# urbste/OpenImuCameraCalibrator

Measured on AMD Instinct MI355X. Metric: residual+Jacobian blocks/sec; wall-clock per LM iter, GoPro9 full calib, higher is better.
Workload: dtype f64

## Files before the change

include/oicc_hip.h:

```cpp
#ifndef OICC_HIP_H_
#define OICC_HIP_H_

#include <stdint.h>

#ifdef __cplusplus
extern "C" {
#endif

#define OICC_SPLINE_N 6
#define OICC_BIAS_SPLINE_N 3

typedef struct oicc_problem oicc_problem;

typedef enum oicc_status {
  OICC_OK = 0,
  OICC_ERR_INVALID_ARG = -1,
  OICC_ERR_NO_DEVICE = -2,
  OICC_ERR_HIP = -3,
  OICC_ERR_STATE = -4,
  OICC_ERR_UNSUPPORTED = -5
} oicc_status;

typedef enum oicc_camera_model {
  OICC_CAM_PINHOLE = 0,
// ... 189 lines not shown
int oicc_get_imu_intrinsics(const oicc_problem* p, double accl[6], double gyro[9]);
int oicc_get_bias_knots(const oicc_problem* p, double* accl_xyz, int64_t n_accl,
                        double* gyro_xyz, int64_t n_gyro);
int64_t oicc_get_num_accl_bias_knots(const oicc_problem* p);
int64_t oicc_get_num_gyro_bias_knots(const oicc_problem* p);
int oicc_get_mean_reprojection_error(oicc_problem* p, double* mean_px,
                                     int64_t* num_points);
int oicc_get_trajectory(oicc_problem* p, int64_t n, const int64_t* t_ns,
                        double* pose7, double* gyro3, double* accel3,
                        double* gyro_bias3, double* accl_bias3, uint8_t* valid);


int oicc_sew_knot_spacing_and_variance(int32_t device_ordinal, int32_t dims, int64_t n, const double* signal,
                                       const double* times, double quality, double min_dt, double max_dt,
                                       double* dt, double* variance, int32_t* num_evaluations);


int oicc_estimate_imu_to_camera_rotation(int32_t device_ordinal, int64_t n_vis, const double* t_vis_s, const double* q_vis_xyzw,
                                         int64_t n_imu, const double* t_imu_s, const double* gyro_xyz, double dt_imu,
                                         int32_t estimate_gyro_bias, double q_imu_to_cam_xyzw[4], double* time_offset_imu_to_cam,
                                         double gyro_bias[3], double* alignment_error, int32_t* iterations);

enum { OICC_ALLAN_GYRO = 0, OICC_ALLAN_ACC = 1, OICC_ALLAN_REPORT_SIZE = 6 };
int oicc_allan_factors(int64_t n, int32_t num_clusters, int32_t* factors, int32_t* num_factors);
int oicc_allan_variance(int32_t device_ordinal, int32_t channels, int64_t n, const double* samples, const double* t_s,
                        const double* scale, int32_t num_clusters, int32_t* num_factors, int32_t* factors, double* taus,
                        double* sigma2, double* freq, double* period, double* mean, double* device_ms);
int oicc_allan_fit(int32_t kind, int64_t num, const double* taus, const double* sigma2, double freq, double params_QNBKR[5],
                   double init_C[5], double report[6], int32_t* num_used, int32_t* iterations);

typedef struct oicc_ba oicc_ba;
enum { OICC_BA_POSITION = 1, OICC_BA_ORIENTATION = 2,
       OICC_BA_POINTS = 4 };
int oicc_ba_create(oicc_ba** out, int32_t device_ordinal);
void oicc_ba_destroy(oicc_ba* p);
const char* oicc_ba_last_error(const oicc_ba* p);
int oicc_ba_set_option(oicc_ba* p, const char* name, double value);
int oicc_ba_set_camera(oicc_ba* p, int32_t model, const double* intrinsics, int32_t n);
int oicc_ba_get_camera(const oicc_ba* p, double* intrinsics, int32_t n);
int oicc_ba_set_scene_points(oicc_ba* p, const double* xyzw, int64_t n);
int oicc_ba_get_scene_points(const oicc_ba* p, double* xyzw, int64_t n);
int oicc_ba_set_variable_points(oicc_ba* p, const uint8_t* variable, int64_t n);
int oicc_ba_set_views(oicc_ba* p, int64_t nv, const double* pose6, const int64_t* corner_offsets, const double* uv,
                      const int32_t* point_ids);
int oicc_ba_set_poses(oicc_ba* p, const double* pose6, int64_t nv);
int oicc_ba_get_poses(const oicc_ba* p, double* pose6, int64_t nv);
int oicc_ba_evaluate(oicc_ba* p, int32_t flags, int32_t intrinsics_mask, double* cost, double* H, double* g, int32_t Pcap);
int oicc_ba_optimize(oicc_ba* p, int32_t max_iters, int32_t flags, int32_t intrinsics_mask, oicc_summary* summary);
int oicc_ba_get_iterations(const oicc_ba* p, oicc_iteration* out, int32_t cap);
int oicc_ba_optimize_views(oicc_ba* p, int32_t max_iters, int32_t flags, int32_t* iterations, double* final_cost);
int oicc_ba_point_covariances(oicc_ba* p, double* cov9, int64_t n, double* variance_factor);
typedef struct oicc_ba_covariance_info {
  int32_t status;
  int32_t P, pose_dim, a;
  int32_t views_used;
  int32_t first_bad;
  int64_t num_residuals;
  double cost, variance_factor, rcond;
} oicc_ba_covariance_info;
int oicc_ba_estimate_covariance(oicc_ba* p, int32_t flags, int32_t intrinsics_mask, oicc_ba_covariance_info* info);
int oicc_ba_get_covariance_intrinsics(const oicc_ba* p, double* cov, int32_t a_capacity);
int oicc_ba_get_covariance_poses(const oicc_ba* p, double* blocks, int64_t nv);
int oicc_ba_get_covariance_pose_intrinsics(const oicc_ba* p, double* cross, int64_t nv);
int oicc_ba_get_covariance_timing(const oicc_ba* p, double ms[2]);
int oicc_ba_view_reprojection_errors(oicc_ba* p, double* mean_px);

enum {
  OICC_SIMU_THRESHOLDS = 10,
  OICC_SIMU_ACC_IMPOSSIBLE = 1,
  OICC_SIMU_TERM_SKIPPED = -1,
  OICC_SIMU_TERM_GRADIENT = 0,
  OICC_SIMU_TERM_FUNCTION = 1,
  OICC_SIMU_TERM_PARAMETER = 2,
  OICC_SIMU_TERM_MAX_ITERATIONS = 3,
  OICC_SIMU_TERM_MIN_RADIUS = 4,
  OICC_SIMU_TERM_INVALID_STEPS = 5,
  OICC_SIMU_TERM_EVAL_FAILED = 6
};
typedef struct oicc_static_imu_options {
  double gravity_magnitude;
  double init_interval_duration_s;
  double gyro_dt;
  int32_t interval_n_samples;
  int32_t min_num_intervals;
  int32_t win_size;
  int32_t acc_use_means;
  int32_t optimize_gyro_bias;
  int32_t reserved;
} oicc_static_imu_options;
typedef struct oicc_static_imu_report {
  int32_t th_mult;
  int32_t num_intervals[OICC_SIMU_THRESHOLDS];
  int32_t acc_iterations[OICC_SIMU_THRESHOLDS];
  int32_t acc_termination[OICC_SIMU_THRESHOLDS];
  int32_t gyro_num_blocks, gyro_iterations, gyro_termination;
  double norm_th;
  double init_acc_bias[3];
  double acc_final_cost[OICC_SIMU_THRESHOLDS];
  double gyro_init_bias[3];
  double gyro_initial_cost, gyro_final_cost;
  double ms_detector, ms_acc, ms_gyro;
} oicc_static_imu_report;
int oicc_static_imu_intervals(int32_t device_ordinal, int64_t n, const double* acc, int32_t num_thresholds,
                              const double* thresholds, int32_t win_size, int32_t capacity, int32_t* counts,
                              int32_t* intervals, double* norms, double* device_ms);
int oicc_static_imu_eval_acc(int32_t device_ordinal, int64_t num, const double* samples, double g_mag, const double* params,
                             double* residuals, double* jacobian, double* cost, double* gram, double* gradient);
int oicc_static_imu_eval_gyro(int32_t device_ordinal, int64_t n, const double* t_s, const double* gyro, int32_t num_blocks,
                              const int32_t* ranges, const double* g_versors, int32_t optimize_bias, double gyro_dt,
                              const double* params, double* residuals, double* jacobian, double* cost, double* gram,
                              double* gradient, double* device_ms);
int oicc_static_imu_calibrate(int32_t device_ordinal, int64_t n, const double* t_s, const double* acc, const double* gyro,
                              const oicc_static_imu_options* opt, double* acc_params, double* gyro_params,
                              oicc_static_imu_report* report);

typedef struct oicc_board_options {
  int32_t radius;
  float threshold_rel;
  int32_t max_candidates;
  int32_t subpix_iterations;
  double subpix_eps;
  int32_t batch;
  int32_t reserved;
} oicc_board_options;
typedef struct oicc_board_report {
  int32_t frames_found, frames_overflow;
  int32_t output_width, output_height;
  int64_t num_candidates;
  double ms_resize, ms_response, ms_candidates, ms_subpix, ms_marker;
  double ms_assembly_host;
  double ms_total;
} oicc_board_report;
typedef struct oicc_board_stages {
  uint8_t* gray;
  float* response;
  int32_t* candidates;
  double* refined;
  int32_t capacity;
  int32_t reserved;
} oicc_board_stages;
int oicc_board_output_size(int32_t width, int32_t height, double downsample_factor, int32_t* out_width, int32_t* out_height);
int oicc_board_radon_detect(int32_t device_ordinal, int32_t num_frames, int32_t width, int32_t height, int32_t channels,
                            const uint8_t* frames, double downsample_factor, int32_t W, int32_t H,
                            const oicc_board_options* opt, double* corners, int32_t* found, int32_t* candidates_per_frame,
                            oicc_board_report* report, const oicc_board_stages* stages);

int oicc_planar_ransac(int32_t device_ordinal, int32_t num_views, const int64_t* corner_offsets, const double* ab, const double* xy,
                       int32_t mode, double threshold, int32_t num_hypotheses, uint64_t seed, uint8_t* inlier,
                       int32_t* num_inliers, double* q, double* pose, int32_t* hypothesis_counts, double* device_ms);

int oicc_debug_bcr_plan(int32_t n, int32_t ghost, int32_t odd_only, int64_t* levels, int32_t cap_levels, int64_t info[3]);
int oicc_debug_bcr_join_plan(int32_t n, int32_t ghost, int32_t odd_only, int32_t b0, int32_t rtf, int32_t join_levels, int32_t budget,
                             int32_t build_inverts, int32_t* joined, int32_t cap_levels);

#ifdef __cplusplus
}
#endif
#endif
```

openimucameracalibrator_amd/_abi.py:

```python
import ctypes as C

c_i64p = C.POINTER(C.c_int64)
c_i32p = C.POINTER(C.c_int32)
c_dp = C.POINTER(C.c_double)
c_u8p = C.POINTER(C.c_uint8)


class Summary(C.Structure):
    _fields_ = [
        ("termination", C.c_int32), ("num_iterations", C.c_int32),
        ("num_successful_steps", C.c_int32), ("num_unsuccessful_steps", C.c_int32),
        ("num_parameters_tangent", C.c_int32), ("band_dim", C.c_int32),
        ("arrow_dim", C.c_int32), ("half_bandwidth", C.c_int32),
        ("num_residual_blocks", C.c_int64), ("num_residuals", C.c_int64),
        ("initial_cost", C.c_double), ("final_cost", C.c_double),
        ("final_radius", C.c_double), ("final_gradient_max_norm", C.c_double),
        ("seconds_total", C.c_double), ("seconds_jacobian", C.c_double),
        ("seconds_residual", C.c_double), ("seconds_linear_solver", C.c_double),
        ("message", C.c_char * 128),
        ("inner_sweeps", C.c_int32), ("line_search_steps", C.c_int32), ("inner_lm_iterations", C.c_int64),
        ("seconds_inner", C.c_double),
        ("seconds_setup", C.c_double),
    ]

# ... 151 lines not shown
    "view_reprojection_errors": (C.c_int, [HB, c_dp]),
    "point_covariances": (C.c_int, [HB, c_dp, C.c_int64, c_dp]),
    "estimate_covariance": (C.c_int, [HB, C.c_int32, C.c_int32, C.POINTER(BaCovarianceInfo)]),
    "get_covariance_intrinsics": (C.c_int, [HB, c_dp, C.c_int32]),
    "get_covariance_poses": (C.c_int, [HB, c_dp, C.c_int64]),
    "get_covariance_pose_intrinsics": (C.c_int, [HB, c_dp, C.c_int64]),
    "get_covariance_timing": (C.c_int, [HB, c_dp]),
}
BA_DEVICE_ONLY = ("point_covariances", "estimate_covariance", "get_covariance_intrinsics", "get_covariance_poses",
                  "get_covariance_pose_intrinsics", "get_covariance_timing")


class BoundBa:

    def __init__(self, lib, prefix):
        self.lib = lib
        self.prefix = prefix
        for name, (res, args) in BA_SIGNATURES.items():
            if name in BA_DEVICE_ONLY and prefix != "oicc_ba_" and not hasattr(lib, prefix + name):
                continue
            fn = getattr(lib, prefix + name)
            fn.restype = res
            fn.argtypes = args
            setattr(self, name, fn)


class Bound:

    def __init__(self, lib, prefix, device=True):
        self.lib = lib
        self.prefix = prefix
        table = dict(SIGNATURES)
        if device:
            table.update(DEVICE_ONLY)
        for name, (res, args) in table.items():
            fn = getattr(lib, prefix + name)
            fn.restype = res
            fn.argtypes = args
            setattr(self, name, fn)
        self.device = device


INNER_DEBUG_SIGNATURES = {
    "oicc_debug_inner_first_evaluations": (C.c_int, [H, C.c_int32, c_i32p, c_dp, C.c_int32]),
    "oicc_debug_inner_cholesky": (C.c_int, [C.c_int32, C.c_int32, C.c_int64, c_dp, c_dp, c_dp, c_u8p]),
}
INNER_ROUTES = ("set_kernel<0>", "set_kernel<1>", "set_kernel<2>", "wave_kernel", "shared: resident workgroups", "shared: launches")
INNER_KINDS = ("so3", "r3", "T_i_c", "gravity", "line_delay", "accl_bias", "gyro_bias", "accl_intrinsics", "gyro_intrinsics", "point")


def bind_inner_debug(lib, name):
    fn = getattr(lib, name)
    fn.restype, fn.argtypes = INNER_DEBUG_SIGNATURES[name]
    return fn


ALLAN_SIGNATURES = {
    "factors": (C.c_int, [C.c_int64, C.c_int32, c_i32p, c_i32p]),
    "variance": (C.c_int, [C.c_int32, C.c_int32, C.c_int64, c_dp, c_dp, c_dp, C.c_int32, c_i32p, c_i32p, c_dp,
                           c_dp, c_dp, c_dp, c_dp, c_dp]),
    "fit": (C.c_int, [C.c_int32, C.c_int64, c_dp, c_dp, C.c_double, c_dp, c_dp, c_dp, c_i32p, c_i32p]),
}


class BoundAllan:

    def __init__(self, lib, prefix):
        self.lib = lib
        self.prefix = prefix
        for name, (res, args) in ALLAN_SIGNATURES.items():
            fn = getattr(lib, prefix + name)
            fn.restype = res
            fn.argtypes = args
            setattr(self, name, fn)


class StaticImuOptions(C.Structure):
    _fields_ = [("gravity_magnitude", C.c_double), ("init_interval_duration_s", C.c_double), ("gyro_dt", C.c_double),
                ("interval_n_samples", C.c_int32), ("min_num_intervals", C.c_int32), ("win_size", C.c_int32),
                ("acc_use_means", C.c_int32), ("optimize_gyro_bias", C.c_int32), ("reserved", C.c_int32)]


class StaticImuReport(C.Structure):
    _fields_ = [("th_mult", C.c_int32), ("num_intervals", C.c_int32 * 10), ("acc_iterations", C.c_int32 * 10),
                ("acc_termination", C.c_int32 * 10), ("gyro_num_blocks", C.c_int32), ("gyro_iterations", C.c_int32),
                ("gyro_termination", C.c_int32), ("norm_th", C.c_double), ("init_acc_bias", C.c_double * 3),
                ("acc_final_cost", C.c_double * 10), ("gyro_init_bias", C.c_double * 3), ("gyro_initial_cost", C.c_double),
                ("gyro_final_cost", C.c_double), ("ms_detector", C.c_double), ("ms_acc", C.c_double), ("ms_gyro", C.c_double)]


STATIC_IMU_SIGNATURES = {
    "intervals": (C.c_int, [C.c_int32, C.c_int64, c_dp, C.c_int32, c_dp, C.c_int32, C.c_int32, c_i32p, c_i32p, c_dp, c_dp]),
    "eval_acc": (C.c_int, [C.c_int32, C.c_int64, c_dp, C.c_double, c_dp, c_dp, c_dp, c_dp, c_dp, c_dp]),
    "eval_gyro": (C.c_int, [C.c_int32, C.c_int64, c_dp, c_dp, C.c_int32, c_i32p, c_dp, C.c_int32, C.c_double, c_dp, c_dp, c_dp,
                            c_dp, c_dp, c_dp, c_dp]),
    "calibrate": (C.c_int, [C.c_int32, C.c_int64, c_dp, c_dp, c_dp, C.POINTER(StaticImuOptions), c_dp, c_dp,
                            C.POINTER(StaticImuReport)]),
}


class BoundStaticImu:

    def __init__(self, lib, prefix):
        self.lib = lib
        self.prefix = prefix
        for name, (res, args) in STATIC_IMU_SIGNATURES.items():
            fn = getattr(lib, prefix + name)
            fn.restype = res
            fn.argtypes = args
            setattr(self, name, fn)


class BoardOptions(C.Structure):
    _fields_ = [("radius", C.c_int32), ("threshold_rel", C.c_float), ("max_candidates", C.c_int32), ("subpix_iterations", C.c_int32),
                ("subpix_eps", C.c_double), ("batch", C.c_int32), ("reserved", C.c_int32)]


class BoardReport(C.Structure):
    _fields_ = [("frames_found", C.c_int32), ("frames_overflow", C.c_int32), ("output_width", C.c_int32), ("output_height", C.c_int32),
                ("num_candidates", C.c_int64), ("ms_resize", C.c_double), ("ms_response", C.c_double), ("ms_candidates", C.c_double),
                ("ms_subpix", C.c_double), ("ms_marker", C.c_double), ("ms_assembly_host", C.c_double), ("ms_total", C.c_double)]

    def as_dict(self):
        return {k: getattr(self, k) for k, _ in self._fields_}


class BoardStages(C.Structure):
    _fields_ = [("gray", c_u8p), ("response", C.POINTER(C.c_float)), ("candidates", c_i32p), ("refined", c_dp),
                ("capacity", C.c_int32), ("reserved", C.c_int32)]


BOARD_SIGNATURES = {
    "output_size": (C.c_int, [C.c_int32, C.c_int32, C.c_double, c_i32p, c_i32p]),
    "radon_detect": (C.c_int, [C.c_int32, C.c_int32, C.c_int32, C.c_int32, C.c_int32, c_u8p, C.c_double, C.c_int32, C.c_int32,
                               C.POINTER(BoardOptions), c_dp, c_i32p, c_i32p, C.POINTER(BoardReport), C.POINTER(BoardStages)]),
}


class BoundBoard:

    def __init__(self, lib, prefix):
        self.lib = lib
        self.prefix = prefix
        for name, (res, args) in BOARD_SIGNATURES.items():
            fn = getattr(lib, prefix + name)
            fn.restype = res
            fn.argtypes = args
            setattr(self, name, fn)


BCR_PLAN_SIGNATURES = {
    "plan": (C.c_int, [C.c_int32, C.c_int32, C.c_int32, c_i64p, C.c_int32, c_i64p]),
    "join_plan": (C.c_int, [C.c_int32] * 8 + [c_i32p, C.c_int32]),
}


class BoundBcrPlan:

    def __init__(self, lib, prefix):
        self.lib = lib
        self.prefix = prefix
        for name, (res, args) in BCR_PLAN_SIGNATURES.items():
            fn = getattr(lib, prefix + name)
            fn.restype = res
            fn.argtypes = args
            setattr(self, name, fn)


LM_RETRACT_SIGNATURES = {
    "retract": (C.c_int, [C.c_void_p, C.c_int32, C.c_double, c_i64p] + [c_dp] * 9),
}


class BoundLmRetract:

    def __init__(self, lib, prefix):
        self.lib = lib
        self.prefix = prefix
        for name, (res, args) in LM_RETRACT_SIGNATURES.items():
            fn = getattr(lib, prefix + name)
            fn.restype = res
            fn.argtypes = args
            setattr(self, name, fn)


PLANAR_RANSAC_SIGNATURES = {
    "ransac": (C.c_int, [C.c_int32, C.c_int32, c_i64p, c_dp, c_dp, C.c_int32, C.c_double, C.c_int32, C.c_uint64, c_u8p, c_i32p, c_dp,
                         c_dp, c_i32p, c_dp]),
}


class BoundPlanarRansac:

    def __init__(self, lib, prefix):
        self.lib = lib
        self.prefix = prefix
        for name, (res, args) in PLANAR_RANSAC_SIGNATURES.items():
            fn = getattr(lib, prefix + name)
            fn.restype = res
            fn.argtypes = args
            setattr(self, name, fn)
```

openimucameracalibrator_amd/csrc/kernels_bcr.hip:

```cpp
#include <hip/hip_runtime.h>
#include <mutex>
#include <unordered_map>
#include "oicc_device.h"
#include "lm_decide.h"
#include "lm_launch.h"
#include "lm_retract.h"
#include "../../include/oicc_hip.h"

namespace oicc {


struct BcrArgs {
  double* D;
  double* F;
  double* S;
  double* Lf;
  double* Mc;
  double* x;
  int32_t* fail;
  long long* prof;
  int n, a, Pb, rtf, LD;
  int delay;
  int o, s, p, m, pn;
  int64_t offS_in, offS_out;
  int carry;
  int last;
  int side;
  int top_l, top_r;
  int b0, ghost;
  const LmCtl* ctl;
};
#define BCR_RETURN_IF_DONE(A) do { if ((A).ctl != nullptr && (A).ctl->done != 0) return; } while (0)

__device__ __forceinline__ void bcr_lds_barrier() { asm volatile("s_waitcnt lgkmcnt(0)\n\ts_barrier" ::: "memory"); }
__device__ __forceinline__ double bcr_readlane(double v, int lane) {
  const int lo = __builtin_amdgcn_readlane(__double2loint(v), lane);
  const int hi = __builtin_amdgcn_readlane(__double2hiint(v), lane);
  return __hiloint2double(hi, lo);
}
typedef double bcr_v4d __attribute__((ext_vector_type(4)));

__device__ __forceinline__ void tri10(int t, int& xt, int& yt) {
  xt = t < 1 ? 0 : (t < 3 ? 1 : (t < 6 ? 2 : 3));
  yt = t - (xt * (xt + 1)) / 2;
}

template <int LD>
__device__ __forceinline__ void bcr_corner_solve(double* C, double* da, int* failp, int a, int tid, int wave, int lane) {
  const int a1 = a + 1;
  if (a1 <= 16) {
    if (wave == 0) {
      double av[16], dinv = 0.0;
#pragma unroll
      for (int c = 0; c < 16; ++c) av[c] = (c < a && lane < a1 && lane >= c) ? C[c * LD + lane] : 0.0;
      bool bad = false;
#pragma unroll
      for (int c = 0; c < 16; ++c) {
        if (c < a) {
          const double piv = bcr_readlane(av[c], c);
          bad |= !(piv > 0.0);
          const double y0 = __builtin_amdgcn_rsq(piv);
          const double g0 = piv * y0, h0 = 0.5 * y0;
          const double r0 = fma(-g0, h0, 0.5);
          const double g1 = fma(g0, r0, g0), h1 = fma(h0, r0, h0);
          const double r1 = fma(-g1, h1, 0.5);
          const double u = (av[c] + av[c]) * h1;
          const double l = fma(u, r1, u);
          av[c] = l;
          if (lane == c) { const double y1 = h1 + h1; dinv = fma(y1, r1, y1); }
#pragma unroll
          for (int c2 = c + 1; c2 < 16; ++c2) {
            const double lc2 = bcr_readlane(l, c2);
            av[c2] = fma(-l, lc2, av[c2]);
          }
        }
      }
#pragma unroll
      for (int c = 0; c < 16; ++c) if (c < a && lane < a1 && lane >= c) C[c * LD + lane] = av[c];
      double lt[16];
#pragma unroll
      for (int q = 0; q < 16; ++q) lt[q] = (q < a && lane < q) ? C[lane * LD + q] : 0.0;
      double z = lane < a ? C[lane * LD + a] : 0.0, xq_mine = 0.0;
#pragma unroll
      for (int q = 15; q >= 0; --q) {
        if (q < a) {
          const double xq = bcr_readlane(z * dinv, q);
          if (lane == q) xq_mine = xq;
          z = fma(-lt[q], xq, z);
        }
      }
      if (lane < a) da[lane] = xq_mine;
      if (bad && lane == 0) *failp = 1;
    }
    __syncthreads();
    return;
  }
  if (wave == 0) {
    bool bad = false;
    for (int c = 0; c < a; ++c) {
      double* col = C + c * LD;
      const double mine = lane < a1 ? col[lane] : 0.0;
      double piv = bcr_readlane(mine, c);
      if (!(piv > 0.0)) { bad = true; piv = 1.0; }
      const double d = sqrt(piv);
      const double l = lane == c ? d : (lane > c ? mine / d : 0.0);
      if (lane >= c && lane < a1) col[lane] = l;
      for (int c2 = c + 1; c2 < a; ++c2) {
        const double l2 = bcr_readlane(l, c2);
        if (lane >= c2 && lane < a1) C[c2 * LD + lane] -= l * l2;
      }
    }
    if (bad && lane == 0) *failp = 1;
    double z = lane < a ? C[lane * LD + a] : 0.0;
    const double dc = lane < a ? 1.0 / C[lane * LD + lane] : 0.0;
    double xq_mine = 0.0;
    for (int q = a - 1; q >= 0; --q) {
      const double xq = bcr_readlane(z * dc, q);
      if (lane == q) xq_mine = xq;
      const double l = lane < q ? C[lane * LD + q] : 0.0;
      z = fma(-l, xq, z);
    }
    if (lane < a) da[lane] = xq_mine;
  }
  __syncthreads();
}

constexpr int kBackWaves = 8;
constexpr int kInvWaves = 16;
constexpr int kInvLD = 145;

template <int XT>
__device__ __forceinline__ bcr_v4d bcri_z_tile(const double* W, int yt, int li, int lq) {
  constexpr int LD = kInvLD, K0 = 4 * XT, NK = 16 - K0;
  const double* py = W + lq * LD + 64 + 16 * yt + li;
  const double* px = W + lq * LD + 64 + 16 * XT + li;
  double vy[NK], vx[NK];
#pragma unroll
  for (int kk = 0; kk < NK; ++kk) { vy[kk] = py[4 * (K0 + kk) * LD]; vx[kk] = px[4 * (K0 + kk) * LD]; }
  asm volatile("" ::: "memory");
  bcr_v4d g = {0.0, 0.0, 0.0, 0.0}, g2 = {0.0, 0.0, 0.0, 0.0};
#pragma unroll
  for (int kk = 0; kk < NK; kk += 2) {
    g = __builtin_amdgcn_mfma_f64_16x16x4f64(vy[kk], vx[kk], g, 0, 0, 0);
    g2 = __builtin_amdgcn_mfma_f64_16x16x4f64(vy[kk + 1], vx[kk + 1], g2, 0, 0, 0);
  }
  g += g2;
  return g;
}

template <bool LAST, bool ZLDS>
__device__ __forceinline__ void bcri_tail(const BcrArgs& A, double* W, double* da, int* failp, const double* Fs, double* Zg, int tid, int wave, int lane, bool report,
                                          const double (&ttop)[16], const double ytop, double* x0s) {
  constexpr int LD = kInvLD, NW = kInvWaves, NT = 64 * NW, FLD = 65;
  const int li = lane & 15, lq = lane >> 4;
  const int a = A.a, a1 = a + 1;
  for (int t = wave; t < 10; t += NW) {
    int xt, yt; tri10(t, xt, yt);
    const bcr_v4d g = xt == 0 ? bcri_z_tile<0>(W, yt, li, lq) : (xt == 1 ? bcri_z_tile<1>(W, yt, li, lq) : (xt == 2 ? bcri_z_tile<2>(W, yt, li, lq) : bcri_z_tile<3>(W, yt, li, lq)));
#pragma unroll
    for (int r = 0; r < 4; ++r) {
      const int x = 16 * xt + li, y = 16 * yt + lq + 4 * r;
      if (LAST || ZLDS) { W[y * LD + x] = g[r]; if (xt != yt) W[x * LD + y] = g[r]; }
      else { Zg[y * 64 + x] = g[r]; if (xt != yt) Zg[x * 64 + y] = g[r]; }
    }
  }
  __syncthreads();
  if (!LAST) {
    if (report && tid == 0 && *failp) atomicOr(A.fail, 1);
    return;
  }
  const int rtf = A.rtf;
  if (wave < 4 * rtf) {
    const int t = wave >> 2, w = wave & 3;
    const double* pf = Fs + lq * FLD + 16 * t + li;
    const double* pz = W + lq * LD + 16 * w + li;
    double vf[16], vz[16];
#pragma unroll
    for (int kk = 0; kk < 16; ++kk) { vf[kk] = pf[4 * kk * FLD]; vz[kk] = pz[4 * kk * LD]; }
    asm volatile("" ::: "memory");
    bcr_v4d tq = {0.0, 0.0, 0.0, 0.0};
#pragma unroll
    for (int kk = 0; kk < 16; ++kk) tq = __builtin_amdgcn_mfma_f64_16x16x4f64(vf[kk], vz[kk], tq, 0, 0, 0);
#pragma unroll
    for (int r = 0; r < 4; ++r) W[(16 * w + li) * LD + 64 + 16 * t + lq + 4 * r] = tq[r];
  }
  __syncthreads();
  if (wave < (rtf * (rtf + 1)) / 2) {
    int t1 = 0, u = wave; while (u >= t1 + 1) { u -= t1 + 1; ++t1; }
    const int t2 = u;
    const double* pt = W + lq * LD + 64 + 16 * t1 + li;
    const double* pf = Fs + lq * FLD + 16 * t2 + li;
    double vt[16], vf[16];
#pragma unroll
    for (int kk = 0; kk < 16; ++kk) { vt[kk] = pt[4 * kk * LD]; vf[kk] = pf[4 * kk * FLD]; }
    asm volatile("" ::: "memory");
    bcr_v4d g = {0.0, 0.0, 0.0, 0.0};
#pragma unroll
    for (int kk = 0; kk < 16; ++kk) g = __builtin_amdgcn_mfma_f64_16x16x4f64(vf[kk], vt[kk], g, 0, 0, 0);
    const double* Sm = A.side != 0 ? A.Lf + (int64_t)A.last * (192 + a1) * 64 + 4096 + 64 * a1 : nullptr;
    double mc[4];
#pragma unroll
    for (int r = 0; r < 4; ++r) { const int q1 = 16 * t1 + li, q2 = 16 * t2 + lq + 4 * r; mc[r] = (q1 < a1 && q2 < a1) ? A.Mc[q1 * a1 + q2] + (Sm != nullptr ? Sm[q1 * a1 + q2] : 0.0) : 0.0; }
#pragma unroll
    for (int r = 0; r < 4; ++r) { const int q1 = 16 * t1 + li, q2 = 16 * t2 + lq + 4 * r; if (q1 < a1 && q2 < a1) W[q2 * LD + q1] = mc[r] - g[r]; }
  }
  __syncthreads();
  bcr_corner_solve<LD>(W, da, failp, a, tid, wave, lane);
  for (int q = tid; q < a; q += NT) A.x[A.Pb + q] = da[q];
  if (wave == 0) {
    const double* tc = W + lane * LD + 64;
    double v = tc[a];
    for (int q = 0; q < a; q += 8) {
      double t8[8], d8[8];
#pragma unroll
      for (int k = 0; k < 8; ++k) { const bool ok = q + k < a; t8[k] = ok ? tc[q + k] : 0.0; d8[k] = ok ? da[q + k] : 0.0; }
#pragma unroll
      for (int k = 0; k < 8; ++k) v = fma(-t8[k], d8[k], v);
    }
    const int gi = A.last * 64 + lane;
    if (gi < A.Pb) A.x[gi] = v;
    x0s[lane] = gi < A.Pb ? v : 0.0;
  }
  __syncthreads();
  if (tid == 0 && *failp) atomicOr(A.fail, 1);
  if (A.top_l >= 0 || A.top_r >= 0) {
    double sum_r = 0.0, sum_l = 0.0;
#pragma unroll
    for (int k = 0; k < 4; ++k) {
      const int r = wave + NW * k;
      const double xn = x0s[r], xa = r < a ? da[r] : 0.0;
      sum_r = fma(ttop[k], xn, sum_r);     sum_r = fma(ttop[4 + k], xa, sum_r);
      sum_l = fma(ttop[8 + k], xn, sum_l); sum_l = fma(ttop[12 + k], xa, sum_l);
    }
    W[wave * 64 + lane] = sum_r;
    W[(NW + wave) * 64 + lane] = sum_l;
    __syncthreads();
    if (wave < 2) {
      const int blk = wave == 0 ? A.top_r : A.top_l;
      double acc = 0.0;
#pragma unroll
      for (int w = 0; w < NW; ++w) acc += W[(wave * NW + w) * 64 + lane];
      const int gi = blk * 64 + lane;
      if (blk >= 0 && gi < A.Pb) A.x[gi] = ytop - acc;
    }
  }
}


struct BcrNoPark { __device__ __forceinline__ void operator()(double*) const {} };
template <bool LAST, bool PROF, bool ZLDS = false, class LoadD, class Park = BcrNoPark>
__device__ __forceinline__ void bcri_invert_body(const BcrArgs& A, const int i, LoadD load_d, const bool report = true, Park park = Park()) {
  constexpr int LD = kInvLD, NW = kInvWaves, NT = 64 * NW, NTILE = 20, SLOTS = (NTILE + NW - 1) / NW, RU = 128, NAW = 3, FLD = 65;
  static_assert(NW == 16, "the corner phases of block 0 take one tile per wave");
  extern __shared__ double lds[];
  const int tid = threadIdx.x, lane = tid & 63;
  const int wave = __builtin_amdgcn_readfirstlane(tid >> 6);
  const int li = lane & 15, lq = lane >> 4;
  double* const W = lds;
  double* const da = W + 64 * LD;
  int* const failp = reinterpret_cast<int*>(da + 64);
  double* const dg = da + 64 + 8;
  double* const Fs = dg + 256;
  const int a1 = A.a + 1;
  double* Zg = A.Lf + (int64_t)i * (192 + a1) * 64;
  const double* Fg = A.F + (int64_t)i * 64 * a1;
  const double* Sf = (LAST && A.side != 0) ? Zg + 4096 : nullptr;
  const bool prof = PROF && A.prof != nullptr && blockIdx.x == 0 && wave == 0;
  long long pc[8] = {0, 0, 0, 0, 0, 0, 0, 0};
  long long tprev = prof ? clock64() : 0;
#define BCR_MARK(k) do { if (PROF && prof) { const long long tn_ = clock64(); pc[k] += tn_ - tprev; tprev = tn_; } } while (0)
  if (tid == 0) *failp = 0;
  double ttop[16], ytop = 0.0;
#pragma unroll
  for (int k = 0; k < 16; ++k) ttop[k] = 0.0;
  if (LAST && (A.top_l >= 0 || A.top_r >= 0)) {
    const int64_t ru64 = (int64_t)(192 + a1) * 64;
    const double* Tr = A.Lf + (A.top_r >= 0 ? A.top_r : 0) * ru64 + 4096;
    const double* Tl = A.Lf + (A.top_l >= 0 ? A.top_l : 0) * ru64 + 4096;
#pragma unroll
    for (int k = 0; k < 4; ++k) {
      const int r = wave + NW * k;
      if (A.top_r >= 0) { ttop[k] = Tr[r * 64 + lane]; if (r < A.a) ttop[4 + k] = Tr[(128 + r) * 64 + lane]; }
      if (A.top_l >= 0) { ttop[8 + k] = Tl[(64 + r) * 64 + lane]; if (r < A.a) ttop[12 + k] = Tl[(128 + r) * 64 + lane]; }
    }
    if (wave == 0 && A.top_r >= 0) ytop = Tr[(128 + A.a) * 64 + lane];
    if (wave == 1 && A.top_l >= 0) ytop = Tl[(128 + A.a) * 64 + lane];
    asm volatile("" ::: "memory");
  }
  {
    constexpr int PER = 4096 / NT;
    double gd[PER], gf[PER];
#pragma unroll
    for (int k = 0; k < PER; ++k) {
      const int e = tid + k * NT;
      gd[k] = load_d(e);
      if (LAST) { const int c = e >> 6, q = e & 63; gf[k] = q < a1 ? Fg[c * a1 + q] + (Sf != nullptr ? Sf[c * a1 + q] : 0.0) : 0.0; }
    }
#pragma unroll
    for (int k = 0; k < PER; ++k) {
      const int e = tid + k * NT;
      const int c = e >> 6, r = e & 63;
      W[c * LD + r] = r >= c ? gd[k] : 0.0;
      if (c < 16 && r < 16) dg[c * 16 + r] = r >= c ? gd[k] : 0.0;
      W[c * LD + 64 + r] = r == c ? 1.0 : 0.0;
      if (LAST) Fs[c * FLD + r] = gf[k];
    }
    park(Fs);
  }
  __syncthreads();
  int t_rt[SLOTS], t_ct[SLOTS]; bool t_ok[SLOTS];
  bcr_v4d acc[SLOTS];
#pragma unroll
  for (int k = 0; k < SLOTS; ++k) {
    const int t = wave + NW * k;
    t_ok[k] = t < NTILE;
    int xt, yt; tri10(t < 10 ? t : (t < NTILE ? t - 10 : 0), xt, yt);
    if (t < 10) { t_rt[k] = xt; t_ct[k] = yt; } else { t_rt[k] = 4 + yt; t_ct[k] = xt; }
    const double* src = W + (16 * t_ct[k] + lq) * LD + 16 * t_rt[k] + li;
    acc[k][0] = src[0]; acc[k][1] = src[4 * LD]; acc[k][2] = src[8 * LD]; acc[k][3] = src[12 * LD];
  }
  BCR_MARK(0);
  const int prow = 16 + wave * 48 + (lane - 16);
  for (int p = 0; p < 4; ++p) {
    const int j0 = 16 * p;
    if (wave < NAW) {
      const int rho = lane < 16 ? j0 + lane : prow;
      const bool act = lane < 16 || (rho >= j0 + 16 && rho < RU && !(rho >= 64 && rho - 64 > j0 + 15));
      if (A.delay > 0 && wave > 0) for (int k = 0; k < A.delay; ++k) __builtin_amdgcn_s_sleep(16);
      const double* colp = lane < 16 ? dg + lane : W + j0 * LD + (act ? rho : 0);
      const int cstride = lane < 16 ? 16 : LD;
      double av[16];
#pragma unroll
      for (int c = 0; c < 16; ++c) { const double v = colp[c * cstride]; av[c] = (act && (lane >= 16 || lane >= c)) ? v : 0.0; }
      if (PROF && prof) { asm volatile("s_waitcnt lgkmcnt(0)" ::: "memory"); }
      BCR_MARK(6);
      bool bad = false;
#pragma unroll
      for (int c = 0; c < 16; ++c) {
        const double piv = bcr_readlane(av[c], c);
        bad |= !(piv > 0.0);
        const double y0 = __builtin_amdgcn_rsq(piv);
        const double g0 = piv * y0, h0 = 0.5 * y0;
        const double r0 = fma(-g0, h0, 0.5);
        const double g1 = fma(g0, r0, g0), h1 = fma(h0, r0, h0);
        const double r1 = fma(-g1, h1, 0.5);
        const double u = (av[c] + av[c]) * h1;
        const double l = fma(u, r1, u);
        av[c] = l;
#pragma unroll
        for (int c2 = c + 1; c2 < 16; ++c2) {
          const double lc2 = bcr_readlane(l, c2);
          av[c2] = fma(-l, lc2, av[c2]);
        }
      }
      if (PROF && prof) { asm volatile("s_nop 0" :: "v"(av[15])); }
      BCR_MARK(7);
      if (act && (lane >= 16 || wave == 0)) {
        double* cp = W + j0 * LD + rho;
#pragma unroll
        for (int c = 0; c < 16; ++c) cp[c * LD] = av[c];
      }
      if (bad && lane == 0) *failp = 1;
    }
    BCR_MARK(1);
    bcr_lds_barrier();
    BCR_MARK(2);
    if (p < 3) {
#pragma unroll
      for (int k = 0; k < SLOTS; ++k) {
        if (t_ok[k] && t_ct[k] > p && (t_rt[k] < 4 || t_rt[k] - 4 <= p)) {
          const double* pa = W + (j0 + lq) * LD + 16 * t_ct[k] + li;
          const double* pb = W + (j0 + lq) * LD + 16 * t_rt[k] + li;
          double va[4], vb[4];
#pragma unroll
          for (int kq = 0; kq < 4; ++kq) { va[kq] = pa[4 * kq * LD]; vb[kq] = -pb[4 * kq * LD]; }
#pragma unroll
          for (int kq = 0; kq < 4; ++kq) acc[k] = __builtin_amdgcn_mfma_f64_16x16x4f64(va[kq], vb[kq], acc[k], 0, 0, 0);
          if (t_ct[k] == p + 1) {
            double* dst = W + (16 * t_ct[k] + lq) * LD + 16 * t_rt[k] + li;
            dst[0] = acc[k][0]; dst[4 * LD] = acc[k][1]; dst[8 * LD] = acc[k][2]; dst[12 * LD] = acc[k][3];
            if (t_rt[k] == t_ct[k]) { dg[lq * 16 + li] = acc[k][0]; dg[(lq + 4) * 16 + li] = acc[k][1]; dg[(lq + 8) * 16 + li] = acc[k][2]; dg[(lq + 12) * 16 + li] = acc[k][3]; }
          }
        }
      }
    }
    BCR_MARK(3);
    bcr_lds_barrier();
    BCR_MARK(4);
  }
  BCR_MARK(4);
  bcri_tail<LAST, ZLDS>(A, W, da, failp, Fs, Zg, tid, wave, lane, report, ttop, ytop, dg);
  BCR_MARK(5);
  if (PROF && prof && lane == 0) for (int k = 0; k < 8; ++k) A.prof[k] = pc[k];
#undef BCR_MARK
}

template <bool LAST, bool PROF>
__global__ __launch_bounds__(64 * kInvWaves) void bcri_invert_kernel(BcrArgs A) {
  BCR_RETURN_IF_DONE(A);
  const int i = LAST ? A.last : A.o + A.s * (2 * (int)blockIdx.x + A.p);
  const double* Dg = A.D + (int64_t)i * 4096;
  const double* Sd = (LAST && A.side != 0) ? A.Lf + (int64_t)i * (192 + A.a + 1) * 64 : nullptr;
  bcri_invert_body<LAST, PROF>(A, i, [Dg, Sd](int e) { double v = Dg[e]; if (LAST && Sd != nullptr && (e & 63) >= (e >> 6)) v += Sd[e]; return v; });
}

struct BcrSchurGroup {
  int k, i, irs;
  bool hasL, hasR, ghostR;
  int xk, xt, yk, ny;
  bool store_t;
  bool leaves;
};
__device__ __forceinline__ BcrSchurGroup bcri_schur_group(const BcrArgs& A, int g, int piv) {
  BcrSchurGroup G;
  const int rtf = A.rtf;
  G.k = 2 * piv + A.p;
  G.i = A.o + G.k * A.s;
  G.hasL = G.k > 0;
  G.ghostR = A.ghost != 0 && G.k == A.m - 1;
  G.hasR = G.k < A.m - 1 || G.ghostR;
  G.irs = G.ghostR ? A.n : G.i + A.s;
  if (g < 4) { G.xk = 0; G.xt = g; G.yk = 0; G.ny = g + 1; G.store_t = true; }
  else if (g < 8) { G.xk = 1; G.xt = g - 4; G.yk = 0; G.ny = 4; G.store_t = false; }
  else if (g < 12) { G.xk = 1; G.xt = g - 8; G.yk = 1; G.ny = G.xt + 1; G.store_t = true; }
  else { g -= 12; G.yk = g / rtf; G.xt = g - G.yk * rtf; G.xk = 2; G.ny = G.yk < 2 ? 4 : G.xt + 1; G.store_t = G.yk == (G.hasL ? 0 : 1); }
  G.leaves = ((G.xk == 1 || G.yk == 1) && !G.hasR) || ((G.xk == 0 || G.yk == 0) && !G.hasL);
  return G;
}
struct BcrSchurGlobalOps {
  static constexpr bool kLateY = false;
  const double *px, *pz, *py; int sx, sy; bool okx, oky;
  __device__ __forceinline__ double x(int kk) const { return px[4 * kk * sx]; }
  __device__ __forceinline__ double z(int kk) const { return pz[4 * kk * 64]; }
  __device__ __forceinline__ double y(int kk) const { return oky ? py[4 * kk * sy] : 0.0; }
};
struct BcrSchurLdsOps {
  static constexpr bool kLateY = true;
  const double *px, *pz, *py; bool okx;
  __device__ __forceinline__ double x(int kk) const { return px[64 * kk]; }
  __device__ __forceinline__ double z(int kk) const { return pz[4 * kk * kInvLD]; }
  __device__ __forceinline__ double y(int kk) const { return py[64 * kk]; }
};
template <class Ops>
__device__ __forceinline__ void bcri_schur_body(const BcrArgs& A, const BcrSchurGroup& G, double (*Ts)[68], const Ops& ops, const bool active, const int wave, const int lane) {
  const int li = lane & 15, lq = lane >> 4;
  const int a1 = A.a + 1, s = A.s;
  const int k = G.k, i = G.i, il = i - s, irs = G.irs, xk = G.xk, xt = G.xt, yk = G.yk, ny = G.ny;
  const bool hasL = G.hasL, ghostR = G.ghostR, store_t = G.store_t, okx = ops.okx;
  double* Tg = A.Lf + (int64_t)i * (192 + a1) * 64 + 4096;
  double vx[16], vz[16], vy[16];
  if (active) {
#pragma unroll
    for (int kk = 0; kk < 16; ++kk) { vx[kk] = ops.x(kk); vz[kk] = ops.z(kk); }
    if (!Ops::kLateY) {
#pragma unroll
      for (int kk = 0; kk < 16; ++kk) vy[kk] = ops.y(kk);
    }
    asm volatile("" ::: "memory");
    bcr_v4d tq = {0.0, 0.0, 0.0, 0.0}, tq2 = {0.0, 0.0, 0.0, 0.0};
#pragma unroll
    for (int kk = 0; kk < 16; kk += 2) {
      tq = __builtin_amdgcn_mfma_f64_16x16x4f64(okx ? vx[kk] : 0.0, vz[kk], tq, 0, 0, 0);
      tq2 = __builtin_amdgcn_mfma_f64_16x16x4f64(okx ? vx[kk + 1] : 0.0, vz[kk + 1], tq2, 0, 0, 0);
    }
    tq += tq2;
    const int trow0 = xk == 0 ? 16 * xt : (xk == 1 ? 64 + 16 * xt : 128 + 16 * xt);
#pragma unroll
    for (int r = 0; r < 4; ++r) {
      const int row = lq + 4 * r;
      Ts[row][16 * wave + li] = tq[r];
      if (store_t && (xk != 2 || 16 * xt + row < a1)) Tg[(int64_t)(trow0 + row) * 64 + 16 * wave + li] = tq[r];
    }
  }
  __syncthreads();
  if (!active || wave >= ny) return;
  const int yt = wave;
  const int kn = hasL ? (k - 2 + A.p) / 2 : 0;
  const bool il_is_pivot = (kn & 1) == A.pn;
  const bool swap = xk == 1 && yk == 0 && !il_is_pivot && !ghostR;
  double vt[16];
  if (Ops::kLateY) {
#pragma unroll
    for (int kk = 0; kk < 16; ++kk) vy[kk] = ops.y(kk);
  }
#pragma unroll
  for (int kk = 0; kk < 16; ++kk) vt[kk] = Ts[li][4 * kk + lq];
  asm volatile("" ::: "memory");
  bcr_v4d gq = {0.0, 0.0, 0.0, 0.0}, gq2 = {0.0, 0.0, 0.0, 0.0};
  if (swap) {
#pragma unroll
    for (int kk = 0; kk < 16; kk += 2) {
      gq = __builtin_amdgcn_mfma_f64_16x16x4f64(vt[kk], vy[kk], gq, 0, 0, 0);
      gq2 = __builtin_amdgcn_mfma_f64_16x16x4f64(vt[kk + 1], vy[kk + 1], gq2, 0, 0, 0);
    }
  } else {
#pragma unroll
    for (int kk = 0; kk < 16; kk += 2) {
      gq = __builtin_amdgcn_mfma_f64_16x16x4f64(vy[kk], vt[kk], gq, 0, 0, 0);
      gq2 = __builtin_amdgcn_mfma_f64_16x16x4f64(vy[kk + 1], vt[kk + 1], gq2, 0, 0, 0);
    }
  }
  gq += gq2;
  const int ils = hasL ? il : i;
  double* Dl = A.D + (int64_t)ils * 4096; double* Dr = A.D + (int64_t)irs * 4096;
  double* Fl = A.F + (int64_t)ils * 64 * a1; double* Fr = A.F + (int64_t)irs * 64 * a1;
  double* So = A.S + (A.offS_out + kn) * 4096;
  const bool to_side = A.side != 0 && !hasL;
  double* Sd = A.Lf + (int64_t)irs * (192 + a1) * 64;
#pragma unroll
  for (int r = 0; r < 4; ++r) {
    const double v = -gq[r];
    if (xk == 1 && yk == 0) {
      if (!swap) { const int x = 16 * xt + li, y = 16 * yt + lq + 4 * r; So[y * 64 + x] = v; }
      else       { const int y = 16 * yt + li, x = 16 * xt + lq + 4 * r; So[x * 64 + y] = v; }
    } else if (xk < 2) {
      const int x = 16 * xt + li, y = 16 * yt + lq + 4 * r;
      if (to_side) { if (x >= y) Sd[y * 64 + x] = v; }
      else if (x >= y && v != 0.0) unsafeAtomicAdd((xk == 0 ? Dl : Dr) + y * 64 + x, v);
    } else if (yk < 2) {
      const int q = 16 * xt + li, y = 16 * yt + lq + 4 * r;
      if (to_side) { if (q < a1) Sd[4096 + y * a1 + q] = v; }
      else if (q < a1 && v != 0.0) unsafeAtomicAdd((yk == 0 ? Fl : Fr) + y * a1 + q, v);
    } else {
      const int q1 = 16 * xt + li, q2 = 16 * yt + lq + 4 * r;
      if (to_side) { if (q1 < a1 && q2 <= q1) { Sd[4096 + 64 * a1 + q1 * a1 + q2] = v; Sd[4096 + 64 * a1 + q2 * a1 + q1] = v; } }
      else if (q1 < a1 && q2 <= q1 && v != 0.0) {
        unsafeAtomicAdd(A.Mc + q1 * a1 + q2, v);
        if (q1 != q2) unsafeAtomicAdd(A.Mc + q2 * a1 + q1, v);
      }
    }
  }
}

__global__ __launch_bounds__(256) void bcri_schur_kernel(BcrArgs A) {
  BCR_RETURN_IF_DONE(A);
  __shared__ double Ts[16][68];
  const int tid = threadIdx.x, lane = tid & 63;
  const int wave = __builtin_amdgcn_readfirstlane(tid >> 6);
  const int li = lane & 15, lq = lane >> 4;
  const int a1 = A.a + 1;
  if ((int)blockIdx.y == (int)gridDim.y - 1 && A.carry > 0) {
    const int m = A.carry;
    const double* src = A.S + (A.offS_in + (m - 1)) * 4096; double* dst = A.S + (A.offS_out + (m - 1) / 2) * 4096;
    for (int e = (int)blockIdx.x * 256 + tid; e < 4096; e += (int)gridDim.x * 256) dst[e] = src[e];
    return;
  }
  const BcrSchurGroup G = bcri_schur_group(A, (int)blockIdx.x, (int)blockIdx.y);
  if (G.leaves) return;
  const double* SL = A.S + (A.offS_in + (G.hasL ? G.k - 1 : 0)) * 4096;
  const double* SR = A.S + (A.offS_in + G.k) * 4096;
  const double* Fg = A.F + (int64_t)G.i * 64 * a1;
  const double* Zg = A.Lf + (int64_t)G.i * (192 + a1) * 64;
  auto border_ptr = [&](int kind, int t, int& stride, bool& ok) -> const double* {
    if (kind == 0) { stride = 64; ok = true; return SL + lq * 64 + 16 * t + li; }
    if (kind == 1) { stride = 64; ok = true; return SR + lq * 64 + 16 * t + li; }
    const int q = 16 * t + li; ok = q < a1; stride = a1; return Fg + lq * a1 + (ok ? q : 0);
  };
  BcrSchurGlobalOps ops;
  ops.px = border_ptr(G.xk, G.xt, ops.sx, ops.okx);
  ops.py = border_ptr(G.yk, wave < G.ny ? wave : 0, ops.sy, ops.oky);
  ops.pz = Zg + lq * 64 + 16 * wave + li;
  bcri_schur_body(A, G, Ts, ops, true, wave, lane);
}

constexpr int kInvLdsDoubles = 64 * kInvLD + 64 + 8 + 256;
constexpr int kJoinLdsDoubles = kInvLdsDoubles + 5 * 1024 + 16 * 68;
__global__ __launch_bounds__(64 * kInvWaves) void bcri_invert_schur_kernel(BcrArgs A) {
  BCR_RETURN_IF_DONE(A);
  const BcrSchurGroup G = bcri_schur_group(A, (int)blockIdx.x, (int)blockIdx.y);
  if (G.leaves) return;
  const int tid = threadIdx.x, lane = tid & 63;
  const int wave = __builtin_amdgcn_readfirstlane(tid >> 6);
  const int li = lane & 15, lq = lane >> 4;
  const int a1 = A.a + 1;
  const double* SL = A.S + (A.offS_in + (G.hasL ? G.k - 1 : 0)) * 4096;
  const double* SR = A.S + (A.offS_in + G.k) * 4096;
  const double* Fg = A.F + (int64_t)G.i * 64 * a1;
  const int kv = tid >> 4, l = tid & 15;
  auto border_at = [&](int kind, int t) -> double {
    if (kind == 0) return SL[kv * 64 + 16 * t + l];
    if (kind == 1) return SR[kv * 64 + 16 * t + l];
    const int q = 16 * t + l; return q < a1 ? Fg[kv * a1 + q] : 0.0;
  };
  double bx = border_at(G.xk, G.xt), by[4];
#pragma unroll
  for (int t = 0; t < 4; ++t) by[t] = t < G.ny ? border_at(G.yk, t) : 0.0;
  asm volatile("" ::: "memory");
  const double* Dg = A.D + (int64_t)G.i * 4096;
  const bool report = (int)blockIdx.x == (G.hasL ? 0 : 8);
  bcri_invert_body<false, false, true>(A, G.i, [Dg](int e) { return Dg[e]; }, report,
    [&](double* P) {
      P[tid] = bx;
#pragma unroll
      for (int t = 0; t < 4; ++t) P[1024 * (1 + t) + tid] = by[t];
    });
  extern __shared__ double lds[];
  const double* W = lds;
  const double* P = lds + kInvLdsDoubles;
  double (*Ts)[68] = reinterpret_cast<double (*)[68]>(lds + kInvLdsDoubles + 5 * 1024);
  const bool active = wave < 4;
  BcrSchurLdsOps ops;
  ops.okx = true;
  ops.px = P + lq * 16 + li;
  ops.py = P + 1024 * (1 + (active && wave < G.ny ? wave : 0)) + lq * 16 + li;
  ops.pz = W + lq * kInvLD + 16 * (active ? wave : 0) + li;
  bcri_schur_body(A, G, Ts, ops, active, wave, lane);
}

struct BcrOwn {
  int e = -1, code = -1;
  double sc0 = 0.0, d2 = 0.0, g = 0.0;
  const double* x = nullptr; double* xc = nullptr;
};
constexpr int kRetractPark = 12;
template <int NB>
__device__ __forceinline__ BcrOwn bcr_retract_claim(const BcrArgs& A, const RetractReq& R, const SolveBuffers& sb, int b_lo, int b_hi, bool arrow_wg, int tid) {
  BcrOwn o; o.x = R.x; o.xc = R.xc;
  NormalEq ne = R.ne;
  if (A.ctl != nullptr) { o.x = A.ctl->xp[0]; o.xc = A.ctl->xp[1]; ne.base = A.ctl->nep[0]; }
  const int e_hi = b_hi * 64 < A.Pb ? b_hi * 64 : A.Pb;
  if (tid < 64 * NB) { const int e = b_lo * 64 + tid; if (e < e_hi) o.e = e; }
  else if (tid < 64 * NB + A.a && arrow_wg) o.e = A.Pb + (tid - 64 * NB);
  if (o.e >= 0) { o.code = R.rmap[o.e]; o.sc0 = sb.scale[o.e]; o.d2 = sb.D2[o.e]; o.g = ne.g()[o.e]; }
  return o;
}
__device__ __forceinline__ int bcr_rm_steps(int kind) { return kind == kRmEucl ? 1 : (kind == kRmTic ? 6 : 3); }
__device__ __forceinline__ int bcr_rm_params(int kind) { return kind == kRmEucl ? 1 : (kind == kRmTic ? 7 : (kind == kRmSo3 || kind == kRmPt ? 4 : 3)); }
__device__ __forceinline__ void bcr_retract_park(const SolveBuffers& sb, const BcrOwn& o, double* rpark, int stride, int tid) {
  if (o.code < 0) return;
  const int kind = o.code & 7; const int64_t po = o.code >> 3;
  const int nd = bcr_rm_steps(kind), np = bcr_rm_params(kind);
  for (int c = 0; c < np; ++c) rpark[c * stride + tid] = o.x[po + c];
  for (int c = 1; c < nd; ++c) rpark[(6 + c) * stride + tid] = sb.scale[o.e + c];
}
template <int OW>
__device__ __forceinline__ void bcr_retract_finish(const BcrArgs& A, const RetractReq& R, const SolveBuffers& sb, const BcrOwn& o, const double* xflat, int e_base,
                                                   const double* xarrow, const double* rpark, int stride, double* red, int tid, int wave, int lane) {
  __syncthreads();
  if (blockIdx.x == 0 && tid == 0) {
    if (A.ctl != nullptr) { if (A.ctl->stamps != nullptr && A.ctl->seq < A.ctl->trace_cap) A.ctl->stamps[3 * A.ctl->seq + 1] = wall_clock64(); }
    else *R.ne.cost() = 0.0;
  }
  double step_sq = 0.0, x_sq = 0.0, model = 0.0;
  if (o.e >= 0) {
    auto step_at = [&](int e) { return e >= A.Pb ? xarrow[e - A.Pb] : xflat[e - e_base]; };
    model = lm_model_term(step_at(o.e), o.d2, o.g, o.sc0);
    if (o.code >= 0) {
      const int kind = o.code & 7;
      const double alpha = R.alpha;
      const int nd = bcr_rm_steps(kind), np = bcr_rm_params(kind);
      double d[6], sc[6], pv[7];
#pragma unroll
      for (int c = 0; c < 6; ++c) { d[c] = c < nd ? step_at(o.e + c) : 0.0; sc[c] = c == 0 ? o.sc0 : (c < nd ? rpark[(6 + c) * stride + tid] : 0.0); }
#pragma unroll
      for (int c = 0; c < 7; ++c) pv[c] = c < np ? rpark[c * stride + tid] : 0.0;
      double* out = o.xc + (o.code >> 3);
      if (kind == kRmSo3) lm_store_so3(lm_retract_so3(Quat{pv[0], pv[1], pv[2], pv[3]}, d, sc, alpha), pv, out, step_sq, x_sq);
      else if (kind == kRmEucl) lm_retract_eucl(pv[0], d[0], sc[0], alpha, out, step_sq, x_sq);
      else if (kind == kRmAb || kind == kRmGb) { const double bound = kind == kRmAb ? R.max_ab : R.max_gb; for (int c = 0; c < 3; ++c) lm_retract_box(pv[c], d[c], sc[c], alpha, bound, out + c, step_sq, x_sq); }
      else if (kind == kRmPt) lm_retract_point(pv, d, sc, alpha, out, step_sq, x_sq);
      else if (kind == kRmTic) lm_retract_tic(pv, d, sc, alpha, out, step_sq, x_sq);
    }
  }
  if (wave < OW) {
#pragma unroll
    for (int off = 32; off > 0; off >>= 1) { step_sq += __shfl_xor(step_sq, off); x_sq += __shfl_xor(x_sq, off); model += __shfl_xor(model, off); }
    if (lane == 0) { red[wave] = step_sq; red[64 + wave] = x_sq; red[128 + wave] = model; }
  }
  __syncthreads();
  if (tid < 3) {
    double acc = 0.0;
    for (int w = 0; w < OW; ++w) acc += red[64 * tid + w];
    unsafeAtomicAdd(tid == 0 ? &sb.st->step_norm_sq : (tid == 1 ? &sb.st->x_norm_sq : &sb.st->model_cost_change), acc);
  }
}

__global__ __launch_bounds__(64 * kBackWaves) void bcri_backward_kernel(BcrArgs A) {
  BCR_RETURN_IF_DONE(A);
  __shared__ double xs[192];
  __shared__ double part[kBackWaves][64];
  const int tid = threadIdx.x, lane = tid & 63;
  const int wave = __builtin_amdgcn_readfirstlane(tid >> 6);
  const int a = A.a, a1 = a + 1, s = A.s;
  const int kp = 2 * (int)blockIdx.x + A.p;
  const int i = A.o + kp * s, il = i - s;
  const bool hasL = kp > 0;
  const bool hasR = kp < A.m - 1 || A.ghost != 0;
  const int ir = kp < A.m - 1 ? i + s : A.n;
  const double* Tg = A.Lf + (int64_t)i * (192 + a1) * 64 + 4096;
  constexpr int RW = 192 / kBackWaves;
  double lv[RW];
#pragma unroll
  for (int k = 0; k < RW; ++k) {
    const int r = wave + kBackWaves * k;
    const bool ok = r < 128 + a && (hasL || r >= 64) && (hasR || r < 64 || r >= 128);
    lv[k] = ok ? Tg[r * 64 + lane] : 0.0;
  }
  const double yv = wave == 0 ? Tg[(128 + a) * 64 + lane] : 0.0;
  double xin = 0.0;
  if (tid < 64) { const int gi = il * 64 + tid; xin = (hasL && gi < A.Pb) ? A.x[gi] : 0.0; }
  else if (tid < 128) { const int gi = ir * 64 + (tid - 64); xin = (hasR && gi < A.Pb) ? A.x[gi] : 0.0; }
  else if (tid < 128 + a) xin = A.x[A.Pb + (tid - 128)];
  if (tid < 192) xs[tid] = xin;
  __syncthreads();
  double sum = 0.0;
#pragma unroll
  for (int k = 0; k < RW; ++k) { const int r = wave + kBackWaves * k; sum = fma(lv[k], r < 128 + a ? xs[r] : 0.0, sum); }
  part[wave][lane] = sum;
  __syncthreads();
  if (wave == 0) {
    double acc = 0.0;
#pragma unroll
    for (int w = 0; w < kBackWaves; ++w) acc += part[w][lane];
    const int gi = i * 64 + lane;
    if (gi < A.Pb) A.x[gi] = yv - acc;
  }
}

template <bool RETRACT>
__device__ __forceinline__ void bcri_backward2_body(const BcrArgs& A, int ou, int pu, int mu, int npiv_upper, int orphan_l, int orphan_r, const RetractReq& R, const SolveBuffers& sb) {
  constexpr int NW = 16, RW1 = 192 / NW, RW2 = 192 / (NW / 2);
  __shared__ double xw[6][64];
  __shared__ double part[NW][64];
  double* const xs0 = xw[0]; double* const xs1 = xw[2]; double* const xs2 = xw[4]; double* const xs3 = xw[5];
  const int tid = threadIdx.x, lane = tid & 63;
  const int wave = __builtin_amdgcn_readfirstlane(tid >> 6);
  const int a = A.a, a1 = a + 1, s = A.s, n = A.n;
  const int64_t ru64 = (int64_t)(192 + a1) * 64;
  const int lone_ix = (int)blockIdx.x - npiv_upper;
  const bool lone = lone_ix >= 0;
  const bool lone_l = lone && orphan_l >= 0 && lone_ix == 0, lone_r = lone && !lone_l;
  const int ku = 2 * (int)blockIdx.x + pu;
  const int j = lone_l ? orphan_l - s : (lone_r ? orphan_r + s : ou + ku * 2 * s);
  const int jl = j - 2 * s, jr = j + 2 * s;
  const bool ghost = A.ghost != 0;
  const bool has_jl = lone_r || (!lone && ku > 0);
  const bool has_jr = lone_l || (!lone && (ku < mu - 1 || ghost));
  const int jrs = (!lone && ku == mu - 1) ? n : jr;
  const int half = wave >> 3, hw = wave & 7;
  const int ci = half == 0 ? j - s : j + s;
  const bool child = lone ? (half == 0 ? lone_r : lone_l) : (half == 0 ? ci >= A.o : ci <= A.o + (A.m - 1) * s);
  const bool child_hasL = half == 0 ? has_jl : !lone;
  const bool child_hasR = half == 0 ? (!lone || ghost) : has_jr;
  auto xin = [&](int blk, int r) { const int gi = blk * 64 + r; return gi < A.Pb ? A.x[gi] : 0.0; };
  if (tid < 64) xs0[tid] = has_jl ? xin(jl, tid) : 0.0;
  else if (tid < 128) xs2[tid - 64] = has_jr ? xin(jrs, tid - 64) : 0.0;
  else if (tid < 192) xs3[tid - 128] = tid - 128 < a ? A.x[A.Pb + (tid - 128)] : 0.0;
  else if (tid < 256 && lone) xs1[tid - 192] = (lone_r && ghost) ? xin(n, tid - 192) : 0.0;
  __shared__ double rpark[RETRACT ? kRetractPark : 1][384];
  BcrOwn own;
  if (RETRACT) {
    const int b_lo = j - 2 > 0 ? j - 2 : 0;
    int b_hi = j + 2 < n ? j + 2 : n;
    if (!lone && (int)blockIdx.x == npiv_upper - 1 && orphan_r < 0) b_hi = n;
    own = bcr_retract_claim<5>(A, R, sb, b_lo, b_hi, blockIdx.x == 0, tid);
  }
  double l1[RW1], l2[RW2], y1 = 0.0, y2 = 0.0;
  {
    const double* T1 = A.Lf + (lone ? 0 : j) * ru64 + 4096;
#pragma unroll
    for (int k = 0; k < RW1; ++k) {
      const int r = wave + NW * k;
      const bool ok = !lone && r < 128 + a && (has_jl || r >= 64) && (has_jr || r < 64 || r >= 128);
      l1[k] = ok ? T1[r * 64 + lane] : 0.0;
    }
    if (wave == 0 && !lone) y1 = T1[(128 + a) * 64 + lane];
    const double* T2 = A.Lf + (child ? ci : 0) * ru64 + 4096;
#pragma unroll
    for (int k = 0; k < RW2; ++k) {
      const int r = hw + 8 * k;
      const bool ok = child && r < 128 + a && (child_hasL || r >= 64) && (child_hasR || r < 64 || r >= 128);
      l2[k] = ok ? T2[r * 64 + lane] : 0.0;
    }
    if (hw == 0 && child) y2 = T2[(128 + a) * 64 + lane];
  }
  if (RETRACT) bcr_retract_park(sb, own, &rpark[0][0], 384, tid);
  __syncthreads();
  if (!lone) {
    double sum = 0.0;
#pragma unroll
    for (int k = 0; k < RW1; ++k) {
      const int r = wave + NW * k;
      const double xv = r < 64 ? xs0[r] : (r < 128 ? xs2[r - 64] : (r < 128 + a ? xs3[r - 128] : 0.0));
      sum = fma(l1[k], xv, sum);
    }
    part[wave][lane] = sum;
    __syncthreads();
    if (wave == 0) {
      double acc = 0.0;
#pragma unroll
      for (int w = 0; w < NW; ++w) acc += part[w][lane];
      const double xv = y1 - acc;
      const int gi = j * 64 + lane;
      xs1[lane] = gi < A.Pb ? xv : 0.0;
      if (gi < A.Pb) A.x[gi] = xv;
    }
    __syncthreads();
  }
  {
    const double* xl = half == 0 ? xs0 : xs1;
    const double* xr = half == 0 ? xs1 : xs2;
    double sum = 0.0;
#pragma unroll
    for (int k = 0; k < RW2; ++k) {
      const int r = hw + 8 * k;
      const double xv = r < 64 ? xl[r] : (r < 128 ? xr[r - 64] : (r < 128 + a ? xs3[r - 128] : 0.0));
      sum = fma(l2[k], xv, sum);
    }
    part[wave][lane] = sum;
    __syncthreads();
    if (hw == 0 && child) {
      double acc = 0.0;
#pragma unroll
      for (int w = 0; w < 8; ++w) acc += part[8 * half + w][lane];
      const int gi = ci * 64 + lane;
      const double xv = y2 - acc;
      if (gi < A.Pb) A.x[gi] = xv;
      if (RETRACT) xw[half == 0 ? 1 : 3][lane] = gi < A.Pb ? xv : 0.0;
    }
  }
  if (RETRACT) bcr_retract_finish<6>(A, R, sb, own, &xw[0][0], (j - 2) * 64, xs3, &rpark[0][0], 384, &part[0][0], tid, wave, lane);
}
__global__ __launch_bounds__(1024) void bcri_backward2_kernel(BcrArgs A, int ou, int pu, int mu, int npiv_upper, int orphan_l, int orphan_r) {
  BCR_RETURN_IF_DONE(A);
  bcri_backward2_body<false>(A, ou, pu, mu, npiv_upper, orphan_l, orphan_r, RetractReq{}, SolveBuffers{});
}
__global__ __launch_bounds__(1024) void bcri_backward2_retract_kernel(BcrArgs A, int ou, int pu, int mu, int npiv_upper, int orphan_l, int orphan_r, RetractReq R, SolveBuffers sb) {
  BCR_RETURN_IF_DONE(A);
  bcri_backward2_body<true>(A, ou, pu, mu, npiv_upper, orphan_l, orphan_r, R, sb);
}

__device__ __forceinline__ void bcr_build_body(const NormalEq& ne, const TangentLayout& tl, const SolveBuffers& sb, int reuse_diagonal, double min_diag,
                                               double max_diag, const BcrArgs& A, const int64_t tid, const int64_t nthreads) {
  const int Pb = tl.Pb, a = tl.a, W = tl.W, a1 = a + 1, hb = tl.hb, n = A.n;
  const int64_t r0 = (int64_t)A.b0 * 64;
  const double radius = sb.radius;
  if (tid == 0) {
    sb.st->radius = radius; sb.st->model_cost_change = 0.0; sb.st->step_norm_sq = 0.0; sb.st->x_norm_sq = 0.0; sb.st->cand_cost = 0.0; sb.st->chol_failed = 0;
    if (sb.ctl != nullptr && sb.ctl->stamps != nullptr && sb.ctl->seq < sb.ctl->trace_cap) sb.ctl->stamps[3 * sb.ctl->seq] = wall_clock64();
  }
  auto damp = [&](int64_t i, double hii) -> double {
    const double sc = sb.scale[i];
    return (reuse_diagonal ? sb.diag[i] : fmin(fmax(hii * sc * sc, min_diag), max_diag)) / radius;
  };
  for (int64_t i = tid; i < tl.P; i += nthreads) {
    const double hii = i < Pb ? ne.band()[i * W] : ne.C()[(i - Pb) * a + (i - Pb)];
    const double sc = sb.scale[i];
    double d;
    if (!reuse_diagonal) { d = fmin(fmax(hii * sc * sc, min_diag), max_diag); sb.diag[i] = d; }
    else d = sb.diag[i];
    sb.D2[i] = d / radius;
  }
  for (int64_t e = tid; e < (int64_t)n * 4096; e += nthreads) {
    const int blk = int(e >> 12), c = int(e >> 6) & 63, r = int(e) & 63;
    {
      const int64_t gc = r0 + (int64_t)blk * 64 + c, gr = r0 + (int64_t)blk * 64 + r;
      double v = 0.0;
      if (r >= c) {
        const int k = r - c;
        if (gr < Pb) {
          if (k <= hb) v = ne.band()[gc * W + k] * sb.scale[gc] * sb.scale[gr];
          if (k == 0) v += damp(gc, ne.band()[gc * W]);
        } else if (gc >= Pb && k == 0) v = 1.0;
      }
      A.D[e] = v;
    }
    if (blk < n - 1 || A.ghost != 0) {
      const bool right = (blk & 1) == A.p || blk == n - 1;
      const int64_t gr = r0 + (int64_t)(blk + 1) * 64 + (right ? r : c);
// ... 34 lines not shown
  ne.base = s_c.nep[0]; sb.radius = s_c.radius; reuse_diagonal = s_c.reuse_diagonal;
  return true;
}

__global__ void bcr_build_kernel(NormalEq ne, TangentLayout tl, SolveBuffers sb, int reuse_diagonal, double min_diag,
                                 double max_diag, BcrArgs A) {
  if (!lm_ctl_build_inputs(ne, sb, reuse_diagonal, blockIdx.x == 0 && threadIdx.x == 0)) return;
  bcr_build_body(ne, tl, sb, reuse_diagonal, min_diag, max_diag, A, (int64_t)blockIdx.x * blockDim.x + threadIdx.x, (int64_t)gridDim.x * blockDim.x);
}

__global__ __launch_bounds__(64 * kInvWaves) void bcri_build_invert_kernel(NormalEq ne, TangentLayout tl, SolveBuffers sb, int reuse_diagonal,
                                                                           double min_diag, double max_diag, BcrArgs A) {
  const int npiv = (A.n + 1 - A.p) / 2;
  if (!lm_ctl_build_inputs(ne, sb, reuse_diagonal, (int)blockIdx.x == npiv && threadIdx.x == 0)) return;
  if ((int)blockIdx.x >= npiv) {
    bcr_build_body(ne, tl, sb, reuse_diagonal, min_diag, max_diag, A, (int64_t)((int)blockIdx.x - npiv) * blockDim.x + threadIdx.x, (int64_t)((int)gridDim.x - npiv) * blockDim.x);
    return;
  }
  const int i = 2 * (int)blockIdx.x + A.p;
  const int Pb = tl.Pb, Wd = tl.W, hb = tl.hb;
  const double radius = sb.radius;
  const double* band = ne.band();
  bcri_invert_body<false, false>(A, i, [&](int e) -> double {
    const int c = e >> 6, r = e & 63, k = r - c;
    const int64_t gc = (int64_t)(A.b0 + i) * 64 + c, gr = (int64_t)(A.b0 + i) * 64 + r;
    if (k < 0) return 0.0;
    if (gr >= Pb) return (gc >= Pb && k == 0) ? 1.0 : 0.0;
    const double sc = sb.scale[gc];
    double v = k <= hb ? band[gc * Wd + k] * sc * sb.scale[gr] : 0.0;
    if (k == 0) v += (reuse_diagonal ? sb.diag[gc] : fmin(fmax(band[gc * Wd] * sc * sc, min_diag), max_diag)) / radius;
    return v;
  }, false);
}

static void bcr_allow_lds(const void* fn, size_t bytes) {
  static std::mutex mu;
  static std::unordered_map<const void*, uint64_t> done;
  int dev = 0; (void)hipGetDevice(&dev);
  const uint64_t bit = 1ull << (dev & 63);
  {
    std::lock_guard<std::mutex> lock(mu);
    uint64_t& mask = done[fn];
    if (dev < 64 && (mask & bit)) return;
    mask |= bit;
  }
  (void)hipFuncSetAttribute(fn, hipFuncAttributeMaxDynamicSharedMemorySize, (int)bytes);
}


static inline int bcr_blocks(int Pb) { return (Pb + 63) / 64; }
static size_t bcr_lds_inv() { return (size_t)kInvLdsDoubles * sizeof(double); }
static int64_t bcr_coupling_slots(int nblk) { return 2 * (int64_t)nblk + 40; }
static void bcr_carve(BcrArgs& A, double* w, int nblk, int a1) {
  A.D = w; w += (int64_t)nblk * 4096;
  A.F = w; w += (int64_t)nblk * 64 * a1;
  A.S = w; w += bcr_coupling_slots(nblk) * 4096;
  A.Lf = w;
}
static int64_t bcr_carve_doubles(int nblk, int a1) { return (int64_t)nblk * 4096 + (int64_t)nblk * 64 * a1 + bcr_coupling_slots(nblk) * 4096 + (int64_t)nblk * (192 + a1) * 64 + 64; }
bool bcr_applicable(const TangentLayout& tl) { return tl.Pb >= 1 && tl.hb <= 64 && tl.a + 1 <= 64; }
int64_t bcr_workspace_doubles(const TangentLayout& tl) {
  if (!bcr_applicable(tl)) return 0;
  const int64_t n = bcr_blocks(tl.Pb), a1 = tl.a + 1;
  return bcr_carve_doubles(int(n), int(a1));
}

struct BcrLevels {
  int origin[40], strides[40], parity[40], active[40], npivs[40];
  int64_t offS[41];
  int nlev = 0, last = 0;
  int64_t off_end = 0;
};
static BcrLevels bcr_plan(int n, int ghost, bool odd_only) {
  BcrLevels L;
  const int g = ghost != 0 ? 1 : 0;
  int o = 0, s = 1, m = n; int64_t off = 0;
  while (m > 1) {
    const int p = (odd_only || (m & 1) == 0) ? 1 : 0;
    const int npiv = (m + 1 - p) / 2, l = L.nlev++;
    L.origin[l] = o; L.strides[l] = s; L.parity[l] = p; L.active[l] = m; L.npivs[l] = npiv; L.offS[l] = off;
    off += m - 1 + g; o += (1 - p) * s; s *= 2; m -= npiv;
  }
  L.offS[L.nlev] = off; L.off_end = off; L.last = o;
  return L;
}
static void bcr_set_level(BcrArgs& A, const BcrLevels& L, int l) {
  A.o = L.origin[l]; A.s = L.strides[l]; A.p = L.parity[l]; A.m = L.active[l];
  A.pn = l + 1 < L.nlev ? L.parity[l + 1] : 1;
  A.offS_in = L.offS[l]; A.offS_out = L.offS[l + 1];
}
static bool bcr_fused_build(int n, const long long* prof) { return n >= 2 && n <= 512 && prof == nullptr; }
static bool bcr_launch_build(const NormalEq& ne, const TangentLayout& tl, const SolveBuffers& sb, int reuse_diagonal, double min_diag, double max_diag, BcrArgs A, const BcrLevels& L, hipStream_t st) {
  const int n = A.n;
  const bool fused_build = bcr_fused_build(n, A.prof);
  const int64_t work = (int64_t)(n + A.ghost) * 4096;
  A.o = 0; A.s = 1; A.p = 1; A.m = n; A.pn = 1; A.offS_in = 0; A.offS_out = 0;
  if (L.nlev > 0) bcr_set_level(A, L, 0);
  if (fused_build) {
    int grid = int((work + 1023) / 1024); if (grid > 1024) grid = 1024;
    bcr_allow_lds(reinterpret_cast<const void*>(bcri_build_invert_kernel), bcr_lds_inv());
    hipLaunchKernelGGL(bcri_build_invert_kernel, dim3(L.npivs[0] + grid), dim3(64 * kInvWaves), bcr_lds_inv(), st, ne, tl, sb, reuse_diagonal, min_diag, max_diag, A);
  } else {
    int grid = int((work + 255) / 256); if (grid > 4096) grid = 4096;
    hipLaunchKernelGGL(bcr_build_kernel, dim3(grid), dim3(256), 0, st, ne, tl, sb, reuse_diagonal, min_diag, max_diag, A);
  }
  return fused_build;
}
struct BcrJoin { int on = 0; int budget = 0; };
static bool bcr_level_joined(const BcrJoin& J, bool prof, int ghost, int b0, bool carry, bool in_build, int npiv, int rtf) {
  return J.on != 0 && !prof && ghost == 0 && b0 == 0 && !carry && !in_build && (int64_t)npiv * (12 + 3 * rtf) <= (int64_t)J.budget;
}
static int bcr_launch_forward(BcrArgs A, bool level0_inverted, const BcrLevels& L, hipStream_t st, const BcrJoin& J = BcrJoin()) {
  using KernelFn = void (*)(BcrArgs);
  KernelFn k_inv = A.prof ? bcri_invert_kernel<false, true> : bcri_invert_kernel<false, false>;
  bcr_allow_lds(reinterpret_cast<const void*>(k_inv), bcr_lds_inv());
  const int g = A.ghost != 0 ? 1 : 0;
  int joined = 0;
  for (int l = 0; l < L.nlev; ++l) {
    const int m = L.active[l], npiv = L.npivs[l];
    bcr_set_level(A, L, l);
    A.side = (l == L.nlev - 1 && L.parity[l] == 0) ? 1 : 0;
    const bool carry = g != 0 && (m & 1) != 0;
    A.carry = carry ? m : 0;
    if (bcr_level_joined(J, A.prof != nullptr, A.ghost, A.b0, carry, level0_inverted && l == 0, npiv, A.rtf)) {
      const size_t lds_join = (size_t)kJoinLdsDoubles * sizeof(double);
      bcr_allow_lds(reinterpret_cast<const void*>(bcri_invert_schur_kernel), lds_join);
      hipLaunchKernelGGL(bcri_invert_schur_kernel, dim3(12 + 3 * A.rtf, npiv), dim3(64 * kInvWaves), lds_join, st, A);
      ++joined;
      continue;
    }
    BcrArgs Ai = A; if (l != 0) Ai.prof = nullptr;
    if (!(level0_inverted && l == 0)) hipLaunchKernelGGL(k_inv, dim3(npiv), dim3(64 * kInvWaves), bcr_lds_inv(), st, Ai);
    hipLaunchKernelGGL(bcri_schur_kernel, dim3(12 + 3 * A.rtf, npiv + (carry ? 1 : 0)), dim3(256), 0, st, A);
  }
  return joined;
}
static bool bcr_launch_back(BcrArgs A, const BcrLevels& L, int top, hipStream_t st, const RetractReq* R = nullptr, const SolveBuffers* sb = nullptr) {
  int l = top;
  bool fused = false;
  if (l >= 0 && !(l & 1)) { bcr_set_level(A, L, l); hipLaunchKernelGGL(bcri_backward_kernel, dim3(L.npivs[l]), dim3(64 * kBackWaves), 0, st, A); --l; }
  for (; l >= 1; l -= 2) {
    const int lo = l - 1;
    const int orphan_l = (L.parity[lo] == 0 && L.parity[l] == 1) ? L.origin[lo] : -1;
    const int orphan_r = (((L.active[lo] - 1) & 1) == L.parity[lo] && ((L.active[l] - 1) & 1) != L.parity[l]) ? L.origin[lo] + (L.active[lo] - 1) * L.strides[lo] : -1;
    bcr_set_level(A, L, lo);
    const dim3 grid(L.npivs[l] + (orphan_l >= 0 ? 1 : 0) + (orphan_r >= 0 ? 1 : 0));
    if (lo == 0 && R != nullptr) {
      hipLaunchKernelGGL(bcri_backward2_retract_kernel, grid, dim3(1024), 0, st, A, L.origin[l], L.parity[l], L.active[l], L.npivs[l], orphan_l, orphan_r, *R, *sb);
      fused = true;
    } else hipLaunchKernelGGL(bcri_backward2_kernel, grid, dim3(1024), 0, st, A, L.origin[l], L.parity[l], L.active[l], L.npivs[l], orphan_l, orphan_r);
  }
  return fused;
}
static bool bcr_launch_last_and_back(BcrArgs A, const BcrLevels& L, hipStream_t st, const RetractReq* R = nullptr, const SolveBuffers* sb = nullptr) {
  using KernelFn = void (*)(BcrArgs);
  KernelFn k_inv_last = bcri_invert_kernel<true, false>;
  const size_t lds_inv_last = bcr_lds_inv() + (size_t)64 * 65 * sizeof(double);
  bcr_allow_lds(reinterpret_cast<const void*>(k_inv_last), lds_inv_last);
  const int nlev = L.nlev;
  A.o = 0; A.s = 0; A.p = 1; A.m = 1; A.pn = 1; A.offS_in = 0; A.offS_out = 0; A.carry = 0;
  A.last = L.last; A.top_l = -1; A.top_r = -1; A.side = (nlev >= 1 && L.parity[nlev - 1] == 0) ? 1 : 0;
  if (nlev >= 1) {
    const int t = nlev - 1;
    A.top_r = L.last + L.strides[t];
    if (L.parity[t] == 0) A.top_l = L.last - L.strides[t];
  }
  hipLaunchKernelGGL(k_inv_last, dim3(1), dim3(64 * kInvWaves), lds_inv_last, st, A);
  return bcr_launch_back(A, L, nlev - 2, st, R, sb);
}

int bcr_route(const TangentLayout& tl, const SolveBuffers& sb) {
  if (!bcr_applicable(tl) || tl.a + 1 > sb.bcr_max_border || sb.ws == nullptr || sb.ws_doubles < bcr_workspace_doubles(tl)) return kRouteNone;
  if (sb.algo != 0 && sb.algo != 4) return kRouteNone;
  return bcr_fused_build(bcr_blocks(tl.Pb), sb.prof) ? kRouteBcrFused : kRouteBcrUnfused;
}
int launch_bcr_solve(const NormalEq& ne, const TangentLayout& tl, const SolveBuffers& sb, int reuse_diagonal,
                     double min_diag, double max_diag, hipStream_t st, const RetractReq* retract, bool* fused) {
  if (fused) *fused = false;
  if (bcr_route(tl, sb) == kRouteNone) return -1;
  const int n = bcr_blocks(tl.Pb), a1 = tl.a + 1;
  BcrArgs A{};
  bcr_carve(A, sb.ws, n, a1);
  A.Mc = sb.Mc; A.x = sb.step_s; A.fail = &sb.st->chol_failed; A.prof = sb.prof;
  A.n = n; A.a = tl.a; A.Pb = tl.Pb; A.delay = sb.bcr_delay;
  A.rtf = (a1 + 15) / 16; A.ctl = sb.ctl;
  const BcrLevels L = bcr_plan(n, 0, false);
  const bool inverted = bcr_launch_build(ne, tl, sb, reuse_diagonal, min_diag, max_diag, A, L, st);
  BcrJoin J; J.on = sb.bcr_join; J.budget = sb.bcr_join_budget;
  const int joined = bcr_launch_forward(A, inverted, L, st, J);
  if (sb.bcr_joined != nullptr) { sb.bcr_joined[0] = joined; sb.bcr_joined[1] += joined; }
  const bool honour = retract != nullptr && retract->on != 0 && retract->rmap != nullptr && retract->alpha == 1.0 && L.nlev >= 3 && A.ghost == 0 && A.b0 == 0;
  RetractReq R{}; if (honour) { R = *retract; R.ne = ne; }
  const bool did = bcr_launch_last_and_back(A, L, st, honour ? &R : nullptr, &sb);
  if (fused) *fused = did;
  return 0;
}

__global__ void bcr_dist_pack_kernel(BcrArgs A, int64_t off_final, double* msg) {
  const int a1 = A.a + 1; const int64_t fsz = (int64_t)64 * a1;
  const int64_t total = 3 * 4096 + 2 * fsz + (int64_t)a1 * a1;
  for (int64_t e = (int64_t)blockIdx.x * blockDim.x + threadIdx.x; e < total; e += (int64_t)gridDim.x * blockDim.x) {
    double v;
    if (e < 4096) v = A.D[e];
    else if (e < 4096 + fsz) v = A.F[e - 4096];
    else if (e < 2 * 4096 + fsz) v = A.ghost ? A.S[off_final * 4096 + (e - 4096 - fsz)] : 0.0;
    else if (e < 3 * 4096 + fsz) v = A.ghost ? A.D[(int64_t)A.n * 4096 + (e - 2 * 4096 - fsz)] : 0.0;
    else if (e < 3 * 4096 + 2 * fsz) v = A.ghost ? A.F[(int64_t)A.n * fsz + (e - 3 * 4096 - fsz)] : 0.0;
    else v = A.Mc[e - 3 * 4096 - 2 * fsz];
    msg[e] = v;
  }
}
__global__ void bcr_dist_top_kernel(BcrArgs T, const double* msgs, int64_t piece) {
  const int N = T.n, a1 = T.a + 1; const int64_t fsz = (int64_t)64 * a1;
  const int64_t nD = (int64_t)N * 4096, nF = (int64_t)N * fsz, nS = (int64_t)(N - 1) * 4096, nC = (int64_t)a1 * a1;
  for (int64_t e = (int64_t)blockIdx.x * blockDim.x + threadIdx.x; e < nD + nF + nS + nC; e += (int64_t)gridDim.x * blockDim.x) {
    if (e < nD) {
      const int k = int(e >> 12); const int64_t o = e & 4095;
      T.D[e] = msgs[k * piece + o] + (k > 0 ? msgs[(k - 1) * piece + 2 * 4096 + fsz + o] : 0.0);
    } else if (e < nD + nF) {
      const int64_t f = e - nD; const int k = int(f / fsz); const int64_t o = f - k * fsz;
      T.F[f] = msgs[k * piece + 4096 + o] + (k > 0 ? msgs[(k - 1) * piece + 3 * 4096 + fsz + o] : 0.0);
    } else if (e < nD + nF + nS) {
      const int64_t f = e - nD - nF; const int k = int(f >> 12), c = int(f >> 6) & 63, r = int(f) & 63;
      const double* src = msgs + k * piece + 4096 + fsz;
      T.S[f] = (k & 1) ? src[c * 64 + r] : src[r * 64 + c];
    } else {
      const int64_t f = e - nD - nF - nS;
      double v = 0.0;
      for (int k = 0; k < N; ++k) v += msgs[k * piece + 3 * 4096 + 2 * fsz + f];
      T.Mc[f] = v;
    }
  }
}
__global__ void bcr_dist_scatter_kernel(BcrArgs A, const double* xt, int N, int rank) {
  const int t = threadIdx.x;
  if (t < 64) A.x[t] = xt[rank * 64 + t];
  else if (t < 128) { if (A.ghost) A.x[(int64_t)A.n * 64 + (t - 64)] = xt[(rank + 1) * 64 + (t - 64)]; }
  else if (t < 128 + A.a) A.x[A.Pb + (t - 128)] = xt[N * 64 + (t - 128)];
}
__global__ void bcr_dist_pack_x_kernel(BcrArgs A, double* slot, int64_t arrow_at) {
  const int64_t nx = (int64_t)A.n * 64;
  for (int64_t e = (int64_t)blockIdx.x * blockDim.x + threadIdx.x; e < nx + A.a; e += (int64_t)gridDim.x * blockDim.x) {
    if (e < nx) slot[e] = A.x[e]; else slot[arrow_at + (e - nx)] = A.x[A.Pb + (e - nx)];
  }
}
__global__ void bcr_dist_unpack_x_kernel(const double* slots, int64_t piece, const int32_t* b0s, int N, int Pb, int a, int64_t arrow_at, double* x) {
  for (int64_t i = (int64_t)blockIdx.x * blockDim.x + threadIdx.x; i < (int64_t)Pb + a; i += (int64_t)gridDim.x * blockDim.x) {
    if (i >= Pb) { x[i] = slots[arrow_at + (i - Pb)]; continue; }
    const int blk = int(i >> 6); int k = 0; while (k + 1 < N && blk >= b0s[k + 1]) ++k;
    x[i] = slots[k * piece + (i - (int64_t)b0s[k] * 64)];
  }
}

int64_t bcr_dist_workspace_doubles(const TangentLayout& tl, int n_loc, int nranks) {
  const int a1 = tl.a + 1;
  return bcr_carve_doubles(n_loc + 1, a1) + ((int64_t)(n_loc + 1) * 64 + tl.a + 8) + bcr_carve_doubles(nranks, a1) + ((int64_t)nranks * 64 + tl.a + 8) + 2 * (int64_t)a1 * a1 + 64;
}
int64_t bcr_dist_msg_doubles(const TangentLayout& tl) { const int a1 = tl.a + 1; return 3 * 4096 + 2 * (int64_t)64 * a1 + (int64_t)a1 * a1; }

namespace {
struct DistViews { BcrArgs A, T; double* xt; };
DistViews bcr_dist_views(const TangentLayout& tl, const SolveBuffers& sb, const BcrDist& d) {
  const int a1 = tl.a + 1, ghost = d.rank + 1 < d.nranks ? 1 : 0;
  DistViews v{};
  double* w = d.ws;
  BcrArgs& A = v.A;
  bcr_carve(A, w, d.n_loc + 1, a1); w += bcr_carve_doubles(d.n_loc + 1, a1);
  A.x = w; w += (int64_t)(d.n_loc + 1) * 64 + tl.a + 8;
  A.Mc = w; w += (int64_t)a1 * a1;
  A.fail = &sb.st->chol_failed; A.prof = nullptr; A.n = d.n_loc; A.a = tl.a; A.Pb = (d.n_loc + ghost) * 64; A.delay = sb.bcr_delay;
  A.rtf = (a1 + 15) / 16; A.ctl = nullptr; A.b0 = d.b0; A.ghost = ghost;
  BcrArgs& T = v.T;
  bcr_carve(T, w, d.nranks, a1); w += bcr_carve_doubles(d.nranks, a1);
  T.x = w; w += (int64_t)d.nranks * 64 + tl.a + 8;
  T.Mc = w; w += (int64_t)a1 * a1;
  T.fail = A.fail; T.prof = nullptr; T.n = d.nranks; T.a = tl.a; T.Pb = d.nranks * 64; T.delay = sb.bcr_delay; T.rtf = A.rtf; T.ctl = nullptr; T.b0 = 0; T.ghost = 0;
  v.xt = T.x;
  return v;
}
}

int launch_bcr_dist_forward(const NormalEq& ne, const TangentLayout& tl, const SolveBuffers& sb_in, int reuse_diagonal, double min_diag, double max_diag, const BcrDist& d, hipStream_t st) {
  if (!bcr_applicable(tl) || tl.a + 1 > sb_in.bcr_max_border || d.ws == nullptr || d.n_loc < 1 || d.nranks < 2 || d.ws_doubles < bcr_dist_workspace_doubles(tl, d.n_loc, d.nranks)) return -1;
  DistViews v = bcr_dist_views(tl, sb_in, d);
  SolveBuffers sb = sb_in; sb.Mc = v.A.Mc; sb.ctl = nullptr;
  const BcrLevels L = bcr_plan(v.A.n, v.A.ghost, true);
  const bool inverted = bcr_launch_build(ne, tl, sb, reuse_diagonal, min_diag, max_diag, v.A, L, st);
  bcr_launch_forward(v.A, inverted, L, st);
  const int64_t total = bcr_dist_msg_doubles(tl);
  hipLaunchKernelGGL(bcr_dist_pack_kernel, dim3(int((total + 255) / 256)), dim3(256), 0, st, v.A, L.off_end, d.msg + (int64_t)d.rank * d.msg_piece);
  return 0;
}
int launch_bcr_dist_middle(const TangentLayout& tl, const SolveBuffers& sb, const BcrDist& d, hipStream_t st) {
  DistViews v = bcr_dist_views(tl, sb, d);
  const int a1 = tl.a + 1, N = d.nranks;
  const int64_t work = (int64_t)N * 4096 + (int64_t)N * 64 * a1 + (int64_t)(N - 1) * 4096 + (int64_t)a1 * a1;
  hipLaunchKernelGGL(bcr_dist_top_kernel, dim3(int(std::min<int64_t>(1024, (work + 255) / 256))), dim3(256), 0, st, v.T, d.msg, d.msg_piece);
  const BcrLevels LT = bcr_plan(N, 0, true);
  bcr_launch_forward(v.T, false, LT, st);
  bcr_launch_last_and_back(v.T, LT, st);
  hipLaunchKernelGGL(bcr_dist_scatter_kernel, dim3(1), dim3(256), 0, st, v.A, v.xt, N, d.rank);
  BcrArgs A = v.A;
  const BcrLevels L = bcr_plan(A.n, A.ghost, true);
  bcr_launch_back(A, L, L.nlev - 1, st);
  const int64_t nx = (int64_t)A.n * 64 + A.a;
  hipLaunchKernelGGL(bcr_dist_pack_x_kernel, dim3(int((nx + 255) / 256)), dim3(256), 0, st, v.A, d.xg + (int64_t)d.rank * d.x_piece, (int64_t)d.max_loc * 64);
  return 0;
}
void launch_bcr_dist_finish(const TangentLayout& tl, const SolveBuffers& sb, const BcrDist& d, hipStream_t st) {
  const int64_t n = (int64_t)tl.Pb + tl.a;
  hipLaunchKernelGGL(bcr_dist_unpack_x_kernel, dim3(int(std::min<int64_t>(1024, (n + 255) / 256))), dim3(256), 0, st, d.xg, d.x_piece, d.d_b0, d.nranks, tl.Pb, tl.a, (int64_t)d.max_loc * 64, sb.step_s);
}

}

extern "C" int oicc_debug_bcr_plan(int32_t n, int32_t ghost, int32_t odd_only, int64_t* levels, int32_t cap_levels, int64_t info[3]) {
  if (n < 1 || levels == nullptr || info == nullptr) return OICC_ERR_INVALID_ARG;
  const oicc::BcrLevels L = oicc::bcr_plan(n, ghost, odd_only != 0);
  if (L.nlev > cap_levels) return OICC_ERR_INVALID_ARG;
  for (int l = 0; l < L.nlev; ++l) {
    int64_t* o = levels + 6 * l;
    o[0] = L.origin[l]; o[1] = L.strides[l]; o[2] = L.parity[l]; o[3] = L.active[l]; o[4] = L.npivs[l]; o[5] = L.offS[l];
  }
  info[0] = L.last; info[1] = L.off_end; info[2] = oicc::bcr_coupling_slots(n + (ghost != 0 ? 1 : 0));
  return L.nlev;
}

extern "C" int oicc_debug_bcr_join_plan(int32_t n, int32_t ghost, int32_t odd_only, int32_t b0, int32_t rtf, int32_t join_levels, int32_t budget,
                                        int32_t build_inverts, int32_t* joined, int32_t cap_levels) {
  if (n < 1 || joined == nullptr || rtf < 1 || rtf > 4 || budget < 0 || b0 < 0) return OICC_ERR_INVALID_ARG;
  const oicc::BcrLevels L = oicc::bcr_plan(n, ghost, odd_only != 0);
  if (L.nlev > cap_levels) return OICC_ERR_INVALID_ARG;
  oicc::BcrJoin J; J.on = join_levels; J.budget = budget;
  const bool in_build0 = build_inverts < 0 ? oicc::bcr_fused_build(n, nullptr) : build_inverts != 0;
  for (int l = 0; l < L.nlev; ++l) {
    const bool carry = ghost != 0 && (L.active[l] & 1) != 0;
    joined[l] = oicc::bcr_level_joined(J, false, ghost, b0, carry, in_build0 && l == 0, L.npivs[l], rtf) ? 1 : 0;
  }
  return L.nlev;
}
```

openimucameracalibrator_amd/csrc/oicc_device.h:

```cpp
#pragma once
#include <cstdint>

namespace oicc {

struct ParamLayout {
  int64_t so3, r3, ab, gb, tic, g, ld, ai, gi, total;
  int32_t n_so3, n_r3, n_ab, n_gb;
  int64_t pts; int32_t n_pts, pad_;
};

struct TangentLayout {
  const int32_t* so3;
  const int32_t* r3;
  const int32_t* ab;
  const int32_t* gb;
  int32_t tic, g, ld, ai, gi;
  int32_t P, Pb, a, hb, W;
  const int32_t* pts;
  int32_t n_pts, a_pts;
};

struct NormalEq {
  double* base;
  int64_t off_E, off_C, off_g, off_cost, total;
  __host__ __device__ double* band() const { return base; }
  __host__ __device__ double* Et() const { return base + off_E; }
  __host__ __device__ double* C() const { return base + off_C; }
  __host__ __device__ double* g() const { return base + off_g; }
  __host__ __device__ double* cost() const { return base + off_cost; }
};

struct ViewData {
  int64_t n_views, n_corners;
  const int32_t* corner_view;
  const double* corner_u; const double* corner_v;
  const double* corner_isx; const double* corner_isy;
  const int32_t* corner_pt;
  const int64_t* view_c0;
  const int32_t* view_s_so3; const int32_t* view_s_r3;
  const double* view_u_so3; const double* view_u_r3;
  const uint8_t* view_rs;
  const int64_t* chunk_c0; const int32_t* chunk_n; int32_t n_chunks;
  int32_t max_chunk_n;
};

struct ImuData {
  int64_t n;
  const int32_t* s_so3; const int32_t* s_r3; const int32_t* s_b;
  const double* u_so3; const double* u_r3; const double* u_b;
  const double* mx; const double* my; const double* mz;
  const double* w;
  const int64_t* chunk_i0; const int32_t* chunk_n; int32_t n_chunks;
};

struct EvalCtx {
  const double* x;
  ParamLayout pl;
  TangentLayout tl;
  NormalEq ne;
  const double* pts;
  double inv_so3_dt, inv_r3_dt;
  double intr[10];
  int32_t cam_model;
  int32_t gs_unit_loss;
  int32_t rs_time_in_seconds;
  double* dbg_res;
  double* dbg_jac;
  int32_t only_kind;
  long long* prof;
  int prof_repeat;
};

struct LmState {
  double radius, gradient_max_norm;
  double model_cost_change, step_norm_sq, x_norm_sq, cand_cost;
  int32_t chol_failed, pad;
};
constexpr size_t kLmStepResultsOffset = 2 * sizeof(double);

struct LmIterRec {
  int32_t iteration, step_is_successful;
  double cost, cost_change, gradient_max_norm, step_norm, relative_decrease, trust_region_radius;
};
struct LmHostMsg { long long word; long long pad; };
struct LmCtl {
  double* xp[2];
  double* nep[2];
  double* segp[2];
  double radius, decrease_factor, cost, gmax;
  double ftol, ptol, gtol, min_radius, max_radius, min_rel_dec;
  int32_t reuse_diagonal, done, iter, invalid, num_successful, num_unsuccessful, max_iters, max_invalid;
  int32_t hold;
  int32_t trace_cap, trace_n, pad;
  long long seq;
  LmIterRec* trace;
  long long* stamps;
  LmHostMsg* host;
};
enum { LM_RUNNING = 0, LM_DONE_PARAMETER_TOL = 1, LM_DONE_FUNCTION_TOL = 2, LM_DONE_GRADIENT_TOL = 3, LM_DONE_MIN_RADIUS = 4,
       LM_DONE_MAX_ITERATIONS = 5, LM_DONE_INVALID_STEPS = 6 };

struct SolveBuffers {
  double* Mb;
  double* Mt;
  double* Mc;
  double* scale;
  double* diag;
  double* D2;
  double* step_s;
  LmState* st;
  long long* prof;
  double* ws;
  int64_t ws_doubles;
  int force_p;
  int algo;
  double radius;
  int bcr_max_border = 64;
  int bcr_delay = 0;
  int bcr_join = 0, bcr_join_budget = 0; int64_t* bcr_joined = nullptr;
  const LmCtl* ctl = nullptr;
  const LmCtl* ctl_prev = nullptr; const LmState* st_prev = nullptr; int64_t off_cost = 0;
};

enum { kRmSo3 = 0, kRmEucl = 1, kRmAb = 2, kRmGb = 3, kRmPt = 4, kRmTic = 5 };
constexpr int64_t kRmapMaxParams = int64_t(1) << 28;
__host__ __device__ inline int32_t lm_rmap_code(int kind, int64_t param_off) { return int32_t((param_off << 3) | kind); }

struct RetractReq {
  int on;
  const double* x; double* xc;
  const int32_t* rmap;
  NormalEq ne;
  double max_ab, max_gb, alpha;
};

struct BcrDist {
  int nranks = 1, rank = 0;
  int b0 = 0, n_loc = 0;
  int max_loc = 0;
  const int32_t* d_b0 = nullptr;
  double* ws = nullptr; int64_t ws_doubles = 0;
  double* msg = nullptr; int64_t msg_piece = 0;
  double* xg = nullptr; int64_t x_piece = 0;
};

}
```

openimucameracalibrator_amd/csrc/oicc_exchange.hip:

```cpp
#include "oicc_problem.h"

namespace oicc {


struct RcclApi {
  ncclResult_t (*GetUniqueId)(ncclUniqueId*) = nullptr;
  ncclResult_t (*CommInitRank)(ncclComm_t*, int, ncclUniqueId, int) = nullptr;
  ncclResult_t (*AllReduce)(const void*, void*, size_t, ncclDataType_t, ncclRedOp_t, ncclComm_t, hipStream_t) = nullptr;
  ncclResult_t (*CommDestroy)(ncclComm_t) = nullptr;
  ncclResult_t (*Broadcast)(const void*, void*, size_t, ncclDataType_t, int, ncclComm_t, hipStream_t) = nullptr;
  ncclResult_t (*Send)(const void*, size_t, ncclDataType_t, int, ncclComm_t, hipStream_t) = nullptr;
  ncclResult_t (*Recv)(void*, size_t, ncclDataType_t, int, ncclComm_t, hipStream_t) = nullptr;
  ncclResult_t (*GroupStart)() = nullptr;
  ncclResult_t (*GroupEnd)() = nullptr;
  ncclResult_t (*AllGather)(const void*, void*, size_t, ncclDataType_t, ncclComm_t, hipStream_t) = nullptr;
  bool ok = false, p2p = false;
};
RcclApi& rccl_api() {
  static RcclApi api;
  static bool tried = false;
  if (tried) return api;
  tried = true;
  void* handles[4] = {RTLD_DEFAULT, dlopen("librccl.so.1", RTLD_NOW | RTLD_NOLOAD), dlopen("librccl.so", RTLD_NOW | RTLD_NOLOAD), nullptr};
  for (int k = 0; k < 5 && !api.ok; ++k) {
// ... 249 lines not shown
    BcrDist& d = ds[size_t(k)];
    d.nranks = nranks; d.rank = k; d.b0 = b0[size_t(k)]; d.n_loc = b0[size_t(k) + 1] - d.b0; d.max_loc = max_loc; d.d_b0 = d_b0.p;
    d.ws_doubles = bcr_dist_workspace_doubles(tl, d.n_loc, nranks);
    if (!ws[size_t(k)].resize(size_t(d.ws_doubles))) { p->err = "hipMalloc distributed solve"; return OICC_ERR_HIP; }
    d.ws = ws[size_t(k)].p; d.msg = msg.p; d.msg_piece = msg_piece; d.xg = xg.p; d.x_piece = x_piece;
  }
  EventPair ev;
  if (ms) { HIPCK(p, hipEventCreate(&ev.a)); HIPCK(p, hipEventCreate(&ev.b)); }
  const double min_diag = p->opt["min_lm_diagonal"], max_diag = p->opt["max_lm_diagonal"];
  const int runs = ms ? reps + 1 : 1;
  for (int phase = 0; phase < 2; ++phase)
    for (int k = 0; k < nranks; ++k) {
      for (int it = 0; it < runs; ++it) {
        if (ms && it == 1) HIPCK(p, hipEventRecord(ev.a, st));
        const int r2 = phase == 0 ? launch_bcr_dist_forward(p->ne, tl, sb, reuse_diagonal, min_diag, max_diag, ds[size_t(k)], st) : launch_bcr_dist_middle(tl, sb, ds[size_t(k)], st);
        if (r2 != 0) { p->err = "distributed solve: geometry / workspace"; return OICC_ERR_STATE; }
      }
      if (!ms) continue;
      HIPCK(p, hipEventRecord(ev.b, st)); HIPCK(p, hipEventSynchronize(ev.b));
      float t = 0; (void)hipEventElapsedTime(&t, ev.a, ev.b);
      ms[2 * k + phase] = double(t) / reps;
    }
  launch_bcr_dist_finish(tl, sb, ds[0], st);
  HIPCK(p, hipStreamSynchronize(st));
  return OICC_OK;
}
}
extern "C" {

int oicc_rccl_get_unique_id(uint8_t id[128]) {
  static_assert(sizeof(ncclUniqueId) == 128, "ncclUniqueId is 128 bytes");
  if (!id) return OICC_ERR_INVALID_ARG;
  RcclApi& api = rccl_api();
  if (!api.ok) return OICC_ERR_UNSUPPORTED;
  ncclUniqueId u;
  if (api.GetUniqueId(&u) != ncclSuccess) return OICC_ERR_HIP;
  std::memcpy(id, &u, 128);
  return OICC_OK;
}

int oicc_rccl_init(oicc_problem* p, int32_t nranks, int32_t rank, const uint8_t id[128]) {
  ARG(p, id != nullptr && nranks >= 1 && rank >= 0 && rank < nranks, "bad RCCL rank / size");
  RcclApi& api = rccl_api();
  if (!api.ok) { p->err = "RCCL (librccl.so.1) not found in this process"; return OICC_ERR_UNSUPPORTED; }
  (void)hipSetDevice(p->device);
  if (p->rccl_comm) { (void)api.CommDestroy(static_cast<ncclComm_t>(p->rccl_comm)); p->rccl_comm = nullptr; }
  ncclUniqueId u; std::memcpy(&u, id, 128);
  ncclComm_t comm = nullptr;
  if (api.CommInitRank(&comm, nranks, u, rank) != ncclSuccess) { p->err = "ncclCommInitRank failed"; return OICC_ERR_HIP; }
  p->rccl_comm = comm; p->rccl_nranks = nranks;
  p->reduce = rccl_reduce_in_place; p->reduce_user = p;
  return OICC_OK;
}

int oicc_set_shard(oicc_problem* p, int32_t nranks, int32_t rank) {
  ARG(p, nranks >= 1 && rank >= 0 && rank < nranks, "shard rank");
  p->shard_n = nranks; p->shard_rank = rank; p->layout_flags = -1;
  return OICC_OK;
}

int oicc_set_exchange(oicc_problem* p, oicc_exchange_fn fn, void* user) { p->exchange = fn; p->exchange_user = user; return OICC_OK; }
int oicc_debug_dist_solve_emulated(oicc_problem* p, int32_t flags, int32_t nranks, double radius, int32_t repeats, double* out) {
  int rc = prepare(p, flags); if (rc) return rc;
  ARG(p, out != nullptr && dist_emulated_applies(p, nranks), "distributed solve: ranks / geometry");
  SolveBuffers sb = solve_buffers(p); sb.radius = radius;
  rc = system_at_current_point(p, local_pass(p->d_x.p, true), sb.scale, p->opt["jacobi_scaling"] != 0, 0.0); if (rc) return rc;
  rc = dist_solve_emulated(p, sb, nranks, 0, std::max<int>(repeats, 1), out + 2); if (rc) return rc;
  return read_solve_residual(p, sb, &out[0], nullptr, &out[1]);
}
int oicc_debug_lm_step(oicc_problem* p, int32_t flags, double radius, int32_t reuse_diagonal, int32_t nranks, int64_t geom[8], double* band,
                       double* Et, double* C, double* g, double* scale, double* diag, double* D2, double* step_s, int32_t* chol_failed) {
  int rc = prepare(p, flags); if (rc) return rc;
  const bool solve = band != nullptr;
  ARG(p, geom != nullptr && (!solve || (Et != nullptr && C != nullptr && g != nullptr && scale != nullptr && diag != nullptr && D2 != nullptr &&
      step_s != nullptr && chol_failed != nullptr)) && radius > 0.0 && (nranks == 0 || nranks >= 2), "debug_lm_step: arguments");
  const TangentLayout& tl = p->tl;
  ARG(p, tl.P > 0, "debug_lm_step: no parameters");
  ARG(p, nranks == 0 || dist_emulated_applies(p, nranks), "debug_lm_step: distributed ranks / geometry");
  SolveBuffers sb = solve_buffers(p); sb.radius = radius;
  const LmRoute route = nranks == 0 ? lm_solve_route(tl, sb) : LmRoute{kRouteDistributed, 1};
  const int64_t P = tl.P, Pb = tl.Pb, a = tl.a;
  geom[0] = Pb; geom[1] = tl.hb; geom[2] = a; geom[3] = (Pb + 63) / 64; geom[4] = route.route; geom[5] = route.p; geom[6] = tl.W; geom[7] = P;
  if (!solve) return OICC_OK;
  ARG(p, route.route != kRouteNone, "debug_lm_step: solver geometry unsupported");
  hipStream_t st = p->stream;
  rc = system_at_current_point(p, local_pass(p->d_x.p, true), sb.scale, p->opt["jacobi_scaling"] != 0, 0.0); if (rc) return rc;
  if (p->opt["debug_poison_lds"] != 0.0) launch_lds_poison(st);
  const double min_diag = p->opt["min_lm_diagonal"], max_diag = p->opt["max_lm_diagonal"];
  if (nranks == 0) {
    if (launch_lm_solve(p->ne, tl, sb, radius, reuse_diagonal ? 1 : 0, min_diag, max_diag, st) != 0) { p->err = "solver geometry unsupported"; return OICC_ERR_UNSUPPORTED; }
  } else {
    rc = dist_solve_emulated(p, sb, nranks, reuse_diagonal ? 1 : 0, 0, nullptr); if (rc) return rc;
  }
  HIPCK(p, hipGetLastError());
  auto d2h = [&](double* dst, const double* src, int64_t count) { return count <= 0 ? hipSuccess : hipMemcpyAsync(dst, src, size_t(count) * sizeof(double), hipMemcpyDeviceToHost, st); };
  HIPCK(p, d2h(band, p->ne.band(), Pb * tl.W)); HIPCK(p, d2h(Et, p->ne.Et(), a * Pb)); HIPCK(p, d2h(C, p->ne.C(), a * a)); HIPCK(p, d2h(g, p->ne.g(), P));
  HIPCK(p, d2h(scale, sb.scale, P)); HIPCK(p, d2h(diag, sb.diag, P)); HIPCK(p, d2h(D2, sb.D2, P)); HIPCK(p, d2h(step_s, sb.step_s, P));
  LmState hs;
  HIPCK(p, hipMemcpyAsync(&hs, p->d_state.p, sizeof(hs), hipMemcpyDeviceToHost, st));
  HIPCK(p, hipStreamSynchronize(st));
  *chol_failed = hs.chol_failed;
  return OICC_OK;
}
int oicc_debug_lm_retract(oicc_problem* p, int32_t flags, double radius, int64_t info[4], double* x, double* xc_loop, double s_loop[3],
                          double* xc_alone, double s_alone[3], double* step_s, double* scale, double* D2, double* g) {
  int rc = prepare(p, flags); if (rc) return rc;
  const bool run = x != nullptr;
  ARG(p, info != nullptr && radius > 0.0 && (!run || (xc_loop && s_loop && xc_alone && s_alone && step_s && scale && D2 && g)), "debug_lm_retract: arguments");
  const TangentLayout& tl = p->tl;
  ARG(p, tl.P > 0, "debug_lm_retract: no parameters");
  const int64_t P = tl.P, N = p->pl.total;
  info[0] = 0; info[1] = P; info[2] = N; info[3] = (tl.Pb + 63) / 64;
  if (!run) return OICC_OK;
  hipStream_t st = p->stream;
  SolveBuffers sb = solve_buffers(p);
  rc = system_at_current_point(p, local_pass(p->d_x.p, true), sb.scale, p->opt["jacobi_scaling"] != 0, 0.0); if (rc) return rc;
  auto d2h = [&](double* dst, const double* src, int64_t count) { return count <= 0 ? hipSuccess : hipMemcpyAsync(dst, src, size_t(count) * sizeof(double), hipMemcpyDeviceToHost, st); };
  LmState hs;
  HIPCK(p, hipMemsetAsync(p->d_xc.p, 0xff, size_t(N) * sizeof(double), st));
  bool fused = false;
  rc = lm_solve_and_retract(p, sb, radius, 0, p->opt["min_lm_diagonal"], p->opt["max_lm_diagonal"], st, &fused, true); if (rc) return rc;
  HIPCK(p, hipGetLastError());
  HIPCK(p, d2h(xc_loop, p->d_xc.p, N));
  HIPCK(p, hipMemcpyAsync(&hs, p->d_state.p, sizeof(hs), hipMemcpyDeviceToHost, st));
  HIPCK(p, hipStreamSynchronize(st));
  s_loop[0] = hs.model_cost_change; s_loop[1] = hs.step_norm_sq; s_loop[2] = hs.x_norm_sq;
  const bool failed = hs.chol_failed != 0;
  HIPCK(p, hipMemsetAsync(p->d_xc.p, 0xff, size_t(N) * sizeof(double), st));
  HIPCK(p, hipMemsetAsync(&p->d_state.p->model_cost_change, 0, 3 * sizeof(double), st));
  launch_lm_retract(p->d_x.p, p->d_xc.p, p->pl, tl, sb, p->ne, p->max_ab, p->max_gb, st, 1.0, 1, nullptr);
  HIPCK(p, hipGetLastError());
  HIPCK(p, d2h(xc_alone, p->d_xc.p, N)); HIPCK(p, d2h(x, p->d_x.p, N));
  HIPCK(p, d2h(step_s, sb.step_s, P)); HIPCK(p, d2h(scale, sb.scale, P)); HIPCK(p, d2h(D2, sb.D2, P)); HIPCK(p, d2h(g, p->ne.g(), P));
  HIPCK(p, hipMemcpyAsync(&hs, p->d_state.p, sizeof(hs), hipMemcpyDeviceToHost, st));
  HIPCK(p, hipMemcpyAsync(p->d_xc.p, p->d_x.p, size_t(N) * sizeof(double), hipMemcpyDeviceToDevice, st));
  HIPCK(p, hipStreamSynchronize(st));
  p->seg_invalidate(p->d_xc.p);
  s_alone[0] = hs.model_cost_change; s_alone[1] = hs.step_norm_sq; s_alone[2] = hs.x_norm_sq;
  info[0] = fused ? 1 : 0;
  if (failed) { p->err = "debug_lm_retract: the factorisation failed"; return OICC_ERR_STATE; }
  return OICC_OK;
}
int oicc_debug_dist_solve_info(const oicc_problem* p, int64_t out4[4]) {
  if (!p || !out4) return OICC_ERR_INVALID_ARG;
  out4[0] = p->dist.solves; out4[1] = p->dist.d.b0; out4[2] = p->dist.d.n_loc; out4[3] = dist_solve_usable(p) ? p->dist.d.nranks : 0;
  return OICC_OK;
}
int oicc_debug_bcr_join_info(oicc_problem* p, int64_t out4[4]) {
  if (!p || !out4) return OICC_ERR_INVALID_ARG;
  const SolveBuffers sb = solve_buffers(p);
  out4[0] = p->bcr_joined[0]; out4[1] = p->bcr_joined[1]; out4[2] = sb.bcr_join_budget; out4[3] = sb.bcr_join;
  return OICC_OK;
}

int oicc_time_allreduce(oicc_problem* p, int32_t flags, int32_t repeats, double* ms_per_call, int64_t* bytes) {
  int rc = prepare(p, flags); if (rc) return rc;
  if (!p->reduce) { p->err = "no reduction path installed (oicc_rccl_init / oicc_set_allreduce)"; return OICC_ERR_STATE; }
  hipStream_t st = p->stream;
  HIPCK(p, hipMemsetAsync(p->d_ne2.p, 0, p->ne.total * sizeof(double), st));
  EventPair ev; HIPCK(p, hipEventCreate(&ev.a)); HIPCK(p, hipEventCreate(&ev.b)); hipEvent_t e0 = ev.a, e1 = ev.b;
  if (p->reduce(p->reduce_user, p->d_ne2.p, p->ne.total, st) != 0) { p->err = "allreduce callback failed"; return OICC_ERR_STATE; }
  HIPCK(p, hipEventRecord(e0, st));
  for (int i = 0; i < repeats; ++i) if (p->reduce(p->reduce_user, p->d_ne2.p, p->ne.total, st) != 0) { p->err = "allreduce callback failed"; return OICC_ERR_STATE; }
  HIPCK(p, hipEventRecord(e1, st)); HIPCK(p, hipEventSynchronize(e1));
  float ms = 0; (void)hipEventElapsedTime(&ms, e0, e1);
  if (ms_per_call) *ms_per_call = double(ms) / std::max(repeats, 1);
  if (bytes) *bytes = int64_t(p->ne.total) * int64_t(sizeof(double));
  return OICC_OK;
}

int oicc_time_exchange(oicc_problem* p, int32_t flags, int32_t repeats, double* ms_per_call, int64_t* bytes_moved) {
  int rc = prepare(p, flags); if (rc) return rc;
  if (!owner_exchange_ready(p)) { p->err = "owner-computes exchange not set up (oicc_set_shard, remote measurements with their owners, a transport)"; return OICC_ERR_STATE; }
  if (repeats < 0) return OICC_OK;
  hipStream_t st = p->stream;
  bool use = false;
  rc = owner_exchange_agree(p, st, &use); if (rc) return rc;
  if (!use) { p->err = "owner-computes exchange not agreed on by all ranks"; return OICC_ERR_STATE; }
  HIPCK(p, hipMemsetAsync(p->d_ne2.p, 0, p->ne.total * sizeof(double), st));
  EventPair ev; HIPCK(p, hipEventCreate(&ev.a)); HIPCK(p, hipEventCreate(&ev.b)); hipEvent_t e0 = ev.a, e1 = ev.b;
  int64_t moved = 0;
  rc = owner_exchange(p, p->ne2, st, false, &moved); if (rc) return rc;
  HIPCK(p, hipEventRecord(e0, st));
  for (int i = 0; i < repeats; ++i) { rc = owner_exchange(p, p->ne2, st, false, &moved); if (rc) return rc; }
  HIPCK(p, hipEventRecord(e1, st)); HIPCK(p, hipEventSynchronize(e1));
  float ms = 0; (void)hipEventElapsedTime(&ms, e0, e1);
  if (ms_per_call) *ms_per_call = double(ms) / std::max(repeats, 1);
  if (bytes_moved) *bytes_moved = moved;
  return OICC_OK;
}

}
```

openimucameracalibrator_amd/csrc/oicc_problem.h:

```cpp
#pragma once
#include <hip/hip_runtime.h>
#include <rccl/rccl.h>
#include <dlfcn.h>

#include <algorithm>
#include <chrono>
#include <cmath>
#include <cstdio>
#include <cstring>
#include <map>
#include <thread>
#include <memory>
#include <type_traits>
#include <string>
#include <vector>

#include "../../include/oicc_hip.h"
#include "oicc_device.h"
#include "lm_launch.h"
#include "tiles.h"
#include "inner_plan.h"
#include "line_search.h"
#include "covariance.h"


namespace oicc {
void launch_trajectory(const EvalCtx& ctx, int64_t n, const int32_t* s_so3, const int32_t* s_r3, const double* u_so3,
                       const double* u_r3, const int32_t* s_gb, const double* u_gb, const int32_t* s_ab, const double* u_ab,
                       double inv_gb_dt, double inv_ab_dt, double* pose7, double* gyro3, double* accel3, double* gb3, double* ab3,
                       hipStream_t st);
int launch_tile_pass(const TileStatic& hS, const TileStatic* dS, const TileDyn& dyn, bool jac, hipStream_t st);
void launch_lds_poison(hipStream_t st);
void launch_point_columns(const EvalCtx& ctx, const ViewData& vd, const uint8_t* view_rs, bool spline_active, hipStream_t st);
void launch_inner_seg(const double* so3, int n_pairs, double* seg, hipStream_t st);
void launch_inner_set(const InnerArgs* dA, double* xv, const InnerWg* wgs, long long* prof, int n_wgs, int mode, hipStream_t st, bool read_out = false);
void launch_inner_wave(const InnerArgs* dA, double* xv, int b0, int n_blocks, bool r3_only, hipStream_t st, bool read_out = false);
void launch_inner_shared_eval(const InnerArgs* dA, double* xv, const InnerWg* wgs, int n_wgs, double* partials, int max_parts, hipStream_t st);
void launch_inner_shared_advance(const InnerArgs* dA, double* xv, const int32_t* block_ids, const int32_t* block_parts, int n_blocks, const double* partials, int max_parts, void* states, bool count_iterations, hipStream_t st, bool read_out = false);
size_t inner_lm_state_bytes();
void launch_inner_records(const ViewData& vd, const ImuData& ia, const ImuData& ig, InnerItemRec* rc, InnerItemRec* ra, InnerItemRec* rg, hipStream_t st);
int inner_set_resident_capacity(int n_cu);
void launch_rank_pack(const double* x, int64_t n, const LmState* s, double* pack, hipStream_t st);
void launch_rank_unpack(double* x, int64_t n, LmState* s, const double* pack, hipStream_t st);
void launch_ne_pack_rows(const NormalEq& ne, const TangentLayout& tl, const int32_t* rows, int n_rows, double* buf, hipStream_t st);
void launch_ne_add_rows(const NormalEq& ne, const TangentLayout& tl, const int32_t* rows, int n_rows, const double* buf, hipStream_t st);
void launch_ne_pack_range(const NormalEq& ne, const TangentLayout& tl, int row0, int n_rows, double* buf, hipStream_t st);
void launch_ne_pack_diag_g(const NormalEq& ne, const TangentLayout& tl, int row0, int n_rows, double* buf, hipStream_t st);
void launch_ne_unpack_diag_g(const NormalEq& ne, const TangentLayout& tl, const int32_t* cut, int n, int me, int64_t piece, const double* buf, hipStream_t st);
void launch_ne_unpack_ranges(const NormalEq& ne, const TangentLayout& tl, const int32_t* cut, int n, int me, int64_t piece, const double* buf, hipStream_t st);
void launch_inner_diff_norm(const double* x, const double* xc, const InnerBlock* blocks, int nb, double* step_norm_sq, hipStream_t st);
void launch_lm_retract(const double* x, double* xc, const ParamLayout& pl, const TangentLayout& tl, const SolveBuffers& sb,
                       const NormalEq& ne, double max_ab, double max_gb, hipStream_t st, double alpha = 1.0, int with_model = 1, double* seg_out = nullptr);
void launch_lm_step_slope(const double* g, const SolveBuffers& sb, int P, double* out, hipStream_t st);
void launch_lm_projected_gradient(const double* x, const ParamLayout& pl, const TangentLayout& tl, const NormalEq& ne, double max_ab, double max_gb, LmState* s, hipStream_t st);
void launch_report_views(const EvalCtx& ctx, const ViewData& vd, const uint8_t* gate, double* e_uv, uint8_t* status, int32_t* n_used,
                         double* sum_sq, double* max_e, hipStream_t st);
void launch_report_imu(const EvalCtx& ctx, const ImuData& id, int kind, double* r3, double* partials, hipStream_t st);
void launch_lm_decide(LmCtl* out, const LmCtl* prev, const LmState* st, int64_t off_cost, hipStream_t stream);
}


namespace oicc {


constexpr int kN = OICC_SPLINE_N;
constexpr int kNb = OICC_BIAS_SPLINE_N;

struct ImuHost {
  std::vector<int32_t> s_so3, s_r3, s_b;
  std::vector<double> u_so3, u_r3, u_b, mx, my, mz, w;
  size_t size() const { return s_so3.size(); }
};
struct ImuDev { DevBuf<int32_t> s_so3, s_r3, s_b; DevBuf<double> u_so3, u_r3, u_b, mx, my, mz, w; };
struct ImuGroups { std::vector<int32_t> first, count; size_t size() const { return first.size(); } };

struct Active { bool tic, ld, g, spline, ab, gb, intr_a, intr_g, pts; };

struct HostLayout {
  std::vector<int32_t> so3, r3, ab, gb;
  int32_t other[5];
  int32_t P, Pb, a, hb;
  std::vector<int32_t> rmap;
  std::vector<int32_t> pts; int32_t a_pts = 0;
};

}

using namespace oicc;

struct InnerPlanOptions { int flags; bool gs_unit; bool general_kernel; int resident_wgs; double shared_share; int64_t layout_gen; int wave_blocks = 0; int n_cu = 256; int big_slots = 65536; };

struct oicc_problem {
  int device = 0;
  hipStream_t stream = nullptr;
  bool own_stream = false;
  std::string err;
  int64_t dt_so3 = 0, dt_r3 = 0, start_ns = 0, end_ns = 0;
  double inv_so3_dt = 0, inv_r3_dt = 0;
  int64_t dt_ab = 0, dt_gb = 0; double inv_ab_dt = 0, inv_gb_dt = 0, max_ab = 1.0, max_gb = 1e-2;
  ParamLayout pl{};
  std::vector<double> x;
  bool x_host_dirty = true;
  bool x_host_dirty_pts = false;
  std::vector<char> so3_in, r3_in, ab_in, gb_in;
  int cam_model = 0, n_intr = 0; double intr[10] = {0};
  std::vector<double> pts;
  int32_t max_corner_pt = -1;
  std::vector<int32_t> corner_view, corner_pt; std::vector<double> cu, cv, cisx, cisy;
  std::vector<double> cisx0, cisy0; std::vector<uint8_t> cgate;
  std::vector<int64_t> view_c0{0}; std::vector<int32_t> view_s_so3, view_s_r3; std::vector<double> view_u_so3, view_u_r3;
  std::vector<uint8_t> view_rs;
  ImuHost acc, gyr;
  ImuGroups acc_groups, gyr_groups;
  bool views_unsorted = false, acc_unsorted = false, gyr_unsorted = false;
  std::vector<int64_t> corner_orig; std::vector<int32_t> acc_orig, gyr_orig;
  std::vector<int32_t> view_orig;
  std::vector<int32_t> remote_so3, remote_r3;
  std::vector<int32_t> remote_owner;
  int shard_n = 1, shard_rank = 0;
  oicc_exchange_fn exchange = nullptr; void* exchange_user = nullptr;
  struct OwnerPlan { bool valid = false; std::vector<int32_t> cut; std::vector<std::vector<int32_t>> send_rows, recv_rows; std::vector<int32_t> flat, send_off, recv_off; int max_rows = 0;
                     int max_owned = 0;
                     int64_t agreed_gen = -1; bool agreed = false;
                     uint32_t hash = 0; } owner;
  DevBuf<int32_t> d_xrows, d_xcut; DevBuf<double> d_xsend, d_xrecv, d_xgather, d_xagree;
  struct DistSolve { bool usable = false; int64_t gen = -1; BcrDist d; std::vector<int32_t> b0; DevBuf<int32_t> d_b0; DevBuf<double> ws, msg, xg; int64_t solves = 0;
                     bool last_step_gathered = false;
                   } dist;
  bool has_ld_block = false, has_tic_block = false, has_acc = false, has_gyr = false;
  std::vector<uint8_t> pts_seen_global; int64_t pts_seen_meas_gen = -1, meas_gen = 0;
  bool has_remote_views = false;
  bool meas_dirty = true, groups_dirty = true;
  std::thread plan_thread; InnerPlanOptions plan_job{}; bool plan_job_valid = false; double plan_ms[3] = {0, 0, 0};
  void wait_plan() { if (plan_thread.joinable()) plan_thread.join(); }
  int plan_wanted_flags = -2;
  std::map<std::string, double> opt;
  std::vector<oicc_iteration> trace;
  std::vector<double> inner_set_costs; DevBuf<double> d_dbg_cost;
  oicc_allreduce_fn reduce = nullptr; void* reduce_user = nullptr;
  void* rccl_comm = nullptr;
  int rccl_nranks = 1;
  oicc_problem* inner_src = nullptr;
  DevBuf<double> d_x, d_xc;
  struct SegTable { DevBuf<double> buf; const double* of = nullptr; bool valid = false; } seg_tab[2];
  SegTable* seg_of(const double* xbuf) { for (auto& t : seg_tab) if (t.of == xbuf) return &t; return nullptr; }
  void seg_invalidate(const double* xbuf) { if (SegTable* t = seg_of(xbuf)) t->valid = false; }
  int n_cu = 256;
  int64_t bcr_joined[2] = {0, 0};
  bool seg_precomputed() const { const auto it = opt.find("debug_seg_precompute"); const int force = it == opt.end() ? 0 : int(it->second); return force == 1 || (force == 0 && tp.n_tiles > n_cu); }
  DevBuf<int32_t> d_corner_view, d_corner_pt, d_view_s_so3, d_view_s_r3;
  DevBuf<double> d_cu, d_cv, d_cisx, d_cisy, d_view_u_so3, d_view_u_r3;
  DevBuf<int64_t> d_view_c0; DevBuf<uint8_t> d_view_rs, d_view_rs_all, d_cgate; std::vector<uint8_t> h_view_rs_all;
  DevArena meas_arena, layout_arena, tile_arena, plan_arena;
  ImuDev d_acc, d_gyr;
  DevBuf<int32_t> d_tl_so3, d_tl_r3, d_tl_ab, d_tl_gb, d_tl_pts, d_tl_rmap;
  DevBuf<double> d_ws;
  DevBuf<double> d_rank_pack;
  DevBuf<double> d_ne2;
  DevBuf<double> d_ne, d_Mb, d_Mt, d_Mc, d_scale, d_diag, d_D2, d_step, d_dbg_res, d_dbg_jac, d_traj;
  DevBuf<int32_t> d_traj_i;
  DevBuf<LmState> d_state; DevBuf<double> d_ls; int64_t line_search_steps = 0;
  DevBuf<LmCtl> d_ctl; DevBuf<LmIterRec> d_trace; DevBuf<long long> d_stamps; LmHostMsg* hmsg = nullptr; LmHostMsg* hmsg_dev = nullptr; double wall_clock_hz = 1e8;
  struct HostPin { LmState st; double cost; double radius; double ls[2]; unsigned int inner_words[32]; };
  HostPin* pin = nullptr;
  hipEvent_t ev[8] = {nullptr, nullptr, nullptr, nullptr, nullptr, nullptr, nullptr, nullptr};
  std::vector<TileDesc> h_tiles; std::vector<UnitDesc> h_units; std::vector<int32_t> h_tile_rows, h_merge_rows; std::vector<uint8_t> h_row_direct;
  DevBuf<int32_t> d_merge_rows, d_merge_ptr; DevBuf<int64_t> d_merge_src, d_merge_tab; DevBuf<uint8_t> d_row_direct; std::vector<int32_t> h_merge_ptr; std::vector<int64_t> h_merge_src, h_merge_tab;
  DevBuf<TileDesc> d_tiles; DevBuf<UnitDesc> d_units; DevBuf<int32_t> d_tile_rows; DevBuf<double> d_slabs;
  RowFmt fv{}, fa{}, fg{}; TileParams tp{}; int tile_T = 0;
  std::unique_ptr<TileStatic> h_tstatic; DevBuf<TileStatic> d_tstatic; bool tstatic_valid = false;
  struct InnerPlan {
    std::vector<InnerBlock> blocks; std::vector<int32_t> group_first; std::vector<InnerRun> runs; std::vector<InnerWg> wgs; std::vector<int32_t> group_wg0; std::vector<char> group_r3only;
    DevBuf<InnerBlock> d_blocks; DevBuf<InnerRun> d_runs; DevBuf<InnerWg> d_wgs; DevBuf<InnerCtl> d_ctls; DevBuf<unsigned long long> d_lm_iterations; DevBuf<double> d_seg; int n_ctls = 0;
    std::vector<InnerWg> big_wgs; std::vector<int32_t> group_bigwg0, big_blocks, big_parts, group_bigb0; int big_max_parts = 1;
    DevBuf<InnerWg> d_big_wgs; DevBuf<int32_t> d_big_blocks, d_big_parts; DevBuf<double> d_partials; DevBuf<unsigned char> d_lm_states;
    std::vector<char> group_wave;
    bool has_points = false;
    DevBuf<InnerItemRec> d_rec[3];
    DevBuf<InnerArgs> d_args; std::unique_ptr<InnerArgs> h_args; bool args_valid = false;
    struct RankPart { std::vector<InnerWg> wgs; std::vector<int32_t> group_wg0; std::vector<uint8_t> group_kinds; std::vector<int32_t> so3_lo, so3_hi, r3_lo, r3_hi;
                      DevBuf<InnerWg> d_wgs; uint64_t key = 0; bool valid = false; } rank_part;
    int flags = -2; int64_t layout_gen = -1; bool gs_unit = false;
    size_t n_items = 0; int64_t lm_iterations = 0; int sweeps = 0;
  } inner;
  int layout_flags = -1; bool layout_ld_zero = false; int64_t opt_gen = 0, layout_opt_gen = -1, layout_gen = 0;
  struct Cov { bool valid = false; int flags = 0; int P = 0, Pb = 0, a = 0; oicc_covariance_info info{};
               std::vector<int32_t> so3, r3;
               std::vector<double> arrow, cov3, cross;
               DevBuf<double> d_s, d_Cs, d_Sc, d_Zaa, d_aa, d_zb, d_G, d_cov3, d_cross, d_zs; DevBuf<int32_t> d_flags;
               double ms[4] = {0, 0, 0, 0};
             } cov;
  struct Report { bool valid = false;
                  std::vector<double> e_uv, view_sum, view_max; std::vector<uint8_t> status; std::vector<int32_t> view_n;
                  size_t n_acc = 0, n_gyr = 0;
                  DevBuf<double> d_e, d_vsum, d_vmax, d_acc_r, d_gyr_r, d_part; DevBuf<uint8_t> d_status; DevBuf<int32_t> d_vn;
                } report;
  void invalidate_estimates() { cov.valid = false; report.valid = false; }
  HostLayout L; TangentLayout tl{}; TangentLayout tl_tiles{}; NormalEq ne{}; NormalEq ne2{};
  Active act{};

  oicc_problem() {
    opt["function_tolerance"] = 1e-4; opt["parameter_tolerance"] = 1e-7; opt["gradient_tolerance"] = 1e-10;
    opt["initial_trust_region_radius"] = 1e4; opt["max_trust_region_radius"] = 1e16;
    opt["min_trust_region_radius"] = 1e-32; opt["min_relative_decrease"] = 1e-3;
    opt["min_lm_diagonal"] = 1e-6; opt["max_lm_diagonal"] = 1e32; opt["jacobi_scaling"] = 1;
    opt["max_num_consecutive_invalid_steps"] = 5; opt["gs_unit_loss"] = 0; opt["rs_time_in_seconds"] = 0;
    opt["verbose"] = 0; opt["num_threads"] = 0; opt["solver_partitions"] = 0; opt["solver_algorithm"] = 0; opt["imu_chunk_cells"] = 0;
    opt["inner_iterations"] = 0;
    opt["inner_iteration_tolerance"] = 1e-3;
    opt["setup_threads"] = 1;
    opt["distributed_solve"] = 1;
    opt["owner_computes_sweeps"] = 1;
    opt["inner_shared_launch_slots"] = 65536;
    opt["inner_wave_blocks"] = 0;
    opt["fused_retract"] = 1;
    opt["device_lm"] = 1;
    opt["inner_shared_residency"] = 0.5;
    opt["debug_inner_general_kernel"] = 0;
    opt["debug_inner_set_costs"] = 0;
    opt["debug_inner_profile"] = 0;
    opt["projected_gradient_norm"] = 0;
    opt["bounds_line_search"] = 0;
    opt["assembly"] = 0;
    opt["tile_windows"] = 0;
    opt["chain_tiles"] = 0;
    opt["accumulation"] = 0;
    opt["view_unit_items"] = 0; opt["accel_unit_items"] = 0; opt["gyro_unit_items"] = 0;
    opt["wide_cells"] = 1;
    opt["debug_unit_order"] = 0;
    opt["debug_no_direct_rows"] = 0;
    opt["debug_seg_precompute"] = 0;
    opt["debug_bcr_delay"] = 0;
    opt["bcr_max_border"] = 64;
    opt["bcr_join_levels"] = 1;
    opt["bcr_join_max_workgroups"] = 0;
    opt["debug_check_ne"] = 0;
    opt["debug_sync"] = 0;
    opt["covariance_min_rcond"] = 1e-12;
    opt["debug_poison_lds"] = 0;
  }
};

#define HIPCK(p, call)                                                                 \
  do {                                                                                 \
    hipError_t e_ = (call);                                                            \
    if (e_ != hipSuccess) {                                                            \
      (p)->err = std::string(#call) + ": " + hipGetErrorString(e_);                    \
      return OICC_ERR_HIP;                                                             \
    }                                                                                  \
  } while (0)
#define ARG(p, c, msg) do { if (!(c)) { (p)->err = msg; return OICC_ERR_INVALID_ARG; } } while (0)


namespace oicc {
double now_s();
bool calc_times(int64_t sensor_time, int64_t start_ns, int64_t dt_ns, size_t nr_knots, int N, double* u, int64_t* s);
double* xs(oicc_problem* p, int64_t off);
void rebuild_param_layout(oicc_problem* p, int64_t n_so3, int64_t n_r3, int64_t n_ab, int64_t n_gb);
int sync_params_to_device(oicc_problem* p);
int sync_params_to_host(oicc_problem* p);
void build_imu_groups(const ImuHost& h, bool accel, ImuGroups& g);
int sync_measurements(oicc_problem* p);
void sync_groups(oicc_problem* p);
Active active_set(const oicc_problem* p, int flags);
void build_owner_plan(oicc_problem* p);
void make_layout_host(oicc_problem* p, int flags);
void layout_scalars(oicc_problem* p);
int make_layout_device(oicc_problem* p, int flags, std::thread* tiles_thread = nullptr, int* tiles_rc = nullptr);
int build_tiles_host(oicc_problem* p);
int build_tiles_device(oicc_problem* p);
int prepare(oicc_problem* p, int flags);
EvalCtx make_ctx(oicc_problem* p, const double* x);
ViewData view_data(oicc_problem* p, bool force_rs = false);
ImuData imu_data(const ImuHost& h, const ImuDev& d);
void build_inner_plan_host(oicc_problem* p, const InnerPlanOptions& o, double t_ms[3]);
InnerPlanOptions inner_plan_options(oicc_problem* p, int flags, int64_t layout_gen);
void start_inner_plan(oicc_problem* p, int flags, int64_t layout_gen);
int build_inner_plan(oicc_problem* p, int flags);
struct InnerFirstEval { double* rows; double* seg; InnerCtl* ctls; InnerArgs* d_args; };
int inner_sweep(oicc_problem* p, double* xv, hipStream_t st, oicc_problem* shard = nullptr, bool* owner_computes = nullptr, const InnerFirstEval* fe = nullptr);
struct PassRequest {
  const double* x = nullptr;
  bool jac = false;
  const NormalEq* target = nullptr;
  double* cost_out = nullptr;
  bool cost_already_zero = false;
  const LmCtl* ctl = nullptr;
  double* dbg_res = nullptr; double* dbg_jac = nullptr;
  int only_kind = -1;
  bool force_rs = false;
  long long* prof = nullptr;
  LmState* gmax_into = nullptr;
  bool* gmax_folded = nullptr;
  bool local = false;
  bool full_system = false;
};
inline PassRequest jacobian_pass(const double* x, const NormalEq* target = nullptr) { PassRequest rq; rq.x = x; rq.jac = true; rq.target = target; return rq; }
inline PassRequest cost_pass(const double* x, double* cost_out = nullptr) { PassRequest rq; rq.x = x; rq.cost_out = cost_out; rq.cost_already_zero = cost_out != nullptr; return rq; }
inline PassRequest local_pass(const double* x, bool jac, int only_kind = -1) { PassRequest rq; rq.x = x; rq.jac = jac; rq.only_kind = only_kind; rq.local = true; return rq; }
int eval_pass(oicc_problem* p, const PassRequest& rq);
struct EventPair { hipEvent_t a = nullptr, b = nullptr; ~EventPair() { if (a) (void)hipEventDestroy(a); if (b) (void)hipEventDestroy(b); } };
SolveBuffers solve_buffers(oicc_problem* p, long long* prof = nullptr);
RetractReq retract_request(oicc_problem* p);
int lm_solve_and_retract(oicc_problem* p, const SolveBuffers& sb, double radius, int reuse_diagonal, double min_diag, double max_diag, hipStream_t st, bool* fused_out = nullptr, bool local = false);
int system_at_current_point(oicc_problem* p, const PassRequest& rq, double* scale, bool jacobi_scaling, double radius);
int read_solve_residual(oicc_problem* p, const SolveBuffers& sb, double* relative, double* rhs_norm, double* chol_failed);
int read_cost(oicc_problem* p, double* cost);
void rccl_release(oicc_problem* p);
int rccl_reduce_in_place(void* user, void* device_ptr, int64_t count, void* stream);
int rccl_broadcast_from_root(oicc_problem* p, void* device_ptr, int64_t count_doubles, hipStream_t stream);
int make_rank_consistent(oicc_problem* p, double* xv, bool with_state, hipStream_t st, bool x_identical = false);
bool owner_exchange_ready(const oicc_problem* p);
int owner_exchange_agree(oicc_problem* p, hipStream_t st, bool* use);
int shard_broadcast_begin(oicc_problem* p);
int shard_broadcast(oicc_problem* p, double* ptr, int64_t count, int root, hipStream_t st);
int shard_broadcast_end(oicc_problem* p);
int owner_exchange(oicc_problem* p, const NormalEq& ne, hipStream_t st, bool full_system, int64_t* bytes_moved = nullptr);
bool dist_solve_usable(const oicc_problem* p);
int dist_solve(oicc_problem* p, const NormalEq& ne, const SolveBuffers& sb, double radius, int reuse_diagonal, double min_diag, double max_diag, hipStream_t st);
int lm_solve_any(oicc_problem* p, const NormalEq& ne, const SolveBuffers& sb, double radius, int reuse_diagonal, double min_diag, double max_diag, hipStream_t st, const RetractReq* retract = nullptr, bool* fused = nullptr, bool local = false);
}
```

openimucameracalibrator_amd/csrc/oicc_problem.hip:

```cpp
#include "oicc_problem.h"

namespace oicc {

int eval_pass(oicc_problem* p, const PassRequest& rq) {
  const double* const x = rq.x; const bool jac = rq.jac; const int only_kind = rq.only_kind;
  const oicc_allreduce_fn reduce = rq.local ? nullptr : p->reduce;
  hipStream_t st = p->stream;
  const NormalEq ne = rq.target ? *rq.target : p->ne;
  if (p->opt["debug_poison_lds"] != 0.0) launch_lds_poison(st);
  {
    const bool with_points = jac && p->tl.a_pts > 0 && (only_kind < 0 || only_kind == 0);
    if (jac && (p->tp.direct || p->tp.n_tiles == 0)) HIPCK(p, hipMemsetAsync(ne.base, 0, ne.total * sizeof(double), st));
    else if (jac && p->tl.a_pts > 0) {
      const int a_np = p->tl.a - p->tl.a_pts;
      HIPCK(p, hipMemsetAsync(ne.base + ne.off_E + int64_t(a_np) * p->tl.Pb, 0, size_t(ne.off_g - ne.off_E - int64_t(a_np) * p->tl.Pb) * sizeof(double), st));
      HIPCK(p, hipMemsetAsync(ne.g() + p->tl.Pb + a_np, 0, size_t(p->tl.a_pts) * sizeof(double), st));
    }
    else if (!jac && !rq.cost_already_zero) HIPCK(p, hipMemsetAsync(ne.cost(), 0, sizeof(double), st));
    const TileParams& tp = p->tp;
    const bool gmax_folded = jac && rq.gmax_into != nullptr && !tp.direct && tp.n_tiles > 0 && !reduce && p->tl.a_pts == 0;
    if (rq.gmax_folded) *rq.gmax_folded = gmax_folded;
    if (!p->h_tstatic) { p->h_tstatic.reset(new TileStatic); std::memset(p->h_tstatic.get(), 0, sizeof(TileStatic)); p->tstatic_valid = false; }
    {
      static_assert(std::is_trivially_copyable<TileStatic>::value, "TileStatic is copied bytewise");
      TileStatic S; std::memset(&S, 0, sizeof(S));
      S.ctx = make_ctx(p, nullptr); S.ctx.ne = p->ne; S.ctx.ne.base = nullptr; S.ctx.pts = nullptr; S.ctx.tl = p->tl_tiles;
      S.vd = view_data(p, false); S.vd.view_rs = nullptr;
      S.ia = imu_data(p->acc, p->d_acc); S.ig = imu_data(p->gyr, p->d_gyr);
      S.fmt[0] = p->fv; S.fmt[1] = p->fa; S.fmt[2] = p->fg; S.tp = tp; S.tp.gmax = nullptr;
      if (!p->tstatic_valid || std::memcmp(&S, p->h_tstatic.get(), sizeof(S)) != 0) {
        if (!p->d_tstatic.resize(1)) { p->err = "hipMalloc tile arguments"; return OICC_ERR_HIP; }
        *p->h_tstatic = S;
        HIPCK(p, hipMemcpyAsync(p->d_tstatic.p, p->h_tstatic.get(), sizeof(TileStatic), hipMemcpyHostToDevice, st));
        HIPCK(p, hipStreamSynchronize(st));
        p->tstatic_valid = true;
      }
    }
    TileDyn dyn{};
    dyn.ctl = rq.ctl;
    if (rq.ctl != nullptr) { if (p->seg_precomputed()) dyn.seg = p->seg_tab[0].buf.p; }
    else if (p->seg_precomputed()) {
      oicc_problem::SegTable* sgt = p->seg_of(x);
      if (sgt == nullptr) { p->err = "residual pass on an unknown parameter buffer"; return OICC_ERR_STATE; }
      if (!sgt->valid) { launch_inner_seg(x + p->pl.so3, int(p->pl.n_so3 - 1), sgt->buf.p, st); sgt->valid = true; }
      dyn.seg = sgt->buf.p;
    }
    dyn.x = x; dyn.ne_base = ne.base; dyn.cost_out = (!jac && rq.cost_out) ? rq.cost_out : ne.cost(); dyn.dbg_res = rq.dbg_res; dyn.dbg_jac = rq.dbg_jac; dyn.prof = rq.prof; dyn.only_kind = only_kind;
    dyn.gmax = gmax_folded ? &rq.gmax_into->gradient_max_norm : nullptr;
    dyn.view_rs = rq.force_rs ? p->d_view_rs_all.p : p->d_view_rs.p;
    if (launch_tile_pass(*p->h_tstatic, p->d_tstatic.p, dyn, jac, st) != 0) {
      p->err = "tile kernel launch failed"; return OICC_ERR_HIP; }
    if (with_points) {
      EvalCtx c = make_ctx(p, x); c.ne = ne;
      launch_point_columns(c, view_data(p, false), dyn.view_rs, p->act.spline, st);
    }
  }
  HIPCK(p, hipGetLastError());
  if (p->opt["debug_sync"] != 0.0) HIPCK(p, hipStreamSynchronize(st));
  if (reduce) {
    double* cdst = (!jac && rq.cost_out) ? rq.cost_out : ne.cost();
    int rc;
    if (jac && p->shard_n > 1) {
      bool use = false; rc = owner_exchange_agree(p, st, &use); if (rc) return rc;
      if (use) return owner_exchange(p, ne, st, rq.full_system);
    }
    rc = jac ? reduce(p->reduce_user, ne.base, ne.total, st) : reduce(p->reduce_user, cdst, 1, st);
    if (rc != 0) { p->err = "allreduce callback failed"; return OICC_ERR_STATE; }
  }
  return OICC_OK;
}

SolveBuffers solve_buffers(oicc_problem* p, long long* prof) {
  SolveBuffers sb{p->d_Mb.p, p->d_Mt.p, p->d_Mc.p, p->d_scale.p, p->d_diag.p, p->d_D2.p, p->d_step.p, p->d_state.p, prof, p->d_ws.p, (int64_t)p->d_ws.n, int(p->opt["solver_partitions"]), int(p->opt["solver_algorithm"])};
  sb.radius = 0.0; sb.bcr_max_border = int(p->opt["bcr_max_border"]); sb.bcr_delay = int(p->opt["debug_bcr_delay"]);
  const int join_max = int(p->opt["bcr_join_max_workgroups"]);
  sb.bcr_join = p->opt["bcr_join_levels"] != 0.0 ? 1 : 0; sb.bcr_join_budget = join_max > 0 ? join_max : p->n_cu; sb.bcr_joined = p->bcr_joined;
  return sb;
}

int read_cost(oicc_problem* p, double* cost) {
  HIPCK(p, hipMemcpyAsync(cost, p->ne.cost(), sizeof(double), hipMemcpyDeviceToHost, p->stream));
  HIPCK(p, hipStreamSynchronize(p->stream));
  return OICC_OK;
}


RetractReq retract_request(oicc_problem* p) {
  RetractReq R{};
  R.on = (p->opt["fused_retract"] != 0.0 && !p->seg_precomputed() && p->d_tl_rmap.p != nullptr && p->pl.total < kRmapMaxParams) ? 1 : 0;
  R.x = p->d_x.p; R.xc = p->d_xc.p; R.rmap = p->d_tl_rmap.p; R.ne = p->ne;
  R.max_ab = p->max_ab; R.max_gb = p->max_gb; R.alpha = 1.0;
  return R;
}
int lm_solve_and_retract(oicc_problem* p, const SolveBuffers& sb, double radius, int reuse_diagonal, double min_diag, double max_diag, hipStream_t st, bool* fused_out, bool local) {
  const RetractReq R = retract_request(p);
  bool fused = false;
  const int rc = lm_solve_any(p, p->ne, sb, radius, reuse_diagonal, min_diag, max_diag, st, &R, &fused, local); if (rc) return rc;
  if (fused_out) *fused_out = fused;
  oicc_problem::SegTable* sgt = p->seg_of(p->d_xc.p);
  if (!fused) launch_lm_retract(p->d_x.p, p->d_xc.p, p->pl, p->tl, sb, p->ne, p->max_ab, p->max_gb, st, 1.0, 1, (sgt && p->seg_precomputed()) ? sgt->buf.p : nullptr);
  if (sgt) sgt->valid = !fused && p->seg_precomputed();
  return OICC_OK;
}

static_assert(sizeof(LmIterRec) == sizeof(oicc_iteration) && offsetof(LmIterRec, trust_region_radius) == offsetof(oicc_iteration, trust_region_radius), "LmIterRec mirrors oicc_iteration");

bool device_lm_applicable(oicc_problem* p, bool inner, bool line_search, bool projected_gmax) {
  if (p->opt["device_lm"] == 0.0 || p->hmsg == nullptr || inner || line_search || projected_gmax || p->reduce != nullptr) return false;
  if (p->tp.direct || p->tp.n_tiles == 0 || p->tl.a_pts != 0 || p->tl.P == 0) return false;
  for (const char* name : {"debug_sync", "debug_check_ne", "debug_poison_lds"}) if (p->opt[name] != 0.0) return false;
  return true;
}
int device_lm_begin(oicc_problem* p, LmCtl h, int trace_cap) {
  hipStream_t st = p->stream;
  if (!p->d_ctl.resize(2) || !p->d_trace.resize(size_t(std::max(trace_cap, 1))) || !p->d_stamps.resize(size_t(3) * std::max(trace_cap, 1))) { p->err = "hipMalloc LM control"; return OICC_ERR_HIP; }
  h.xp[0] = p->d_x.p; h.xp[1] = p->d_xc.p; h.nep[0] = p->ne.base; h.nep[1] = p->ne2.base;
  oicc_problem::SegTable* s0 = p->seg_of(p->d_x.p); oicc_problem::SegTable* s1 = p->seg_of(p->d_xc.p);
  h.segp[0] = s0 ? s0->buf.p : nullptr; h.segp[1] = s1 ? s1->buf.p : nullptr;
  h.done = 0; h.iter = 0; h.invalid = 0; h.num_successful = 0; h.num_unsuccessful = 0; h.seq = 0; h.trace_n = 0; h.trace_cap = trace_cap;
  h.trace = p->d_trace.p; h.stamps = p->d_stamps.p; h.host = p->hmsg_dev;
  __atomic_store_n(&p->hmsg->word, 0ll, __ATOMIC_RELEASE);
  HIPCK(p, hipMemcpyAsync(p->d_ctl.p, &h, sizeof(LmCtl), hipMemcpyHostToDevice, st));
  HIPCK(p, hipMemsetAsync(p->d_state.p, 0, 2 * sizeof(LmState), st));
  HIPCK(p, hipStreamSynchronize(st));
  return OICC_OK;
}
int device_lm_enqueue(oicc_problem* p, SolveBuffers sb, double min_diag, double max_diag, int k) {
  hipStream_t st = p->stream;
  LmCtl* const cur = p->d_ctl.p + (k & 1); LmState* const stc = p->d_state.p + (k & 1);
  sb.ctl = cur; sb.st = stc; sb.off_cost = p->ne.off_cost;
  sb.ctl_prev = k > 0 ? p->d_ctl.p + ((k - 1) & 1) : nullptr; sb.st_prev = k > 0 ? p->d_state.p + ((k - 1) & 1) : nullptr;
  const RetractReq R = retract_request(p);
  bool fused = false;
  if (launch_lm_solve(p->ne, p->tl, sb, 0.0, 0, min_diag, max_diag, st, &R, &fused) != 0) {
    p->err = "band/arrow geometry exceeds the single-workgroup solver (half bandwidth or arrow too large for 160 KB LDS)"; return OICC_ERR_UNSUPPORTED; }
  if (!fused) launch_lm_retract(p->d_x.p, p->d_xc.p, p->pl, p->tl, sb, p->ne, p->max_ab, p->max_gb, st, 1.0, 1, p->seg_precomputed() ? p->seg_tab[0].buf.p : nullptr);
  PassRequest rq = jacobian_pass(p->d_xc.p, &p->ne2); rq.ctl = cur; rq.gmax_into = stc;
  const int rc = eval_pass(p, rq); if (rc) return rc;
  HIPCK(p, hipGetLastError());
  return OICC_OK;
}
int device_lm_settle(oicc_problem* p, int k_last) {
  launch_lm_decide(p->d_ctl.p + ((k_last + 1) & 1), p->d_ctl.p + (k_last & 1), p->d_state.p + (k_last & 1), p->ne.off_cost, p->stream);
  HIPCK(p, hipGetLastError());
  return OICC_OK;
}
int device_lm_wait(oicc_problem* p, long long want, int* done) {
  unsigned spins = 0;
  auto look = [&](long long* seq) { const long long w = __atomic_load_n(&p->hmsg->word, __ATOMIC_ACQUIRE); *seq = w & 0xffffffffll; return int(w >> 32); };
  while (true) {
    long long s; const int d = look(&s);
    if (d != 0 || s >= want) { *done = d; return OICC_OK; }
    if ((++spins & 0xfff) == 0) {
      const hipError_t e = hipStreamQuery(p->stream);
      if (e == hipSuccess) {
        *done = look(&s);
        if (*done != 0 || s >= want) return OICC_OK;
        p->err = "device-side LM control: the stream drained without the awaited decision"; return OICC_ERR_STATE;
      }
      if (e != hipErrorNotReady) { p->err = std::string("device-side LM control: ") + hipGetErrorString(e); return OICC_ERR_HIP; }
    }
#if defined(__x86_64__)
    __builtin_ia32_pause();
#endif
  }
}
int device_lm_end(oicc_problem* p, int k_last, LmCtl* out, std::vector<LmIterRec>* trace, std::vector<long long>* stamps) {
  hipStream_t st = p->stream;
  HIPCK(p, hipMemcpyAsync(out, p->d_ctl.p + ((k_last + 1) & 1), sizeof(LmCtl), hipMemcpyDeviceToHost, st));
  HIPCK(p, hipStreamSynchronize(st));
  const int n = std::min(out->trace_n, out->trace_cap);
  if (trace) { trace->resize(size_t(n)); if (n > 0) HIPCK(p, hipMemcpyAsync(trace->data(), p->d_trace.p, size_t(n) * sizeof(LmIterRec), hipMemcpyDeviceToHost, st)); }
  const long long ns = std::min<long long>(out->seq, out->trace_cap);
  if (stamps) { stamps->resize(size_t(3 * ns)); if (ns > 0) HIPCK(p, hipMemcpyAsync(stamps->data(), p->d_stamps.p, size_t(3 * ns) * sizeof(long long), hipMemcpyDeviceToHost, st)); }
  HIPCK(p, hipStreamSynchronize(st));
  if (out->xp[0] != p->d_x.p) { std::swap(p->d_x.p, p->d_xc.p); std::swap(p->ne.base, p->ne2.base); }
  p->seg_invalidate(p->d_x.p); p->seg_invalidate(p->d_xc.p);
  return OICC_OK;
}
LmCtl device_lm_control(oicc_problem* p, double radius, double cost, double gmax, int max_iters, int hold) {
  LmCtl h; std::memset(&h, 0, sizeof(h));
  h.radius = radius; h.decrease_factor = 2.0; h.cost = cost; h.gmax = gmax;
  h.ftol = p->opt["function_tolerance"]; h.ptol = p->opt["parameter_tolerance"]; h.gtol = p->opt["gradient_tolerance"];
  h.min_radius = p->opt["min_trust_region_radius"]; h.max_radius = p->opt["max_trust_region_radius"]; h.min_rel_dec = p->opt["min_relative_decrease"];
  h.reuse_diagonal = 0; h.max_iters = max_iters; h.max_invalid = int(p->opt["max_num_consecutive_invalid_steps"]); h.hold = hold;
  return h;
}
int device_lm_run(oicc_problem* p, const SolveBuffers& sb, LmCtl* h, std::vector<LmIterRec>* recs, std::vector<long long>* stamps) {
  const int max_iters = h->max_iters; const double min_diag = p->opt["min_lm_diagonal"], max_diag = p->opt["max_lm_diagonal"];
  int rc = device_lm_begin(p, *h, max_iters); if (rc) return rc;
  int done = 0, k_last = -1;
  for (int k = 0; k < max_iters && done == 0; ++k) {
    rc = device_lm_enqueue(p, sb, min_diag, max_diag, k); if (rc) return rc;
    k_last = k;
    if (k >= 2) { rc = device_lm_wait(p, k - 1, &done); if (rc) return rc; }
  }
  rc = device_lm_settle(p, k_last); if (rc) return rc;
  return device_lm_end(p, k_last, h, recs, stamps);
}

int system_at_current_point(oicc_problem* p, const PassRequest& rq, double* scale, bool jacobi_scaling, double radius) {
  hipStream_t st = p->stream;
  const int rc = eval_pass(p, rq); if (rc) return rc;
  launch_lm_scale(p->ne, p->tl, scale, jacobi_scaling ? 1 : 0, st);
  if (radius == 0.0) { HIPCK(p, hipMemsetAsync(p->d_state.p, 0, sizeof(LmState), st)); return OICC_OK; }
  LmState hs; std::memset(&hs, 0, sizeof(hs)); hs.radius = radius;
  HIPCK(p, hipMemcpyAsync(p->d_state.p, &hs, sizeof(hs), hipMemcpyHostToDevice, st));
  return OICC_OK;
}
int read_solve_residual(oicc_problem* p, const SolveBuffers& sb, double* relative, double* rhs_norm, double* chol_failed) {
  hipStream_t st = p->stream;
  DevBuf<double> acc; if (!acc.resize(2 + size_t(p->tl.a))) return OICC_ERR_HIP;
  launch_lm_solve_residual(p->ne, p->tl, sb, acc.p, st);
  double h[2] = {0, 0}; LmState hs;
  HIPCK(p, hipMemcpyAsync(h, acc.p, sizeof(h), hipMemcpyDeviceToHost, st));
  HIPCK(p, hipMemcpyAsync(&hs, p->d_state.p, sizeof(hs), hipMemcpyDeviceToHost, st));
  HIPCK(p, hipStreamSynchronize(st));
  *relative = h[1] > 0.0 ? std::sqrt(h[0] / h[1]) : std::sqrt(h[0]); if (rhs_norm) *rhs_norm = std::sqrt(h[1]); *chol_failed = double(hs.chol_failed);
  return OICC_OK;
}

}

extern "C" {

const char* oicc_version(void) { return "oicc-hip-gfx950-r1"; }

int oicc_create(oicc_problem** out, int device_ordinal) {
  if (!out) return OICC_ERR_INVALID_ARG;
// ... 811 lines not shown
```

openimucameracalibrator_amd/estimator.py:

```python
import ctypes as C
from dataclasses import dataclass
import numpy as np

from . import _abi

POINTS = 1 << 0
T_I_C = 1 << 1
IMU_BIASES = 1 << 2
IMU_INTRINSICS = 1 << 3
GRAVITY_DIR = 1 << 4
CAM_LINE_DELAY = 1 << 5
SPLINE = 1 << 6
ACC_BIAS = 1 << 7
GYR_BIAS = 1 << 8

S_TO_NS = 1e9
NS_TO_S = 1e-9
SPLINE_N = 6
BIAS_SPLINE_N = 3


def _dp(a):
    return a.ctypes.data_as(_abi.c_dp)

# ... 168 lines not shown
        acc = np.zeros(len(t_ns), dtype=np.uint8)
        self._ck(fn(self._h, len(t_ns), t_ns.ctypes.data_as(_abi.c_i64p), _dp(m), float(weight),
                    acc.ctypes.data_as(_abi.c_u8p)))
        return acc.astype(bool)

    def AddAccelerometerMeasurements(self, meas, t_ns, weight_se3):
        return self._add_imu(self._b.add_accelerometer_measurements, meas, t_ns, weight_se3)

    def AddGyroscopeMeasurements(self, meas, t_ns, weight_so3):
        return self._add_imu(self._b.add_gyroscope_measurements, meas, t_ns, weight_so3)

    def AddAccelerometerMeasurement(self, meas, time_ns, weight_se3):
        return bool(self.AddAccelerometerMeasurements([meas], [time_ns], weight_se3)[0])

    def AddGyroscopeMeasurement(self, meas, time_ns, weight_so3):
        return bool(self.AddGyroscopeMeasurements([meas], [time_ns], weight_so3)[0])

    def Optimize(self, max_iters, flags):
        s = _abi.Summary()
        self._ck(self._b.optimize(self._h, int(max_iters), int(flags), C.byref(s)))
        if int(flags) & POINTS and getattr(self, "_points", None) is not None:
            self._points = self.GetScenePoints()
        return s.as_dict()

    def GetIterations(self, capacity=256):
        arr = (_abi.Iteration * capacity)()
        n = self._b.get_iterations(self._h, arr, capacity)
        return [arr[i].as_dict() for i in range(n)]

    def GetInnerSetCosts(self):
        n = self._b.get_inner_set_costs(self._h, None, 0)
        buf = np.zeros(max(n, 1))
        self._b.get_inner_set_costs(self._h, buf.ctypes.data_as(_abi.c_dp), n)
        sweeps = []
        for k in range(0, n, 2):
            if buf[k] < 0:
                sweeps.append([])
            sweeps[-1].append((int(buf[k]), float(buf[k + 1])))
        return sweeps

    def SetAllReduce(self, fn):
        if fn is None:
            self._ck(self._b.set_allreduce(self._h, C.cast(None, _abi.ALLREDUCE_FN), None))
            return

        def tramp(user, ptr, count, stream):
            try:
                fn(int(ptr or 0), int(count), int(stream or 0))
                return 0
            except Exception as e:
                print("allreduce callback failed:", e)
                return -1
        cb = _abi.ALLREDUCE_FN(tramp)
        self._keep.append(cb)
        self._ck(self._b.set_allreduce(self._h, cb, None))

    def RcclUniqueId(self):
        buf = (C.c_uint8 * 128)()
        rc = self._b.rccl_get_unique_id(buf)
        if rc != 0:
            raise RuntimeError("oicc_rccl_get_unique_id failed with status %d (RCCL not found in this process?)" % rc)
        return bytes(buf)

    def EnableRccl(self, nranks, rank, unique_id):
        buf = (C.c_uint8 * 128).from_buffer_copy(bytes(unique_id))
        self._ck(self._b.rccl_init(self._h, int(nranks), int(rank), buf))

    def GetTangentLayout(self, flags):
        n_so3, n_r3 = self.GetNumSO3Knots(), self.GetNumR3Knots()
        na, ng = self._b.get_num_accl_bias_knots(self._h), self._b.get_num_gyro_bias_knots(self._h)
        nt = C.c_int32(0)
        so3 = np.zeros(n_so3, np.int32); r3 = np.zeros(n_r3, np.int32)
        ab = np.zeros(max(na, 1), np.int32); gb = np.zeros(max(ng, 1), np.int32); other = np.zeros(5, np.int32)
        p = lambda a: a.ctypes.data_as(_abi.c_i32p)
        self._ck(self._b.get_tangent_layout(self._h, int(flags), C.byref(nt), p(so3), p(r3), p(ab), p(gb), p(other)))
        return dict(P=nt.value, so3=so3, r3=r3, accl_bias=ab[:na], gyro_bias=gb[:ng], other=other)

    def Evaluate(self, flags, want_H=True):
        P = self.GetTangentLayout(flags)["P"]
        cost = C.c_double(0)
        H = np.zeros((P, P)) if want_H else None
        g = np.zeros(P)
        self._ck(self._b.evaluate(self._h, int(flags), C.byref(cost), _dp(H) if want_H else None, _dp(g), P))
        return cost.value, H, g

    def EvaluateEntries(self, flags, rows, cols):
        rows = np.ascontiguousarray(rows, dtype=np.int32); cols = np.ascontiguousarray(cols, dtype=np.int32)
        out = np.zeros(len(rows))
        self._ck(self._b.evaluate_entries(self._h, int(flags), len(rows), rows.ctypes.data_as(_abi.c_i32p), cols.ctypes.data_as(_abi.c_i32p), _dp(out)))
        return out

    def EvaluateCost(self, flags):
        cost = C.c_double(0)
        self._ck(self._b.evaluate_cost(self._h, int(flags), C.byref(cost)))
        return cost.value

    def EvaluateBlocks(self, flags, kind, n_rows, want_jac=True):
        ncols = {0: 43, 1: 54, 2: 36}[kind]
        r = np.zeros(n_rows)
        J = np.zeros((n_rows, ncols)) if want_jac else None
        self._ck(self._b.evaluate_blocks(self._h, int(flags), int(kind), _dp(r), _dp(J) if want_jac else None))
        return r, J

    def TimeJacobianPass(self, flags, repeats=10, families=True):
        ms = C.c_double(0); k = np.zeros(3)
        self._ck(self._b.time_jacobian_pass(self._h, int(flags), int(repeats), C.byref(ms), _dp(k) if families else None))
        return ms.value, k

    def RunLmIterations(self, flags, steps):
        self._ck(self._b.run_lm_iterations(self._h, int(flags), int(steps)))

    def DeclareRemoteMeasurements(self, kind, t_ns, owner=None):
        t_ns = np.ascontiguousarray(t_ns, dtype=np.int64)
        if owner is None:
            self._ck(self._b.declare_remote_measurements(self._h, int(kind), len(t_ns), t_ns.ctypes.data_as(_abi.c_i64p)))
        else:
            self._ck(self._b.declare_remote_measurements_from(self._h, int(owner), int(kind), len(t_ns), t_ns.ctypes.data_as(_abi.c_i64p)))

    def SetShard(self, nranks, rank):
        self._ck(self._b.set_shard(self._h, int(nranks), int(rank)))

    def SetExchange(self, fn):
        def tramp(user, op, sp, sc, rp, rc_, peer, stream):
            try:
                fn(int(op), int(sp or 0), int(sc), int(rp or 0), int(rc_), int(peer), int(stream or 0))
                return 0
            except Exception as e:
                print("exchange callback failed:", e)
                return -1
        cb = _abi.EXCHANGE_FN(tramp)
        self._keep.append(cb)
        self._ck(self._b.set_exchange(self._h, cb, None))

    def DistributedSolveInfo(self):
        fn = self._b.lib.oicc_debug_dist_solve_info
        fn.restype = C.c_int; fn.argtypes = [C.c_void_p, C.POINTER(C.c_int64)]
        out = (C.c_int64 * 4)()
        self._ck(fn(self._h, out))
        return dict(solves=int(out[0]), first_block=int(out[1]), blocks=int(out[2]), ranks=int(out[3]))

    def DistributedSolveEmulated(self, flags, nranks, radius=1e4, repeats=3):
        fn = self._b.lib.oicc_debug_dist_solve_emulated
        fn.restype = C.c_int; fn.argtypes = [C.c_void_p, C.c_int32, C.c_int32, C.c_double, C.c_int32, _abi.c_dp]
        out = np.zeros(2 + 2 * nranks)
        self._ck(fn(self._h, flags, nranks, float(radius), repeats, _dp(out)))
        return float(out[0]), bool(out[1]), out[2::2].copy(), out[3::2].copy()

    def BcrJoinInfo(self):
        fn = self._b.lib.oicc_debug_bcr_join_info
        fn.restype = C.c_int; fn.argtypes = [C.c_void_p, C.POINTER(C.c_int64)]
        out = (C.c_int64 * 4)()
        self._ck(fn(self._h, out))
        return dict(last=int(out[0]), total=int(out[1]), budget=int(out[2]), on=bool(out[3]))

    ROUTES = ("bcr_fused", "bcr_unfused", "sweep64", "sweep128", "partitioned", "global", "distributed")

    def DebugLmStep(self, flags, radius=1e4, reuse_diagonal=0, nranks=0, solve=True):
        fn = self._b.lib.oicc_debug_lm_step
        fn.restype = C.c_int
        fn.argtypes = [C.c_void_p, C.c_int32, C.c_double, C.c_int32, C.c_int32, C.POINTER(C.c_int64)] + [_abi.c_dp] * 8 + [C.POINTER(C.c_int32)]
        geom = (C.c_int64 * 8)()
        args = (self._h, int(flags), float(radius), int(reuse_diagonal), int(nranks), geom)
        self._ck(fn(*args, *([None] * 8), None))
        if solve:
            Pb, a, W, P = int(geom[0]), int(geom[2]), int(geom[6]), int(geom[7])
            arr = dict(band=np.zeros((Pb, W)), Et=np.zeros((a, Pb)), C=np.zeros((a, a)), g=np.zeros(P), scale=np.zeros(P), diag=np.zeros(P),
                       D2=np.zeros(P), step_s=np.zeros(P))
            failed = C.c_int32(0)
            self._ck(fn(*args, *(_dp(arr[k]) for k in ("band", "Et", "C", "g", "scale", "diag", "D2", "step_s")), C.byref(failed)))
        out = dict(Pb=int(geom[0]), hb=int(geom[1]), a=int(geom[2]), n=int(geom[3]), route=self.ROUTES[int(geom[4])] if geom[4] >= 0 else None,
                   p=int(geom[5]), W=int(geom[6]), P=int(geom[7]))
        if solve:
            out.update(arr); out["chol_failed"] = bool(failed.value)
        return out

    def DebugLmRetract(self, flags, radius=1e4, run=True):
        from . import _lib
        fn = _lib.load_lm_retract().retract
        info = (C.c_int64 * 4)()
        self._ck(fn(self._h, int(flags), float(radius), info, *([None] * 9)))
        P, N = int(info[1]), int(info[2])
        out = dict(fused=False, P=P, N=N, n=int(info[3]))
        if run:
            arr = dict(x=np.zeros(N), xc_loop=np.zeros(N), s_loop=np.zeros(3), xc_alone=np.zeros(N), s_alone=np.zeros(3), step_s=np.zeros(P),
                       scale=np.zeros(P), D2=np.zeros(P), g=np.zeros(P))
            self._ck(fn(self._h, int(flags), float(radius), info,
                        *(_dp(arr[k]) for k in ("x", "xc_loop", "s_loop", "xc_alone", "s_alone", "step_s", "scale", "D2", "g"))))
            out.update(arr); out["fused"] = bool(info[0])
        return out

    def DebugInnerFirstEvaluations(self, flags):
        fn = _abi.bind_inner_debug(self._b.lib, "oicc_debug_inner_first_evaluations")
        cap = 1 << 12
        while True:
            info = np.zeros((cap, 8), np.int32); sums = np.zeros((cap, 56))
            n = fn(self._h, int(flags), info.ctypes.data_as(_abi.c_i32p), _dp(sums), cap)
            if n < -(1 << 30):
                self._ck(-(1 << 31) - n)
            if n >= 0:
                return info[:n].copy(), sums[:n].copy()
            cap = -n

    def TimeExchange(self, flags, repeats=10):
        ms = C.c_double(0.0); nb = C.c_int64(0)
        self._ck(self._b.time_exchange(self._h, int(flags), int(repeats), C.byref(ms), C.byref(nb)))
        return ms.value, nb.value

    def TimeLinearSolve(self, flags, repeats=10):
        ms = C.c_double(0)
        self._ck(self._b.time_linear_solve(self._h, int(flags), int(repeats), C.byref(ms)))
        return ms.value

    def SolveResidual(self, flags, radius=1e4):
        out = (C.c_double * 3)()
        self._ck(self._b.solve_residual(self._h, int(flags), float(radius), out))
        return out[0], out[1], bool(out[2])

    COV_OK, COV_RANK_DEFICIENT, COV_ZERO_COLUMN = 0, 1, 2
    COV_STATUS_NAMES = ("ok", "rank_deficient", "zero_column")

    def EstimateCovariance(self, flags):
        info = _abi.CovarianceInfo()
        self._ck(self._b.estimate_covariance(self._h, int(flags), C.byref(info)))
        out = dict(info=info.as_dict(), status_name=self.COV_STATUS_NAMES[info.status], layout=self.GetTangentLayout(flags),
                   message=self._b.last_error(self._h).decode() if info.status != self.COV_OK else "", arrow=None, so3=None, r3=None)
        self._last_cov_a = int(info.a)
        if info.status == self.COV_OK:
            arrow = np.zeros((info.a, info.a)); so3 = np.zeros((self.GetNumSO3Knots(), 3, 3)); r3 = np.zeros((self.GetNumR3Knots(), 3, 3))
            self._ck(self._b.get_covariance_arrow(self._h, _dp(arrow), info.a))
            self._ck(self._b.get_covariance_knots(self._h, _dp(so3), len(so3), _dp(r3), len(r3)))
            out.update(arrow=arrow, so3=so3, r3=r3)
        return out

    def GetCovarianceKnotArrow(self, kind, knot):
        a = int(getattr(self, "_last_cov_a", 0))
        out = np.zeros((3, max(a, 1)))
        rc = self._b.get_covariance_knot_arrow(self._h, int(kind), int(knot), _dp(out))
        if rc != 0:
            raise OiccError("no covariance estimate for the current parameters, or no such knot (status %d)" % rc)
        return out[:, :a]

    def CovarianceTiming(self):
        ms = np.zeros(4)
        self._ck(self._b.get_covariance_timing(self._h, _dp(ms)))
        return dict(build=ms[0], forward=ms[1], corner=ms[2], backward=ms[3])

    CORNER_USED, CORNER_PROJECTION_FAILED, CORNER_GATED = 0, 1, 2

    def ResidualReport(self):
        info = _abi.ResidualInfo()
        self._ck(self._b.residual_report(self._h, C.byref(info)))
        self._last_report = info.as_dict()
        return dict(self._last_report)

    def _report_sizes(self):
        r = getattr(self, "_last_report", None) or dict(num_corners=0, num_views=0, num_accl=0, num_gyro=0)
        return r

    def GetCornerErrors(self):
        n = int(self._report_sizes()["num_corners"])
        e = np.zeros((n, 2)); st = np.zeros(n, np.uint8)
        self._ck(self._b.get_corner_errors(self._h, _dp(e), st.ctypes.data_as(_abi.c_u8p), n))
        return e, st

    def GetViewErrors(self):
        nv = int(self._report_sizes()["num_views"])
        rms = np.zeros(nv); mx = np.zeros(nv); nu = np.zeros(nv, np.int32)
        self._ck(self._b.get_view_errors(self._h, _dp(rms), _dp(mx), nu.ctypes.data_as(_abi.c_i32p), nv))
        return dict(rms_px=rms, max_px=mx, n_used=nu)

    def GetImuResiduals(self, kind):
        n = int(self._report_sizes()["num_accl" if int(kind) == 1 else "num_gyro"])
        r = np.zeros((n, 3))
        self._ck(self._b.get_imu_residuals(self._h, int(kind), _dp(r), n))
        return r

    def GateCorners(self, threshold_px):
        n = C.c_int64(0)
        self._ck(self._b.gate_corners(self._h, float(threshold_px), C.byref(n)))
        return int(n.value)

    def GetCornerGate(self, num_corners):
        g = np.zeros(int(num_corners), np.uint8)
        self._ck(self._b.get_corner_gate(self._h, g.ctypes.data_as(_abi.c_u8p), len(g)))
        return g.astype(bool)

    def GetNumSO3Knots(self):
        return int(self._b.get_num_so3_knots(self._h))

    def GetNumR3Knots(self):
        return int(self._b.get_num_r3_knots(self._h))

    def GetMinTimeNs(self):
        return int(self._b.get_min_time_ns(self._h))

    def GetMaxTimeNs(self):
        return int(self._b.get_max_time_ns(self._h))

    def GetKnots(self):
        so3 = np.zeros((self.GetNumSO3Knots(), 4)); r3 = np.zeros((self.GetNumR3Knots(), 3))
        self._ck(self._b.get_so3_knots(self._h, _dp(so3), len(so3)))
        self._ck(self._b.get_r3_knots(self._h, _dp(r3), len(r3)))
        return so3, r3

    def GetBiasKnots(self):
        na, ng = self._b.get_num_accl_bias_knots(self._h), self._b.get_num_gyro_bias_knots(self._h)
# ... 314 lines not shown
```

Measured before the change: 52.66 million.

## Fold first back-substitution level into the last-block BCR invert kernel

When the BCR plan has an even number of levels and no ghost or offset, the last-block invert kernel is launched with one workgroup per pivot of the top back-substitution level. Idle waves prefetch the back-substitution rows during the corner solve, and each workgroup then computes its pivot's solution from the top-level values it holds locally. This removes one kernel launch and its global round trip per solve. In exchange the last-block inversion is computed redundantly in every workgroup, with only block 0 writing shared outputs, and more LDS is used. A default-on option and debug plan/info entry points are added.

```diff
diff --git a/include/oicc_hip.h b/include/oicc_hip.h
--- a/include/oicc_hip.h
+++ b/include/oicc_hip.h
@@ -365,6 +365,8 @@
 int oicc_debug_bcr_plan(int32_t n, int32_t ghost, int32_t odd_only, int64_t* levels, int32_t cap_levels, int64_t info[3]);
 int oicc_debug_bcr_join_plan(int32_t n, int32_t ghost, int32_t odd_only, int32_t b0, int32_t rtf, int32_t join_levels, int32_t budget,
                              int32_t build_inverts, int32_t* joined, int32_t cap_levels);
+int oicc_debug_bcr_fold_plan(int32_t n, int32_t ghost, int32_t odd_only, int32_t b0, int32_t on);
+int oicc_debug_bcr_fold_info(oicc_problem* problem, int64_t out3[3]);
 
 #ifdef __cplusplus
 }
diff --git a/openimucameracalibrator_amd/_abi.py b/openimucameracalibrator_amd/_abi.py
--- a/openimucameracalibrator_amd/_abi.py
+++ b/openimucameracalibrator_amd/_abi.py
@@ -327,6 +327,8 @@
 BCR_PLAN_SIGNATURES = {
     "plan": (C.c_int, [C.c_int32, C.c_int32, C.c_int32, c_i64p, C.c_int32, c_i64p]),
     "join_plan": (C.c_int, [C.c_int32] * 8 + [c_i32p, C.c_int32]),
+    "fold_plan": (C.c_int, [C.c_int32] * 5),
+    "fold_info": (C.c_int, [C.c_void_p, c_i64p]),
 }
 
 
diff --git a/openimucameracalibrator_amd/csrc/kernels_bcr.hip b/openimucameracalibrator_amd/csrc/kernels_bcr.hip
--- a/openimucameracalibrator_amd/csrc/kernels_bcr.hip
+++ b/openimucameracalibrator_amd/csrc/kernels_bcr.hip
@@ -45,8 +45,9 @@
   yt = t - (xt * (xt + 1)) / 2;
 }
 
-template <int LD>
-__device__ __forceinline__ void bcr_corner_solve(double* C, double* da, int* failp, int a, int tid, int wave, int lane) {
+struct BcrNoIdle { __device__ __forceinline__ void operator()() const {} };
+template <int LD, class Idle = BcrNoIdle>
+__device__ __forceinline__ void bcr_corner_solve(double* C, double* da, int* failp, int a, int tid, int wave, int lane, Idle idle = Idle()) {
   const int a1 = a + 1;
   if (a1 <= 16) {
     if (wave == 0) {
@@ -91,7 +92,7 @@
       }
       if (lane < a) da[lane] = xq_mine;
       if (bad && lane == 0) *failp = 1;
-    }
+    } else idle();
     __syncthreads();
     return;
   }
@@ -121,7 +122,7 @@
       z = fma(-l, xq, z);
     }
     if (lane < a) da[lane] = xq_mine;
-  }
+  } else idle();
   __syncthreads();
 }
 
@@ -148,12 +149,47 @@
   return g;
 }
 
-template <bool LAST, bool ZLDS>
-__device__ __forceinline__ void bcri_tail(const BcrArgs& A, double* W, double* da, int* failp, const double* Fs, double* Zg, int tid, int wave, int lane, bool report,
+constexpr int kBackRows = 192 / kBackWaves;
+struct BcrBackX {
+  const double* xl; const double* xr; const double* xa;
+  bool hasL, hasR;
+  __device__ __forceinline__ double at(int r, int a) const {
+    return r < 64 ? (hasL ? xl[r] : 0.0) : (r < 128 ? (hasR ? xr[r - 64] : 0.0) : (r < 128 + a ? xa[r - 128] : 0.0));
+  }
+};
+__device__ __forceinline__ void bcri_back_rows(const double* Tg, int a, bool hasL, bool hasR, int w, int lane, double (&lv)[kBackRows], double& yv) {
+#pragma unroll
+  for (int k = 0; k < kBackRows; ++k) {
+    const int r = w + kBackWaves * k;
+    const bool ok = r < 128 + a && (hasL || r >= 64) && (hasR || r < 64 || r >= 128);
+    lv[k] = ok ? Tg[r * 64 + lane] : 0.0;
+  }
+  yv = w == 0 ? Tg[(128 + a) * 64 + lane] : 0.0;
+}
+__device__ __forceinline__ double bcri_back_body(const double (&lv)[kBackRows], double yv, const BcrBackX& X, int a, double* part, bool active, int w, int lane) {
+  if (active) {
+    double sum = 0.0;
+#pragma unroll
+    for (int k = 0; k < kBackRows; ++k) { const int r = w + kBackWaves * k; sum = fma(lv[k], X.at(r, a), sum); }
+    part[w * 64 + lane] = sum;
+  }
+  __syncthreads();
+  double acc = 0.0;
+  if (active && w == 0) {
+#pragma unroll
+    for (int ww = 0; ww < kBackWaves; ++ww) acc += part[ww * 64 + lane];
+  }
+  return yv - acc;
+}
+
+template <bool LAST, bool ZLDS, bool FOLD>
+__device__ __forceinline__ void bcri_tail(const BcrArgs& A, double* W, double* da, int* failp, const double* Fs, const double* Cs, double* Zg, int tid, int wave, int lane, bool report,
                                           const double (&ttop)[16], const double ytop, double* x0s) {
+  static_assert(!FOLD || LAST, "the folded level follows the last block");
   constexpr int LD = kInvLD, NW = kInvWaves, NT = 64 * NW, FLD = 65;
   const int li = lane & 15, lq = lane >> 4;
   const int a = A.a, a1 = a + 1;
+  const bool shared_writer = !FOLD || blockIdx.x == 0;
   for (int t = wave; t < 10; t += NW) {
     int xt, yt; tri10(t, xt, yt);
     const bcr_v4d g = xt == 0 ? bcri_z_tile<0>(W, yt, li, lq) : (xt == 1 ? bcri_z_tile<1>(W, yt, li, lq) : (xt == 2 ? bcri_z_tile<2>(W, yt, li, lq) : bcri_z_tile<3>(W, yt, li, lq)));
@@ -197,16 +233,26 @@
     bcr_v4d g = {0.0, 0.0, 0.0, 0.0};
 #pragma unroll
     for (int kk = 0; kk < 16; ++kk) g = __builtin_amdgcn_mfma_f64_16x16x4f64(vf[kk], vt[kk], g, 0, 0, 0);
-    const double* Sm = A.side != 0 ? A.Lf + (int64_t)A.last * (192 + a1) * 64 + 4096 + 64 * a1 : nullptr;
-    double mc[4];
-#pragma unroll
-    for (int r = 0; r < 4; ++r) { const int q1 = 16 * t1 + li, q2 = 16 * t2 + lq + 4 * r; mc[r] = (q1 < a1 && q2 < a1) ? A.Mc[q1 * a1 + q2] + (Sm != nullptr ? Sm[q1 * a1 + q2] : 0.0) : 0.0; }
-#pragma unroll
-    for (int r = 0; r < 4; ++r) { const int q1 = 16 * t1 + li, q2 = 16 * t2 + lq + 4 * r; if (q1 < a1 && q2 < a1) W[q2 * LD + q1] = mc[r] - g[r]; }
+#pragma unroll
+    for (int r = 0; r < 4; ++r) { const int q1 = 16 * t1 + li, q2 = 16 * t2 + lq + 4 * r; if (q1 < a1 && q2 < a1) W[q2 * LD + q1] = Cs[q1 * a1 + q2] - g[r]; }
+  }
+  double lv[kBackRows], yv = 0.0;
+#pragma unroll
+  for (int k = 0; k < kBackRows; ++k) lv[k] = 0.0;
+  constexpr int BW0 = NW - kBackWaves;
+  int fi = 0; bool f_hasL = false, f_hasR = false;
+  if (FOLD) {
+    const int kp = 2 * (int)blockIdx.x + A.p;
+    fi = A.o + kp * A.s; f_hasL = kp > 0; f_hasR = kp < A.m - 1;
   }
   __syncthreads();
-  bcr_corner_solve<LD>(W, da, failp, a, tid, wave, lane);
-  for (int q = tid; q < a; q += NT) A.x[A.Pb + q] = da[q];
+  bcr_corner_solve<LD>(W, da, failp, a, tid, wave, lane, [&]() {
+    if (FOLD && wave >= BW0) {
+      bcri_back_rows(A.Lf + (int64_t)fi * (192 + a1) * 64 + 4096, a, f_hasL, f_hasR, wave - BW0, lane, lv, yv);
+      asm volatile("" ::: "memory");
+    }
+  });
+  if (shared_writer) for (int q = tid; q < a; q += NT) A.x[A.Pb + q] = da[q];
   if (wave == 0) {
     const double* tc = W + lane * LD + 64;
     double v = tc[a];
@@ -218,11 +264,11 @@
       for (int k = 0; k < 8; ++k) v = fma(-t8[k], d8[k], v);
     }
     const int gi = A.last * 64 + lane;
-    if (gi < A.Pb) A.x[gi] = v;
+    if (shared_writer && gi < A.Pb) A.x[gi] = v;
     x0s[lane] = gi < A.Pb ? v : 0.0;
   }
   __syncthreads();
-  if (tid == 0 && *failp) atomicOr(A.fail, 1);
+  if (shared_writer && tid == 0 && *failp) atomicOr(A.fail, 1);
   if (A.top_l >= 0 || A.top_r >= 0) {
     double sum_r = 0.0, sum_l = 0.0;
 #pragma unroll
@@ -241,14 +287,25 @@
 #pragma unroll
       for (int w = 0; w < NW; ++w) acc += W[(wave * NW + w) * 64 + lane];
       const int gi = blk * 64 + lane;
-      if (blk >= 0 && gi < A.Pb) A.x[gi] = ytop - acc;
+      const bool ok = blk >= 0 && gi < A.Pb;
+      if (shared_writer && ok) A.x[gi] = ytop - acc;
+      if (FOLD) x0s[64 * (1 + wave) + lane] = ok ? ytop - acc : 0.0;
+    }
+    if (FOLD) {
+      __syncthreads();
+      auto x_of = [&](int blk) -> const double* { return blk == A.last ? x0s : (blk == A.top_r ? x0s + 64 : x0s + 128); };
+      BcrBackX X;
+      X.hasL = f_hasL; X.hasR = f_hasR; X.xl = x_of(fi - A.s); X.xr = x_of(fi + A.s); X.xa = da;
+      const double xv = bcri_back_body(lv, yv, X, a, W + 2 * NW * 64, wave >= BW0, wave - BW0, lane);
+      const int gi = fi * 64 + lane;
+      if (wave == BW0 && gi < A.Pb) A.x[gi] = xv;
     }
   }
 }
 
 
 struct BcrNoPark { __device__ __forceinline__ void operator()(double*) const {} };
-template <bool LAST, bool PROF, bool ZLDS = false, class LoadD, class Park = BcrNoPark>
+template <bool LAST, bool PROF, bool ZLDS = false, bool FOLD = false, class LoadD, class Park = BcrNoPark>
 __device__ __forceinline__ void bcri_invert_body(const BcrArgs& A, const int i, LoadD load_d, const bool report = true, Park park = Park()) {
   constexpr int LD = kInvLD, NW = kInvWaves, NT = 64 * NW, NTILE = 20, SLOTS = (NTILE + NW - 1) / NW, RU = 128, NAW = 3, FLD = 65;
   static_assert(NW == 16, "the corner phases of block 0 take one tile per wave");
@@ -261,10 +318,12 @@
   int* const failp = reinterpret_cast<int*>(da + 64);
   double* const dg = da + 64 + 8;
   double* const Fs = dg + 256;
+  double* const Cs = Fs + 64 * FLD;
   const int a1 = A.a + 1;
   double* Zg = A.Lf + (int64_t)i * (192 + a1) * 64;
   const double* Fg = A.F + (int64_t)i * 64 * a1;
   const double* Sf = (LAST && A.side != 0) ? Zg + 4096 : nullptr;
+  const double* Sm = (LAST && A.side != 0) ? Zg + 4096 + 64 * a1 : nullptr;
   const bool prof = PROF && A.prof != nullptr && blockIdx.x == 0 && wave == 0;
   long long pc[8] = {0, 0, 0, 0, 0, 0, 0, 0};
   long long tprev = prof ? clock64() : 0;
@@ -289,12 +348,13 @@
   }
   {
     constexpr int PER = 4096 / NT;
-    double gd[PER], gf[PER];
+    double gd[PER], gf[PER], gc[PER];
 #pragma unroll
     for (int k = 0; k < PER; ++k) {
       const int e = tid + k * NT;
       gd[k] = load_d(e);
       if (LAST) { const int c = e >> 6, q = e & 63; gf[k] = q < a1 ? Fg[c * a1 + q] + (Sf != nullptr ? Sf[c * a1 + q] : 0.0) : 0.0; }
+      if (LAST) gc[k] = e < a1 * a1 ? A.Mc[e] + (Sm != nullptr ? Sm[e] : 0.0) : 0.0;
     }
 #pragma unroll
     for (int k = 0; k < PER; ++k) {
@@ -304,6 +364,7 @@
       if (c < 16 && r < 16) dg[c * 16 + r] = r >= c ? gd[k] : 0.0;
       W[c * LD + 64 + r] = r == c ? 1.0 : 0.0;
       if (LAST) Fs[c * FLD + r] = gf[k];
+      if (LAST && e < a1 * a1) Cs[e] = gc[k];
     }
     park(Fs);
   }
@@ -389,7 +450,7 @@
     BCR_MARK(4);
   }
   BCR_MARK(4);
-  bcri_tail<LAST, ZLDS>(A, W, da, failp, Fs, Zg, tid, wave, lane, report, ttop, ytop, dg);
+  bcri_tail<LAST, ZLDS, FOLD>(A, W, da, failp, Fs, Cs, Zg, tid, wave, lane, report, ttop, ytop, dg);
   BCR_MARK(5);
   if (PROF && prof && lane == 0) for (int k = 0; k < 8; ++k) A.prof[k] = pc[k];
 #undef BCR_MARK
@@ -402,6 +463,14 @@
   const double* Dg = A.D + (int64_t)i * 4096;
   const double* Sd = (LAST && A.side != 0) ? A.Lf + (int64_t)i * (192 + A.a + 1) * 64 : nullptr;
   bcri_invert_body<LAST, PROF>(A, i, [Dg, Sd](int e) { double v = Dg[e]; if (LAST && Sd != nullptr && (e & 63) >= (e >> 6)) v += Sd[e]; return v; });
+}
+
+__global__ __launch_bounds__(64 * kInvWaves) void bcri_last_backward_kernel(BcrArgs A) {
+  BCR_RETURN_IF_DONE(A);
+  const int i = A.last;
+  const double* Dg = A.D + (int64_t)i * 4096;
+  const double* Sd = A.side != 0 ? A.Lf + (int64_t)i * (192 + A.a + 1) * 64 : nullptr;
+  bcri_invert_body<true, false, false, true>(A, i, [Dg, Sd](int e) { double v = Dg[e]; if (Sd != nullptr && (e & 63) >= (e >> 6)) v += Sd[e]; return v; });
 }
 
 struct BcrSchurGroup {
@@ -687,34 +756,19 @@
   const bool hasL = kp > 0;
   const bool hasR = kp < A.m - 1 || A.ghost != 0;
   const int ir = kp < A.m - 1 ? i + s : A.n;
-  const double* Tg = A.Lf + (int64_t)i * (192 + a1) * 64 + 4096;
-  constexpr int RW = 192 / kBackWaves;
-  double lv[RW];
-#pragma unroll
-  for (int k = 0; k < RW; ++k) {
-    const int r = wave + kBackWaves * k;
-    const bool ok = r < 128 + a && (hasL || r >= 64) && (hasR || r < 64 || r >= 128);
-    lv[k] = ok ? Tg[r * 64 + lane] : 0.0;
-  }
-  const double yv = wave == 0 ? Tg[(128 + a) * 64 + lane] : 0.0;
+  double lv[kBackRows], yv;
+  bcri_back_rows(A.Lf + (int64_t)i * (192 + a1) * 64 + 4096, a, hasL, hasR, wave, lane, lv, yv);
   double xin = 0.0;
   if (tid < 64) { const int gi = il * 64 + tid; xin = (hasL && gi < A.Pb) ? A.x[gi] : 0.0; }
   else if (tid < 128) { const int gi = ir * 64 + (tid - 64); xin = (hasR && gi < A.Pb) ? A.x[gi] : 0.0; }
   else if (tid < 128 + a) xin = A.x[A.Pb + (tid - 128)];
   if (tid < 192) xs[tid] = xin;
   __syncthreads();
-  double sum = 0.0;
-#pragma unroll
-  for (int k = 0; k < RW; ++k) { const int r = wave + kBackWaves * k; sum = fma(lv[k], r < 128 + a ? xs[r] : 0.0, sum); }
-  part[wave][lane] = sum;
-  __syncthreads();
-  if (wave == 0) {
-    double acc = 0.0;
-#pragma unroll
-    for (int w = 0; w < kBackWaves; ++w) acc += part[w][lane];
-    const int gi = i * 64 + lane;
-    if (gi < A.Pb) A.x[gi] = yv - acc;
-  }
+  BcrBackX X;
+  X.xl = xs; X.xr = xs + 64; X.xa = xs + 128; X.hasL = true; X.hasR = true;
+  const double xv = bcri_back_body(lv, yv, X, a, &part[0][0], true, wave, lane);
+  const int gi = i * 64 + lane;
+  if (wave == 0 && gi < A.Pb) A.x[gi] = xv;
 }
 
 template <bool RETRACT>
@@ -1055,21 +1109,26 @@
   }
   return fused;
 }
-static bool bcr_launch_last_and_back(BcrArgs A, const BcrLevels& L, hipStream_t st, const RetractReq* R = nullptr, const SolveBuffers* sb = nullptr) {
+static int bcr_fold_level(int on, bool prof, int ghost, int b0, const BcrLevels& L) {
+  return (on != 0 && !prof && ghost == 0 && b0 == 0 && L.nlev >= 2 && (L.nlev & 1) == 0) ? L.nlev - 2 : -1;
+}
+static bool bcr_launch_last_and_back(BcrArgs A, const BcrLevels& L, hipStream_t st, const RetractReq* R = nullptr, const SolveBuffers* sb = nullptr, int fold = -1) {
   using KernelFn = void (*)(BcrArgs);
-  KernelFn k_inv_last = bcri_invert_kernel<true, false>;
-  const size_t lds_inv_last = bcr_lds_inv() + (size_t)64 * 65 * sizeof(double);
-  bcr_allow_lds(reinterpret_cast<const void*>(k_inv_last), lds_inv_last);
+  KernelFn k_inv_last = fold >= 0 ? bcri_last_backward_kernel : bcri_invert_kernel<true, false>;
+  const int a1 = A.a + 1;
+  const size_t lds_inv_last = bcr_lds_inv() + (size_t)(64 * 65 + a1 * a1) * sizeof(double);
+  bcr_allow_lds(reinterpret_cast<const void*>(k_inv_last), bcr_lds_inv() + (size_t)(64 * 65 + 64 * 64) * sizeof(double));
   const int nlev = L.nlev;
   A.o = 0; A.s = 0; A.p = 1; A.m = 1; A.pn = 1; A.offS_in = 0; A.offS_out = 0; A.carry = 0;
+  if (fold >= 0) bcr_set_level(A, L, fold);
   A.last = L.last; A.top_l = -1; A.top_r = -1; A.side = (nlev >= 1 && L.parity[nlev - 1] == 0) ? 1 : 0;
   if (nlev >= 1) {
     const int t = nlev - 1;
     A.top_r = L.last + L.strides[t];
     if (L.parity[t] == 0) A.top_l = L.last - L.strides[t];
   }
-  hipLaunchKernelGGL(k_inv_last, dim3(1), dim3(64 * kInvWaves), lds_inv_last, st, A);
-  return bcr_launch_back(A, L, nlev - 2, st, R, sb);
+  hipLaunchKernelGGL(k_inv_last, dim3(fold >= 0 ? L.npivs[fold] : 1), dim3(64 * kInvWaves), lds_inv_last, st, A);
+  return bcr_launch_back(A, L, fold >= 0 ? fold - 1 : nlev - 2, st, R, sb);
 }
 
 int bcr_route(const TangentLayout& tl, const SolveBuffers& sb) {
@@ -1094,7 +1153,9 @@
   if (sb.bcr_joined != nullptr) { sb.bcr_joined[0] = joined; sb.bcr_joined[1] += joined; }
   const bool honour = retract != nullptr && retract->on != 0 && retract->rmap != nullptr && retract->alpha == 1.0 && L.nlev >= 3 && A.ghost == 0 && A.b0 == 0;
   RetractReq R{}; if (honour) { R = *retract; R.ne = ne; }
-  const bool did = bcr_launch_last_and_back(A, L, st, honour ? &R : nullptr, &sb);
+  const int fold = bcr_fold_level(sb.bcr_fold, A.prof != nullptr, A.ghost, A.b0, L);
+  if (sb.bcr_folded != nullptr) { sb.bcr_folded[0] = fold >= 0 ? 1 : 0; sb.bcr_folded[1] += fold >= 0 ? 1 : 0; }
+  const bool did = bcr_launch_last_and_back(A, L, st, honour ? &R : nullptr, &sb, fold);
   if (fused) *fused = did;
   return 0;
 }
@@ -1242,3 +1303,9 @@
   }
   return L.nlev;
 }
+
+extern "C" int oicc_debug_bcr_fold_plan(int32_t n, int32_t ghost, int32_t odd_only, int32_t b0, int32_t on) {
+  if (n < 1 || b0 < 0 || ghost < 0 || ghost > 1) return INT32_MIN;
+  const oicc::BcrLevels L = oicc::bcr_plan(n, ghost, odd_only != 0);
+  return oicc::bcr_fold_level(on, false, ghost, b0, L);
+}
diff --git a/openimucameracalibrator_amd/csrc/oicc_device.h b/openimucameracalibrator_amd/csrc/oicc_device.h
--- a/openimucameracalibrator_amd/csrc/oicc_device.h
+++ b/openimucameracalibrator_amd/csrc/oicc_device.h
@@ -118,6 +118,7 @@
   int bcr_max_border = 64;
   int bcr_delay = 0;
   int bcr_join = 0, bcr_join_budget = 0; int64_t* bcr_joined = nullptr;
+  int bcr_fold = 0; int64_t* bcr_folded = nullptr;
   const LmCtl* ctl = nullptr;
   const LmCtl* ctl_prev = nullptr; const LmState* st_prev = nullptr; int64_t off_cost = 0;
 };
diff --git a/openimucameracalibrator_amd/csrc/oicc_exchange.hip b/openimucameracalibrator_amd/csrc/oicc_exchange.hip
--- a/openimucameracalibrator_amd/csrc/oicc_exchange.hip
+++ b/openimucameracalibrator_amd/csrc/oicc_exchange.hip
@@ -425,6 +425,12 @@
   out4[0] = p->bcr_joined[0]; out4[1] = p->bcr_joined[1]; out4[2] = sb.bcr_join_budget; out4[3] = sb.bcr_join;
   return OICC_OK;
 }
+int oicc_debug_bcr_fold_info(oicc_problem* p, int64_t out3[3]) {
+  if (!p || !out3) return OICC_ERR_INVALID_ARG;
+  const SolveBuffers sb = solve_buffers(p);
+  out3[0] = p->bcr_folded[0]; out3[1] = p->bcr_folded[1]; out3[2] = sb.bcr_fold;
+  return OICC_OK;
+}
 
 int oicc_time_allreduce(oicc_problem* p, int32_t flags, int32_t repeats, double* ms_per_call, int64_t* bytes) {
   int rc = prepare(p, flags); if (rc) return rc;
diff --git a/openimucameracalibrator_amd/csrc/oicc_problem.h b/openimucameracalibrator_amd/csrc/oicc_problem.h
--- a/openimucameracalibrator_amd/csrc/oicc_problem.h
+++ b/openimucameracalibrator_amd/csrc/oicc_problem.h
@@ -147,6 +147,7 @@
   void seg_invalidate(const double* xbuf) { if (SegTable* t = seg_of(xbuf)) t->valid = false; }
   int n_cu = 256;
   int64_t bcr_joined[2] = {0, 0};
+  int64_t bcr_folded[2] = {0, 0};
   bool seg_precomputed() const { const auto it = opt.find("debug_seg_precompute"); const int force = it == opt.end() ? 0 : int(it->second); return force == 1 || (force == 0 && tp.n_tiles > n_cu); }
   DevBuf<int32_t> d_corner_view, d_corner_pt, d_view_s_so3, d_view_s_r3;
   DevBuf<double> d_cu, d_cv, d_cisx, d_cisy, d_view_u_so3, d_view_u_r3;
@@ -234,6 +235,7 @@
     opt["bcr_max_border"] = 64;
     opt["bcr_join_levels"] = 1;
     opt["bcr_join_max_workgroups"] = 0;
+    opt["bcr_fold_back"] = 1;
     opt["debug_check_ne"] = 0;
     opt["debug_sync"] = 0;
     opt["covariance_min_rcond"] = 1e-12;
diff --git a/openimucameracalibrator_amd/csrc/oicc_problem.hip b/openimucameracalibrator_amd/csrc/oicc_problem.hip
--- a/openimucameracalibrator_amd/csrc/oicc_problem.hip
+++ b/openimucameracalibrator_amd/csrc/oicc_problem.hip
@@ -75,6 +75,7 @@
   sb.radius = 0.0; sb.bcr_max_border = int(p->opt["bcr_max_border"]); sb.bcr_delay = int(p->opt["debug_bcr_delay"]);
   const int join_max = int(p->opt["bcr_join_max_workgroups"]);
   sb.bcr_join = p->opt["bcr_join_levels"] != 0.0 ? 1 : 0; sb.bcr_join_budget = join_max > 0 ? join_max : p->n_cu; sb.bcr_joined = p->bcr_joined;
+  sb.bcr_fold = p->opt["bcr_fold_back"] != 0.0 ? 1 : 0; sb.bcr_folded = p->bcr_folded;
   return sb;
 }
 
diff --git a/openimucameracalibrator_amd/estimator.py b/openimucameracalibrator_amd/estimator.py
--- a/openimucameracalibrator_amd/estimator.py
+++ b/openimucameracalibrator_amd/estimator.py
@@ -344,6 +344,13 @@
         out = (C.c_int64 * 4)()
         self._ck(fn(self._h, out))
         return dict(last=int(out[0]), total=int(out[1]), budget=int(out[2]), on=bool(out[3]))
+
+    def BcrFoldInfo(self):
+        fn = self._b.lib.oicc_debug_bcr_fold_info
+        fn.restype = C.c_int; fn.argtypes = [C.c_void_p, C.POINTER(C.c_int64)]
+        out = (C.c_int64 * 3)()
+        self._ck(fn(self._h, out))
+        return dict(last=int(out[0]), total=int(out[1]), on=bool(out[2]))
 
     ROUTES = ("bcr_fused", "bcr_unfused", "sweep64", "sweep128", "partitioned", "global", "distributed")
 
```

New measurement: 53.62 million (median of 6 runs). 1.02x the previous value.
